# ideafisher/ssUnet-GAN

Hardware: AMD Instinct MI355X
Metric: train images/sec (512^2 tiles) (higher is better)
Workload: dtype f32; 1 GPU; UNet_R_SS_v2 generator + SRGAN-style discriminator, one G+D step (train_seg_gan.py:182-233), 16 x 3x512x512 tiles per GPU, fp32, Adam lr 2e-5; global_batch=16, tile=512, parallelism=dp1, dead_d_param_grads_of_g_step=computed

## Files before the change

### include/ssunet_hip.h

```cpp
#ifndef SSUNET_HIP_H
#define SSUNET_HIP_H

#include <stdint.h>

#ifdef __cplusplus
extern "C" {
#endif

#define SSG_OK 0
#define SSG_EINVAL (-1)
#define SSG_EALIGN (-2)

#define SSG_ACT_NONE 0
#define SSG_ACT_RELU 1
#define SSG_ACT_LRELU 2
#define SSG_ACT_SWISH 3

#define SSG_MAX_TAPS 9

const char* ssg_last_error(void);
int ssg_abi_version(void);

typedef struct {
  const float* in1; const float* in2;
// ... 39 lines not shown
int ssg_pack_weights_bf16x1_taps(const float* w_packed, int R, int Kp, int ntaps, int BN, void* out, void* stream);

int64_t ssg_conv2d_workspace_bytes(const ssg_conv_desc* d);

int ssg_conv2d_igemm_f32(const ssg_conv_desc* d, void* stream);
int ssg_conv2d_f32(const ssg_conv_desc* d, void* stream);
int ssg_conv2d_kernel_id(const ssg_conv_desc* d);
int ssg_conv2d_bnpart_rows(const ssg_conv_desc* d);

int ssg_pack_weights_f32(const float* w_oihw, int O, int I, int KH, int KW,
                         int transpose, int ntaps, const int* ky, const int* kx,
                         int kmode, int Cred_pad, int Kp, float* out, void* stream);
int ssg_pack_weights_scaled_f32(const float* w_oihw, int O, int I, int KH, int KW,
                                int transpose, int ntaps, const int* ky, const int* kx,
                                int kmode, int Cred_pad, int Kp, const float* sigma, float* out, void* stream);

typedef struct {
  const float* in1; const float* in2; int C1, C2, ld1, ld2;
  int N, H, W;
  const float* dout; int Cout, ldd; int GH, GW;
  int in_sy, in_sx;
  int ntaps; int dy[SSG_MAX_TAPS]; int dx[SSG_MAX_TAPS]; int ky[SSG_MAX_TAPS]; int kx[SSG_MAX_TAPS];
  int KH, KW, Cin_real;
  float* dw_oihw;
  float* ws; int64_t ws_bytes;
  int flags;
  const float* in_scale; const float* in_shift; int in_act; float in_slope;
} ssg_wgrad_desc;

int64_t ssg_conv2d_wgrad_workspace_bytes(const ssg_wgrad_desc* d);
int ssg_conv2d_wgrad_in_affine_ok(const ssg_wgrad_desc* d);
int ssg_conv2d_wgrad_f32(const ssg_wgrad_desc* d, void* stream);
int ssg_conv2d_wgrad_kernel_id(const ssg_wgrad_desc* d);
int ssg_wgrad_set_k32_mode(int mode);

int ssg_conv2d_wgrad_bf16x1_ok(const ssg_wgrad_desc* d);
int64_t ssg_conv2d_wgrad_bf16x1_workspace_bytes(const ssg_wgrad_desc* d);
int ssg_conv2d_wgrad_bf16x1_f32(const ssg_wgrad_desc* d, void* stream);
int ssg_conv2d_wgrad_bf16x1_kernel_id(const ssg_wgrad_desc* d);

int ssg_conv2d_wgrad_bf16x1_s2_ok(const ssg_wgrad_desc* d);
int64_t ssg_conv2d_wgrad_bf16x1_s2_workspace_bytes(const ssg_wgrad_desc* d);
int ssg_conv2d_wgrad_bf16x1_s2_f32(const ssg_wgrad_desc* d, void* stream);
int ssg_conv2d_wgrad_bf16x1_s2_kernel_id(const ssg_wgrad_desc* d);

int ssg_pixel_gate_fwd_f32(const float* x, int ldx, const float* g, int ldg, int64_t P, int C, float* y, int ldy, void* stream);
int ssg_pixel_gate_bwd_f32(const float* x, int ldx, const float* g, int ldg, const float* dy, int lddy, int64_t P, int C,
                           float* dx, int lddx, float* dg, int lddg, void* stream);

int64_t ssg_linear_fwd_workspace_bytes(int n, int k, int o);
int ssg_linear_fwd_f32(const float* x, int n, int k, int ldx, const float* w, int o, const float* bias, int act,
                       float slope, float* y, int ldy, float* ws, int64_t ws_bytes, void* stream);
int ssg_linear_wgrad_f32(const float* x, int n, int k, int ldx, const float* dy, int o, int ldd, float* dw, void* stream);

int ssg_pack_weights_bf16(const float* w, int O, int I, int transpose, int rows_pad, int Kp, void* out, void* stream);
int ssg_gemm_bf16(const void* x, int64_t P, int K, int ldx, const void* w_packed, int Kp, int N,
                  const void* res, int ldr, void* out, int ldo, void* stream);
int64_t ssg_gemm_wgrad_bf16_workspace_bytes(int64_t P, int M, int N);
int ssg_gemm_wgrad_bf16(const void* dy, int ldd, const void* x, int ldx, int64_t P, int M, int N, float* dw,
                        void* ws, int64_t ws_bytes, void* stream);

int ssg_conv2d_thin_bf16(const float* x, int N, int H, int W, int ldx, const float* w_oihw, int Cout, int Cin, int KH, int KW,
                         int stride, int pad_t, int pad_l, int OH, int OW, void* y, int ldy, void* stream);
int64_t ssg_conv2d_thin_bf16_wgrad_workspace_bytes(int N, int OH, int OW, int Cout, int KH, int KW);
int ssg_conv2d_thin_bf16_wgrad(const float* x, int N, int H, int W, int ldx, const void* dy, int lddy, int Cout, int Cin,
                               int KH, int KW, int stride, int pad_t, int pad_l, int OH, int OW, float* dw_oihw, void* ws,
                               void* stream);
int ssg_conv2d_thin_bf16_dgrad(const void* dy, int lddy, int N, int H, int W, const float* w_oihw, int Cout, int Cin, int KH, int KW,
                               int stride, int pad_t, int pad_l, int OH, int OW, float* dx, int lddx, void* stream);

int ssg_bn_stats_bf16(const void* x, int64_t P, int C, int ld, double* sums, int with_count, void* ws, void* stream);
int ssg_bn_apply_bf16(const void* x, int64_t P, int C, int ld, const float* scale, const float* shift,
                      const void* res, int ldr, int act, float slope, void* y, int ldy, void* stream);
int ssg_bn_bwd_reduce_bf16(const void* x, const void* y, const void* dy, int64_t P, int C, int ldx, int ldy, int lddy,
                           const float* mean, const float* invstd, const float* scale, const float* shift,
                           int act, float slope, double* sums, int with_count, void* ws, void* stream);
int ssg_bn_bwd_apply_bf16(const void* x, const void* y, const void* dy, int64_t P, int C, int ldx, int ldy, int lddy,
                          const float* mean, const float* invstd, const float* weight, const float* scale, const float* shift,
                          const double* sums, double count, int act, float slope, void* dx, int lddx, void* dres, int lddres,
                          float* dweight, float* dbias, void* stream);
int ssg_dwconv2d_fwd_bf16(const void* in, int N, int H, int W, int C, int ld, const float* w, const float* bias, int KH, int KW,
                          int stride, int pad_top, int pad_left, int OH, int OW, void* out, int ldo, void* stream);
int ssg_dwconv2d_dgrad_bf16(const void* dout, int lddo, int N, int H, int W, int C, const float* w, int KH, int KW, int stride,
                            int pad_top, int pad_left, int OH, int OW, void* dx, int lddx, void* stream);
int ssg_dwconv2d_wgrad_bf16(const void* in, int N, int H, int W, int C, int ld, const void* dout, int lddo, int KH, int KW,
                            int stride, int pad_top, int pad_left, int OH, int OW, float* dw, void* ws, void* stream);
int ssg_channel_scale_fwd_bf16(const void* x, int ldx, const float* s, int N, int64_t S, int C, void* y, int ldy, void* stream);
int ssg_sample_channel_sum_bf16(const void* a, int lda, const void* b, int ldb, int N, int64_t S, int C, float scale,
                                float* out, void* ws, void* stream);
int ssg_broadcast_rows_bf16(const float* s, int N, int64_t S, int C, float scale, void* y, int ldy, void* stream);
int ssg_add_bf16(const void* a, int lda, const void* b, int ldb, int64_t P, int C, void* out, int ldo, void* stream);
int ssg_convert_f32_to_bf16(const float* src, int ldsrc, int64_t P, int C, void* dst, int lddst, void* stream);
int ssg_convert_bf16_to_f32(const void* src, int ldsrc, int64_t P, int C, float* dst, int lddst, void* stream);

int ssg_nchw_to_nhwc_f32(const float* src, int N, int C, int H, int W, float* dst, int ld, void* stream);
int ssg_nhwc_to_nchw_f32(const float* src, int ld, int N, int C, int H, int W, float* dst, void* stream);

int64_t ssg_bn_workspace_bytes(int64_t P, int C);
int ssg_bn_stats_f32(const float* x, int64_t P, int C, int ld, double* sums, int with_count, void* ws, void* stream);
int64_t ssg_bn_stats_from_partials_workspace_bytes(int rows, int C);
int ssg_bn_stats_from_partials_f32(const double* part, int rows, int C, double* sums, double count, void* ws, void* stream);
int ssg_bn_finalize_f32(const double* sums, double count, int C, const float* weight, const float* bias,
                        float eps, float momentum, int var_mode,
                        float* running_mean, float* running_var,
                        float* mean, float* invstd, float* scale, float* shift, void* stream);

typedef struct ssg_bn_fin {
  const float* weight; const float* bias;
  float eps, momentum; int var_mode;
  float* running_mean; float* running_var;
  float* mean; float* invstd; float* scale; float* shift;
} ssg_bn_fin;
int ssg_bn_stats_finalize_f32(const float* x, int64_t P, int C, int ld, const ssg_bn_fin* fin, void* ws, void* stream);
int ssg_bn_stats_finalize_bf16(const void* x, int64_t P, int C, int ld, const ssg_bn_fin* fin, void* ws, void* stream);
int ssg_bn_stats_from_partials_finalize_f32(const double* part, int rows, int C, double count, const ssg_bn_fin* fin, void* ws, void* stream);
int ssg_bn_apply_f32(const float* x, int64_t P, int C, int ld, const float* scale, const float* shift,
                     const float* res, int ldr, int act, float slope, float* y, int ldy, void* stream);
int ssg_bn_bwd_reduce_f32(const float* x, const float* y, const float* dy, int64_t P, int C,
                          int ldx, int ldy, int lddy, const float* mean, const float* invstd,
                          const float* scale, const float* shift,
                          int act, float slope, double* sums, int with_count, void* ws, void* stream);
int ssg_bn_bwd_apply_f32(const float* x, const float* y, const float* dy, int64_t P, int C,
                         int ldx, int ldy, int lddy, const float* mean, const float* invstd,
                         const float* weight, const float* scale, const float* shift,
                         const double* sums, double count, int act, float slope,
                         float* dx, int lddx, float* dres, int lddres,
                         float* dweight, float* dbias, void* stream);
int ssg_bn_frozen_bwd_f32(const float* x, const float* y, const float* dy, int64_t P, int C, int ldx, int ldy, int lddy,
                          const float* mean, const float* invstd, const float* scale, const float* shift, int act, float slope,
                          float* dx, int lddx, float* dres, int lddres, double* sums, void* ws, void* stream);
int ssg_bn_fold_bwd_f32(const float* dwf, const float* w, int Cout, int64_t K, const float* s, const float* mean,
                        const float* invstd, const double* sums_g, float* dw, float* dgamma, float* dbeta, void* stream);

int ssg_maxpool2x2_fwd_f32(const float* x, int N, int H, int W, int C, int ldx, float* y, int ldy, uint8_t* idx, void* stream);
int ssg_maxpool2x2_bwd_f32(const float* dy, int lddy, const uint8_t* idx, int N, int H, int W, int C, float* dx, int lddx, void* stream);
int ssg_maxpool2x2_bwd_add_f32(const float* dy, int lddy, const uint8_t* idx, const float* res, int ldr, int N, int H, int W, int C,
                               float* dx, int lddx, void* stream);
int ssg_maxunpool2x2_fwd_f32(const float* x, int ldx, const uint8_t* idx, int N, int OH, int OW, int C, float* y, int ldy, void* stream);
int ssg_maxunpool2x2_bwd_f32(const float* dy, int lddy, const uint8_t* idx, int N, int OH, int OW, int C, float* dx, int lddx, void* stream);
int ssg_upsample2x_bilinear_fwd_f32(const float* x, int N, int H, int W, int C, int ldx, float* y, int ldy, void* stream);
int ssg_upsample2x_bilinear_bwd_f32(const float* dy, int lddy, int N, int H, int W, int C, float* dx, int lddx, void* stream);
int ssg_upsample2x_nearest_fwd_f32(const float* x, int N, int H, int W, int C, int ldx, float* y, int ldy, void* stream);
int ssg_upsample2x_nearest_bwd_f32(const float* dy, int lddy, int N, int H, int W, int C, float* dx, int lddx, void* stream);
int ssg_adaptive_avgpool_flat_fwd_f32(const float* x, int N, int H, int W, int C, int ldx, int OHW, float* y, void* stream);
int ssg_adaptive_avgpool_flat_bwd_f32(const float* dy, int N, int H, int W, int C, int OHW, float* dx, int lddx, void* stream);

int ssg_spade_conv_modulate_ok(const ssg_conv_desc* d);
int ssg_spade_conv_modulate_f32(const ssg_conv_desc* d, const float* x, int ldx, float* gamma, int ldg, void* stream);
int ssg_spade_modulate_fwd_f32(const float* x, int ldx, const float* gb, int ldgb, int64_t P, int C, float* y, int ldy, void* stream);
int ssg_spade_modulate_bwd_f32(const float* x, int ldx, const float* gb, int ldgb, const float* dy, int lddy, int64_t P, int C,
                               float* dx, int lddx, float* dgb, int lddgb, void* stream);
int ssg_spade_modulate_bwd_sums_f32(const float* x, int ldx, const float* gb, int ldgb, const float* dy, int lddy, int64_t P,
                                    int C, float* dx, int lddx, float* dgb, int lddgb, double* sums, void* ws, void* stream);
int ssg_act_bwd_f32(const float* y, int ldy, const float* dy, int lddy, int64_t P, int C, int act, float slope, float* dx, int lddx, void* stream);
int ssg_copy_channels_f32(const float* src, int ldsrc, int64_t P, int C, float* dst, int lddst, void* stream);
int ssg_add_f32(const float* a, const float* b, int64_t n, float* out, void* stream);
int ssg_nan_to_zero_f32(float* x, int64_t n, uint8_t* mask, void* stream);
int ssg_mask_zero_f32(const float* g, const uint8_t* mask, int64_t n, float* out, void* stream);

int64_t ssg_seg_loss_workspace_bytes(int N, int64_t S, int C);
int ssg_seg_loss_fwd_f32(const float* x, int ldx, const float* t, int ldt, int N, int64_t S, int C, int mc0,
                         float* res, double* stats, void* ws, void* stream);
int ssg_seg_loss_bwd_f32(const float* x, int ldx, const float* t, int ldt, int N, int64_t S, int C,
                         const float* res, const double* stats, const float* g_seg, const float* g_mse,
                         const float* g_bce, float* dx, int lddx, void* stream);
int ssg_bce_logits_const_fwd_f32(const float* x, int n, int ldx, float label, float* loss, void* stream);
int ssg_bce_logits_const_bwd_f32(const float* x, int n, int ldx, float label, const float* g, float* dx, int lddx, void* stream);

int ssg_clamp_adam_multi_f32(const void* const* ptrs, const int64_t* sizes, const int32_t* blk_tensor,
                             const int32_t* blk_chunk, int nblocks, float clip, double lr, double beta1,
                             double beta2, double eps, double weight_decay, double bias_corr1,
                             double bias_corr2_sqrt, void* stream);
int ssg_clamp_sgd_multi_f32(const void* const* ptrs, const int64_t* sizes, const int32_t* blk_tensor,
                            const int32_t* blk_chunk, int nblocks, float clip, double lr, double momentum,
                            double dampening, double weight_decay, int nesterov, void* stream);
int ssg_clamp_f32(float* x, int64_t n, float lo, float hi, void* stream);
int ssg_clamp_multi_f32(const void* const* ptrs, const int64_t* sizes, const int32_t* blk_tensor, const int32_t* blk_chunk,
                        int nblocks, int which, float lo, float hi, void* stream);

int ssg_channel_sum_f32(const float* x, int64_t P, int C, int ld, float* out, void* ws, void* stream);

int ssg_dwconv2d_fwd_f32(const float* in, int N, int H, int W, int C, int ld, const float* w, const float* bias, int KH, int KW,
                         int stride, int pad_top, int pad_left, int OH, int OW, float* out, int ldo, void* stream);
int ssg_dwconv2d_dgrad_f32(const float* dout, int lddo, int N, int H, int W, int C, const float* w, int KH, int KW, int stride,
                           int pad_top, int pad_left, int OH, int OW, float* dx, int lddx, void* stream);
int64_t ssg_dwconv2d_wgrad_workspace_bytes(int N, int OH, int OW, int C, int KH, int KW);
int ssg_dwconv2d_kernel_id(int op, int stride, int KH, int KW, int pad_left, int64_t NDH, int C, int aligned16);
int ssg_dwconv2d_wgrad_f32(const float* in, int N, int H, int W, int C, int ld, const float* dout, int lddo, int KH, int KW,
                           int stride, int pad_top, int pad_left, int OH, int OW, float* dw, void* ws, void* stream);
#define SSG_UNARY_SWISH 0
#define SSG_UNARY_SIGMOID 1
#define SSG_UNARY_GAUSSIAN 2
int ssg_unary_fwd_f32(const float* x, int ldx, int64_t P, int C, int op, float* y, int ldy, void* stream);
int ssg_unary_bwd_f32(const float* x, int ldx, const float* dy, int lddy, int64_t P, int C, int op, float* dx, int lddx, void* stream);
int ssg_mul_fwd_f32(const float* a, int lda, const float* b, int ldb, int64_t P, int C, float* y, int ldy, void* stream);
int ssg_mul_bwd_f32(const float* a, int lda, const float* b, int ldb, const float* dy, int lddy, int64_t P, int C,
                    float* da, int ldda, float* db, int lddb, void* stream);
int ssg_channel_scale_fwd_f32(const float* x, int ldx, const float* s, int N, int64_t S, int C, float* y, int ldy, void* stream);
int64_t ssg_sample_channel_sum_workspace_bytes(int N, int64_t S, int C);
int ssg_sample_channel_sum_f32(const float* a, int lda, const float* b, int ldb, int N, int64_t S, int C, float scale, float* out,
                               void* ws, void* stream);
int ssg_broadcast_rows_f32(const float* s, int N, int64_t S, int C, float scale, float* y, int ldy, void* stream);
int64_t ssg_spectral_norm_workspace_bytes(int rows, int cols);
int ssg_spectral_norm_fwd_f32(const float* W, int rows, int cols, float* u, float* v, int n_power_iterations, double eps,
                              float* W_out, float* sigma, void* ws, void* stream);
int ssg_spectral_norm_bwd_f32(const float* dWsn, const float* W, int rows, int cols, const float* u, const float* v,
                              const float* sigma, float* dW, void* ws, void* stream);

int ssg_se_gate_ok(int N, int C, int S);
int64_t ssg_se_gate_workspace_floats(int N, int C, int S);
int ssg_se_gate_fwd_f32(const float* sq, int ldq, int N, int C, const float* w1, const float* b1, const float* w2, const float* b2,
                        int S, float* h_pre, float* gate, int ldg, float* tmp, void* stream);
int ssg_se_gate_bwd_f32(const float* dgate, int ldd, const float* gate, int ldg, const float* h_pre, const float* sq, int ldq, int N, int C,
                        const float* w1, const float* w2, int S, float* dsq, int lds_, float* dw1, float* db1, float* dw2, float* db2,
                        float* tmp, void* stream);

int ssg_tool_mfma_peak_f32(float* scratch, int blocks, int iters, void* stream);
int ssg_tool_mfma_peak_bf16(float* scratch, int blocks, int iters, void* stream);
int ssg_tool_mfma_peak_bf16_data(float* scratch, int blocks, int iters, const void* data, void* stream);
int ssg_tool_mfma_peak_bf16_data16(float* scratch, int blocks, int iters, const void* data, void* stream);
int ssg_tool_copy_f32(const float* src, float* dst, int64_t n, void* stream);

int ssg_sw_gather_patches_u8_f32(const uint8_t* img, int H, int W, const int32_t* org, const int32_t* org_host, int P,
                                 int p_size, int out_size, float mean0, float mean1, float mean2,
                                 float rdenom0, float rdenom1, float rdenom2, float* out, void* stream);
int ssg_sw_merge_masks_f32_u8(const float* probs, int ld, int P, int C, int S, const int32_t* org, const int32_t* org_host,
                              const int32_t* weight, int p_size, int H, int W, uint8_t* out, void* stream);

#ifdef __cplusplus
}
#endif
#endif
```

### ssunet-gan_amd/_lib.py

```python
import ctypes as C
import os

import torch

_HERE = os.path.dirname(os.path.abspath(__file__))
LIB_PATH = os.environ.get('SSG_LIB_PATH') or os.path.join(_HERE, 'libssunet_hip.so')
MAX_TAPS = 9
ACT_NONE, ACT_RELU, ACT_LRELU, ACT_SWISH = 0, 1, 2, 3


class HipLibraryError(RuntimeError):
    pass


class ConvDesc(C.Structure):
    _fields_ = [
        ('in1', C.c_void_p), ('in2', C.c_void_p),
        ('C1', C.c_int), ('C2', C.c_int), ('ld1', C.c_int), ('ld2', C.c_int),
        ('N', C.c_int), ('H', C.c_int), ('W', C.c_int),
        ('w', C.c_void_p), ('Kp', C.c_int), ('kmode', C.c_int),
        ('bias', C.c_void_p),
        ('res', C.c_void_p), ('ldr', C.c_int),
        ('out', C.c_void_p), ('Cout', C.c_int), ('ldo', C.c_int),
        ('GH', C.c_int), ('GW', C.c_int), ('OH', C.c_int), ('OW', C.c_int),
        ('in_sy', C.c_int), ('in_sx', C.c_int), ('out_sy', C.c_int), ('out_sx', C.c_int),
        ('out_oy', C.c_int), ('out_ox', C.c_int),
        ('ntaps', C.c_int), ('dy', C.c_int * MAX_TAPS), ('dx', C.c_int * MAX_TAPS),
        ('act', C.c_int), ('slope', C.c_float),
        ('bnpart', C.c_void_p),
        ('ws', C.c_void_p), ('ws_bytes', C.c_int64),
        ('w_split', C.c_void_p), ('parity_merge', C.c_int),
        ('in_scale', C.c_void_p), ('in_shift', C.c_void_p), ('in_act', C.c_int), ('in_slope', C.c_float),
        ('bwd_x', C.c_void_p), ('bwd_ldx', C.c_int), ('bwd_scale', C.c_void_p), ('bwd_shift', C.c_void_p), ('bwd_mean', C.c_void_p),
        ('bwd_act', C.c_int), ('bwd_slope', C.c_float),
    ]


class WgradDesc(C.Structure):
    _fields_ = [
        ('in1', C.c_void_p), ('in2', C.c_void_p),
        ('C1', C.c_int), ('C2', C.c_int), ('ld1', C.c_int), ('ld2', C.c_int),
        ('N', C.c_int), ('H', C.c_int), ('W', C.c_int),
        ('dout', C.c_void_p), ('Cout', C.c_int), ('ldd', C.c_int), ('GH', C.c_int), ('GW', C.c_int),
        ('in_sy', C.c_int), ('in_sx', C.c_int),
        ('ntaps', C.c_int), ('dy', C.c_int * MAX_TAPS), ('dx', C.c_int * MAX_TAPS),
        ('ky', C.c_int * MAX_TAPS), ('kx', C.c_int * MAX_TAPS),
        ('KH', C.c_int), ('KW', C.c_int), ('Cin_real', C.c_int),
        ('dw_oihw', C.c_void_p),
        ('ws', C.c_void_p), ('ws_bytes', C.c_int64),
        ('flags', C.c_int),
        ('in_scale', C.c_void_p), ('in_shift', C.c_void_p), ('in_act', C.c_int), ('in_slope', C.c_float),
    ]


_P, _I, _L, _F, _D = C.c_void_p, C.c_int, C.c_int64, C.c_float, C.c_double


class BnFin(C.Structure):
    _fields_ = [('weight', C.c_void_p), ('bias', C.c_void_p), ('eps', C.c_float), ('momentum', C.c_float), ('var_mode', C.c_int),
                ('running_mean', C.c_void_p), ('running_var', C.c_void_p),
                ('mean', C.c_void_p), ('invstd', C.c_void_p), ('scale', C.c_void_p), ('shift', C.c_void_p)]


SIGNATURES = {
    'ssg_abi_version': [],
    'ssg_conv2d_igemm_f32': [C.POINTER(ConvDesc), _P],
    'ssg_conv2d_f32': [C.POINTER(ConvDesc), _P],
    'ssg_conv2d_kernel_id': [C.POINTER(ConvDesc)],
    'ssg_conv2d_bnpart_rows': [C.POINTER(ConvDesc)],
    'ssg_conv2d_workspace_bytes': [C.POINTER(ConvDesc)],
    'ssg_conv2d_thin_bf16': [_P, _I, _I, _I, _I, _P, _I, _I, _I, _I, _I, _I, _I, _I, _I, _P, _I, _P],
    'ssg_conv2d_thin_bf16_wgrad_workspace_bytes': [_I, _I, _I, _I, _I, _I],
    'ssg_conv2d_thin_bf16_wgrad': [_P, _I, _I, _I, _I, _P, _I, _I, _I, _I, _I, _I, _I, _I, _I, _I, _P, _P, _P],
    'ssg_conv2d_thin_bf16_dgrad': [_P, _I, _I, _I, _I, _P, _I, _I, _I, _I, _I, _I, _I, _I, _I, _P, _I, _P],
    'ssg_conv2d_split_bn': [C.POINTER(ConvDesc)],
    'ssg_conv2d_in_affine_ok': [C.POINTER(ConvDesc)],
    'ssg_conv2d_bwd_stats_ok': [C.POINTER(ConvDesc)],
    'ssg_conv2d_wgrad_in_affine_ok': [C.POINTER(WgradDesc)],
    'ssg_pack_weights_split_bytes': [_I, _I, _I],
    'ssg_conv_set_k32_mode': [_I],
    'ssg_wgrad_set_k32_mode': [_I],
    'ssg_pack_weights_split_bf16x3': [_P, _I, _I, _I, _P, _P],
    'ssg_conv2d_bf16x1_ok': [C.POINTER(ConvDesc)],
    'ssg_conv2d_bf16x1_kernel_id': [C.POINTER(ConvDesc)],
    'ssg_conv2d_bf16x1_f32': [C.POINTER(ConvDesc), _P, _P],
    'ssg_pack_weights_bf16x1_bytes': [_I, _I, _I],
    'ssg_pack_weights_bf16x1': [_P, _I, _I, _I, _P, _P],
    'ssg_conv2d_bf16x1_s2_ok': [C.POINTER(ConvDesc)],
    'ssg_conv2d_bf16x1_s2_kernel_id': [C.POINTER(ConvDesc)],
    'ssg_conv2d_bf16x1_s2_f32': [C.POINTER(ConvDesc), _P, _P],
    'ssg_conv2d_bf16x1_cls_ok': [C.POINTER(ConvDesc)],
    'ssg_conv2d_bf16x1_cls_kernel_id': [C.POINTER(ConvDesc)],
    'ssg_conv2d_bf16x1_cls_f32': [C.POINTER(ConvDesc), _P, _P],
    'ssg_pack_weights_bf16x1_taps_bytes': [_I, _I, _I, _I],
    'ssg_pack_weights_bf16x1_taps': [_P, _I, _I, _I, _I, _P, _P],
    'ssg_conv2d_wgrad_bf16x1_ok': [C.POINTER(WgradDesc)],
    'ssg_conv2d_wgrad_bf16x1_kernel_id': [C.POINTER(WgradDesc)],
    'ssg_conv2d_wgrad_bf16x1_workspace_bytes': [C.POINTER(WgradDesc)],
    'ssg_conv2d_wgrad_bf16x1_f32': [C.POINTER(WgradDesc), _P],
    'ssg_conv2d_wgrad_bf16x1_s2_ok': [C.POINTER(WgradDesc)],
    'ssg_conv2d_wgrad_bf16x1_s2_kernel_id': [C.POINTER(WgradDesc)],
    'ssg_conv2d_wgrad_bf16x1_s2_workspace_bytes': [C.POINTER(WgradDesc)],
    'ssg_conv2d_wgrad_bf16x1_s2_f32': [C.POINTER(WgradDesc), _P],
    'ssg_bn_stats_from_partials_workspace_bytes': [_I, _I],
    'ssg_bn_stats_from_partials_f32': [_P, _I, _I, _P, _D, _P, _P],
    'ssg_conv2d_wgrad_kernel_id': [C.POINTER(WgradDesc)],
    'ssg_pack_weights_f32': [_P, _I, _I, _I, _I, _I, _I, C.POINTER(C.c_int), C.POINTER(C.c_int), _I, _I, _I, _P, _P],
    'ssg_pack_weights_scaled_f32': [_P, _I, _I, _I, _I, _I, _I, C.POINTER(C.c_int), C.POINTER(C.c_int), _I, _I, _I, _P, _P, _P],
    'ssg_conv2d_wgrad_workspace_bytes': [C.POINTER(WgradDesc)],
    'ssg_conv2d_wgrad_f32': [C.POINTER(WgradDesc), _P],
    'ssg_nchw_to_nhwc_f32': [_P, _I, _I, _I, _I, _P, _I, _P],
    'ssg_nhwc_to_nchw_f32': [_P, _I, _I, _I, _I, _I, _P, _P],
    'ssg_bn_workspace_bytes': [_L, _I],
    'ssg_bn_stats_f32': [_P, _L, _I, _I, _P, _I, _P, _P],
    'ssg_bn_finalize_f32': [_P, _D, _I, _P, _P, _F, _F, _I, _P, _P, _P, _P, _P, _P, _P],
    'ssg_bn_apply_f32': [_P, _L, _I, _I, _P, _P, _P, _I, _I, _F, _P, _I, _P],
    'ssg_bn_bwd_reduce_f32': [_P, _P, _P, _L, _I, _I, _I, _I, _P, _P, _P, _P, _I, _F, _P, _I, _P, _P],
    'ssg_bn_bwd_apply_f32': [_P, _P, _P, _L, _I, _I, _I, _I, _P, _P, _P, _P, _P, _P, _D, _I, _F, _P, _I, _P, _I, _P, _P, _P],
    'ssg_bn_frozen_bwd_f32': [_P, _P, _P, _L, _I, _I, _I, _I, _P, _P, _P, _P, _I, _F, _P, _I, _P, _I, _P, _P, _P],
    'ssg_bn_fold_bwd_f32': [_P, _P, _I, _L, _P, _P, _P, _P, _P, _P, _P, _P],
    'ssg_maxpool2x2_fwd_f32': [_P, _I, _I, _I, _I, _I, _P, _I, _P, _P],
    'ssg_maxpool2x2_bwd_f32': [_P, _I, _P, _I, _I, _I, _I, _P, _I, _P],
    'ssg_maxpool2x2_bwd_add_f32': [_P, _I, _P, _P, _I, _I, _I, _I, _I, _P, _I, _P],
    'ssg_maxunpool2x2_fwd_f32': [_P, _I, _P, _I, _I, _I, _I, _P, _I, _P],
    'ssg_maxunpool2x2_bwd_f32': [_P, _I, _P, _I, _I, _I, _I, _P, _I, _P],
    'ssg_upsample2x_bilinear_fwd_f32': [_P, _I, _I, _I, _I, _I, _P, _I, _P],
    'ssg_upsample2x_bilinear_bwd_f32': [_P, _I, _I, _I, _I, _I, _P, _I, _P],
    'ssg_upsample2x_nearest_fwd_f32': [_P, _I, _I, _I, _I, _I, _P, _I, _P],
    'ssg_upsample2x_nearest_bwd_f32': [_P, _I, _I, _I, _I, _I, _P, _I, _P],
    'ssg_adaptive_avgpool_flat_fwd_f32': [_P, _I, _I, _I, _I, _I, _I, _P, _P],
    'ssg_adaptive_avgpool_flat_bwd_f32': [_P, _I, _I, _I, _I, _I, _P, _I, _P],
    'ssg_spade_conv_modulate_ok': [C.POINTER(ConvDesc)],
    'ssg_spade_conv_modulate_f32': [C.POINTER(ConvDesc), _P, _I, _P, _I, _P],
    'ssg_spade_modulate_fwd_f32': [_P, _I, _P, _I, _L, _I, _P, _I, _P],
    'ssg_spade_modulate_bwd_f32': [_P, _I, _P, _I, _P, _I, _L, _I, _P, _I, _P, _I, _P],
    'ssg_spade_modulate_bwd_sums_f32': [_P, _I, _P, _I, _P, _I, _L, _I, _P, _I, _P, _I, _P, _P, _P],
    'ssg_act_bwd_f32': [_P, _I, _P, _I, _L, _I, _I, _F, _P, _I, _P],
    'ssg_add_f32': [_P, _P, _L, _P, _P],
    'ssg_copy_channels_f32': [_P, _I, _L, _I, _P, _I, _P],
    'ssg_nan_to_zero_f32': [_P, _L, _P, _P],
    'ssg_mask_zero_f32': [_P, _P, _L, _P, _P],
    'ssg_seg_loss_workspace_bytes': [_I, _L, _I],
    'ssg_seg_loss_fwd_f32': [_P, _I, _P, _I, _I, _L, _I, _I, _P, _P, _P, _P],
    'ssg_seg_loss_bwd_f32': [_P, _I, _P, _I, _I, _L, _I, _P, _P, _P, _P, _P, _P, _I, _P],
    'ssg_bce_logits_const_fwd_f32': [_P, _I, _I, _F, _P, _P],
    'ssg_bce_logits_const_bwd_f32': [_P, _I, _I, _F, _P, _P, _I, _P],
    'ssg_clamp_adam_multi_f32': [_P, _P, _P, _P, _I, _F, _D, _D, _D, _D, _D, _D, _D, _P],
    'ssg_clamp_sgd_multi_f32': [_P, _P, _P, _P, _I, _F, _D, _D, _D, _D, _I, _P],
    'ssg_clamp_f32': [_P, _L, _F, _F, _P],
    'ssg_clamp_multi_f32': [_P, _P, _P, _P, _I, _I, _F, _F, _P],
    'ssg_channel_sum_f32': [_P, _L, _I, _I, _P, _P, _P],
    'ssg_dwconv2d_fwd_f32': [_P, _I, _I, _I, _I, _I, _P, _P, _I, _I, _I, _I, _I, _I, _I, _P, _I, _P],
    'ssg_dwconv2d_dgrad_f32': [_P, _I, _I, _I, _I, _I, _P, _I, _I, _I, _I, _I, _I, _I, _P, _I, _P],
    'ssg_dwconv2d_wgrad_workspace_bytes': [_I, _I, _I, _I, _I, _I],
    'ssg_dwconv2d_kernel_id': [_I, _I, _I, _I, _I, _L, _I, _I],
    'ssg_dwconv2d_wgrad_f32': [_P, _I, _I, _I, _I, _I, _P, _I, _I, _I, _I, _I, _I, _I, _I, _P, _P, _P],
    'ssg_unary_fwd_f32': [_P, _I, _L, _I, _I, _P, _I, _P],
    'ssg_unary_bwd_f32': [_P, _I, _P, _I, _L, _I, _I, _P, _I, _P],
    'ssg_mul_fwd_f32': [_P, _I, _P, _I, _L, _I, _P, _I, _P],
    'ssg_mul_bwd_f32': [_P, _I, _P, _I, _P, _I, _L, _I, _P, _I, _P, _I, _P],
    'ssg_channel_scale_fwd_f32': [_P, _I, _P, _I, _L, _I, _P, _I, _P],
    'ssg_sample_channel_sum_workspace_bytes': [_I, _L, _I],
    'ssg_sample_channel_sum_f32': [_P, _I, _P, _I, _I, _L, _I, _F, _P, _P, _P],
    'ssg_broadcast_rows_f32': [_P, _I, _L, _I, _F, _P, _I, _P],
    'ssg_spectral_norm_workspace_bytes': [_I, _I],
    'ssg_spectral_norm_fwd_f32': [_P, _I, _I, _P, _P, _I, _D, _P, _P, _P, _P],
    'ssg_spectral_norm_bwd_f32': [_P, _P, _I, _I, _P, _P, _P, _P, _P, _P],
    'ssg_pixel_gate_fwd_f32': [_P, _I, _P, _I, _L, _I, _P, _I, _P],
    'ssg_pixel_gate_bwd_f32': [_P, _I, _P, _I, _P, _I, _L, _I, _P, _I, _P, _I, _P],
    'ssg_linear_fwd_workspace_bytes': [_I, _I, _I],
    'ssg_linear_fwd_f32': [_P, _I, _I, _I, _P, _I, _P, _I, _F, _P, _I, _P, _L, _P],
    'ssg_linear_wgrad_f32': [_P, _I, _I, _I, _P, _I, _I, _P, _P],
    'ssg_pack_weights_bf16': [_P, _I, _I, _I, _I, _I, _P, _P],
    'ssg_gemm_bf16': [_P, _L, _I, _I, _P, _I, _I, _P, _I, _P, _I, _P],
    'ssg_gemm_wgrad_bf16_workspace_bytes': [_L, _I, _I],
    'ssg_gemm_wgrad_bf16': [_P, _I, _P, _I, _L, _I, _I, _P, _P, _L, _P],
    'ssg_bn_stats_finalize_f32': [_P, _L, _I, _I, C.POINTER(BnFin), _P, _P],
    'ssg_bn_stats_finalize_bf16': [_P, _L, _I, _I, C.POINTER(BnFin), _P, _P],
    'ssg_bn_stats_from_partials_finalize_f32': [_P, _I, _I, _D, C.POINTER(BnFin), _P, _P],
    'ssg_se_gate_ok': [_I, _I, _I],
    'ssg_se_gate_workspace_floats': [_I, _I, _I],
    'ssg_se_gate_fwd_f32': [_P, _I, _I, _I, _P, _P, _P, _P, _I, _P, _P, _I, _P, _P],
    'ssg_se_gate_bwd_f32': [_P, _I, _P, _I, _P, _P, _I, _I, _I, _P, _P, _I, _P, _I, _P, _P, _P, _P, _P, _P],
    'ssg_tool_mfma_peak_f32': [_P, _I, _I, _P],
    'ssg_tool_mfma_peak_bf16': [_P, _I, _I, _P],
    'ssg_tool_mfma_peak_bf16_data': [_P, _I, _I, _P, _P],
    'ssg_tool_mfma_peak_bf16_data16': [_P, _I, _I, _P, _P],
    'ssg_tool_copy_f32': [_P, _P, _L, _P],
    'ssg_sw_gather_patches_u8_f32': [_P, _I, _I, _P, _P, _I, _I, _I, _F, _F, _F, _F, _F, _F, _P, _P],
    'ssg_sw_merge_masks_f32_u8': [_P, _I, _I, _I, _I, _P, _P, _P, _I, _I, _I, _P, _P],
}

for _n in ('ssg_bn_stats', 'ssg_bn_apply', 'ssg_bn_bwd_reduce', 'ssg_bn_bwd_apply', 'ssg_dwconv2d_fwd', 'ssg_dwconv2d_dgrad', 'ssg_dwconv2d_wgrad', 'ssg_channel_scale_fwd', 'ssg_sample_channel_sum', 'ssg_broadcast_rows'):
    SIGNATURES[_n + '_bf16'] = SIGNATURES[_n + '_f32']
SIGNATURES['ssg_add_bf16'] = [_P, _I, _P, _I, _L, _I, _P, _I, _P]
SIGNATURES['ssg_convert_f32_to_bf16'] = [_P, _I, _L, _I, _P, _I, _P]
SIGNATURES['ssg_convert_bf16_to_f32'] = [_P, _I, _L, _I, _P, _I, _P]
_RESTYPES = {
    'ssg_conv2d_wgrad_workspace_bytes': C.c_int64,
    'ssg_conv2d_wgrad_bf16x1_workspace_bytes': C.c_int64,
    'ssg_conv2d_wgrad_bf16x1_s2_workspace_bytes': C.c_int64,
    'ssg_conv2d_workspace_bytes': C.c_int64,
    'ssg_pack_weights_split_bytes': C.c_int64,
    'ssg_pack_weights_bf16x1_bytes': C.c_int64,
    'ssg_pack_weights_bf16x1_taps_bytes': C.c_int64,
    'ssg_bn_workspace_bytes': C.c_int64,
    'ssg_se_gate_workspace_floats': C.c_int64,
    'ssg_seg_loss_workspace_bytes': C.c_int64,
    'ssg_dwconv2d_wgrad_workspace_bytes': C.c_int64,
    'ssg_spectral_norm_workspace_bytes': C.c_int64,
    'ssg_linear_fwd_workspace_bytes': C.c_int64,
    'ssg_sample_channel_sum_workspace_bytes': C.c_int64,
    'ssg_gemm_wgrad_bf16_workspace_bytes': C.c_int64,
    'ssg_conv2d_thin_bf16_wgrad_workspace_bytes': C.c_int64,
    'ssg_bn_stats_from_partials_workspace_bytes': C.c_int64,
}
_NO_STATUS = set(_RESTYPES) | {'ssg_abi_version', 'ssg_conv2d_split_bn', 'ssg_conv2d_in_affine_ok', 'ssg_conv2d_wgrad_in_affine_ok', 'ssg_conv2d_bwd_stats_ok', 'ssg_conv2d_kernel_id', 'ssg_conv2d_bnpart_rows', 'ssg_conv2d_bf16x1_ok', 'ssg_conv2d_bf16x1_kernel_id', 'ssg_conv2d_bf16x1_s2_ok', 'ssg_conv2d_bf16x1_s2_kernel_id', 'ssg_conv2d_bf16x1_cls_ok', 'ssg_conv2d_bf16x1_cls_kernel_id', 'ssg_conv2d_wgrad_bf16x1_ok', 'ssg_conv2d_wgrad_bf16x1_kernel_id', 'ssg_conv2d_wgrad_bf16x1_s2_ok', 'ssg_conv2d_wgrad_bf16x1_s2_kernel_id', 'ssg_conv2d_wgrad_kernel_id', 'ssg_dwconv2d_kernel_id',
                                'ssg_spade_conv_modulate_ok', 'ssg_se_gate_ok'}

ABI_VERSION = 10

_lib = None


def load():
    global _lib
    if _lib is not None:
        return _lib
    if not os.path.exists(LIB_PATH):
        raise HipLibraryError(
            'HIP extension not built: %s is missing. Run `python -c "import __graft_entry__ as g; g.build()"` '
            '(or `make -C ssunet-gan_amd/csrc`). There is no CPU fallback.' % LIB_PATH)
    lib = C.CDLL(LIB_PATH)
    lib.ssg_last_error.restype = C.c_char_p
    lib.ssg_last_error.argtypes = []
    for name, args in SIGNATURES.items():
        fn = getattr(lib, name)
        fn.argtypes = args
        fn.restype = _RESTYPES.get(name, C.c_int)
    got = lib.ssg_abi_version()
    if got != ABI_VERSION:
        raise HipLibraryError('%s reports ABI version %d, this package was written against %d: rebuild it '
                              '(`make -C ssunet-gan_amd/csrc`)' % (LIB_PATH, got, ABI_VERSION))
    _lib = lib
    return lib


def call(name, *args):
    lib = load()
    rc = getattr(lib, name)(*args)
    if name in _NO_STATUS:
        return rc
    if rc != 0:
        msg = lib.ssg_last_error().decode('utf-8', 'replace')
        raise HipLibraryError('%s failed (status %d): %s' % (name, rc, msg))
    return rc


def stream_ptr():
    return C.c_void_p(torch.cuda.current_stream().cuda_stream)


def require_gpu(t):
    if not t.is_cuda:
        raise HipLibraryError('ssunet-gan_amd ops run only on an MI355X (cuda/HIP) device; got a %s tensor. '
                              'There is no CPU fallback.' % t.device)


def ptr(t):
    return C.c_void_p(t.data_ptr()) if t is not None else C.c_void_p(0)
```

### ssunet-gan_amd/blocks.py

```python
import ctypes as C

import torch

from . import ops
from ._lib import ACT_NONE, ACT_RELU, call, ptr, stream_ptr
from .ops import (_act_bwd, _bn_bwd_impl, _bn_fwd_impl, _channel_sum, _conv_dgrad_impl, _conv_fwd_impl, _conv_wgrad_impl,
                  _ld, new_nhwc, to_nhwc)


class _BasicBlockFn(torch.autograd.Function):

    @staticmethod
    def forward(ctx, x1, x2, w1, g1, b1, rm1, rv1, w2, g2, b2, rm2, rv2, wsc, eps1, mom1, eps2, mom2, stride, var_mode, group):
        x1 = to_nhwc(x1)
        x2 = to_nhwc(x2) if x2 is not None else None
        ctx.x1m = x1m = ops.train_precision_mode() == 'bf16x1' and stride == 1
        p3 = 'bf16x1' if x1m else 'fp32'
        c1, part1 = _conv_fwd_impl(x1, x2, w1, None, stride, 1, ACT_NONE, 0.0, want_bn=True, precision=p3)
        y1 = None
        c2 = None
        if ops.BN_FUSE_INPUT and part1 is not None and not x1m:
            _, st1, cnt1 = _bn_fwd_impl(c1, g1, b1, rm1, rv1, None, eps1, mom1, ACT_RELU, 0.0, var_mode, group, part=part1, apply=False)
            r = _conv_fwd_impl(c1, None, w2, None, 1, 1, ACT_NONE, 0.0, want_bn=True, in_affine=(st1[2], st1[3], ACT_RELU, 0.0))
            if r is not None:
# ... 59 lines not shown
                None, None, None, None, None, None, None)


def basic_block(x1, x2, conv1, bn1, conv2, bn2, shortcut_conv, group=None):
    for bn in (bn1, bn2):
        if bn.track_running_stats and bn.num_batches_tracked is not None and not ops._synced(group):
            bn.num_batches_tracked.add_(1)
    var_mode = getattr(bn1, '_ssg_var_mode', 1 if group is not None else 0)
    return _BasicBlockFn.apply(x1, x2, conv1.weight, bn1.weight, bn1.bias, bn1.running_mean, bn1.running_var,
                               conv2.weight, bn2.weight, bn2.bias, bn2.running_mean, bn2.running_var,
                               shortcut_conv.weight if shortcut_conv is not None else None,
                               float(bn1.eps), float(bn1.momentum), float(bn2.eps), float(bn2.momentum),
                               int(conv1.stride[0]), var_mode, group)


def _fold_bwd(dwf, w, s, mean, invstd, sums_g, need_w, need_gb):
    o = w.shape[0]
    dw = torch.empty_like(dwf) if need_w else None
    dgb = torch.empty((2, o), dtype=torch.float32, device=w.device) if need_gb else None
    wc = w.detach().contiguous()
    call('ssg_bn_fold_bwd_f32', ptr(dwf), ptr(wc), o, wc.numel() // o, ptr(s), ptr(mean), ptr(invstd), ptr(sums_g), ptr(dw),
         ptr(dgb[0]) if need_gb else None, ptr(dgb[1]) if need_gb else None, stream_ptr())
    return dw, (dgb[0] if need_gb else None), (dgb[1] if need_gb else None)


class _FrozenBasicBlockFn(torch.autograd.Function):

    @staticmethod
    def forward(ctx, x1, x2, w1, g1, b1, w2, g2, b2, wsc, wf1, bf1, wf2, bf2, k1, k2, stride, record):
        x1 = to_nhwc(x1)
        x2 = to_nhwc(x2) if x2 is not None else None
        x1m = record and any(ctx.needs_input_grad) and ops.train_precision_mode() == 'bf16x1' and stride == 1
        p3 = 'bf16x1' if x1m else 'fp32'
        y1 = _conv_fwd_impl(x1, x2, wf1, bf1, stride, 1, ACT_RELU, 0.0, precision=p3)
        if wsc is not None:
            r = _conv_fwd_impl(x1, x2, wsc, None, stride, 0, ACT_NONE, 0.0)
        else:
            if x2 is not None:
                raise ValueError('identity shortcut with a two-tensor input')
            r = x1
        out = _conv_fwd_impl(y1, None, wf2, bf2, 1, 1, ACT_RELU, 0.0, res=r, precision=p3)
        if record and any(ctx.needs_input_grad):
            ctx.save_for_backward(x1, x2, y1, out, w1, w2, wsc, wf1, wf2, *k1, *k2)
            ctx.stride = stride
            ctx.x1m = x1m
        return out

    @staticmethod
    @torch.autograd.function.once_differentiable
    def backward(ctx, dout):
        x1, x2, y1, out, w1, w2, wsc, wf1, wf2, s1, m1, is1, s2, m2, is2 = ctx.saved_tensors
        stride = ctx.stride
        p3 = 'bf16x1' if ctx.x1m else 'fp32'
        dout = to_nhwc(dout)
        n, ca, h, w = x1.shape
        cb = x2.shape[1] if x2 is not None else 0
        need = ctx.needs_input_grad
        need_x1, need_x2 = need[0], (x2 is not None and need[1])
        need_w1, need_gb1, need_w2, need_gb2 = need[2], (need[3] or need[4]), need[5], (need[6] or need[7])
        need_wsc = wsc is not None and need[8]
        if stride != 1 and (need_x1 or need_x2):
            raise NotImplementedError('strided BasicBlock input gradient')
        g2, _, sums2 = ops._frozen_bwd(None, out, dout, None, None, None, None, ACT_RELU, 0.0)
        dw2 = dg2 = db2 = None
        if need_w2 or need[6]:
            dwf2 = _conv_wgrad_impl(y1, None, g2, w2.shape, 1, 1, precision=p3)
            dw2, dg2, db2 = _fold_bwd(dwf2, w2, s2, m2, is2, sums2, need_w2, need_gb2)
        elif need_gb2:
            db2 = sums2[:w2.shape[0]].float()
        dwsc = _conv_wgrad_impl(x1, x2, g2, wsc.shape, stride, 0) if need_wsc else None
        dw1 = dg1 = db1 = dx1 = dx2 = None
        if need_w1 or need_gb1 or need_x1 or need_x2:
            dy1 = _conv_dgrad_impl(g2, wf2, 1, 1, y1.shape[2], y1.shape[3], 0, y1.shape[1], precision=p3)
            g1, _, sums1 = ops._frozen_bwd(None, y1, dy1, None, None, None, None, ACT_RELU, 0.0)
            del dy1
            if need_w1 or need[3]:
                dwf1 = _conv_wgrad_impl(x1, x2, g1, w1.shape, stride, 1, precision=p3)
                dw1, dg1, db1 = _fold_bwd(dwf1, w1, s1, m1, is1, sums1, need_w1, need_gb1)
            elif need_gb1:
                db1 = sums1[:w1.shape[0]].float()
            if need_x1:
                part = _conv_dgrad_impl(g2, wsc, 1, 0, h, w, 0, ca) if wsc is not None else g2
                dx1 = _conv_dgrad_impl(g1, wf1, 1, 1, h, w, 0, ca, res=part, precision=p3)
            if need_x2:
                part = _conv_dgrad_impl(g2, wsc, 1, 0, h, w, ca, ca + cb)
                dx2 = _conv_dgrad_impl(g1, wf1, 1, 1, h, w, ca, ca + cb, res=part, precision=p3)
        return (dx1, dx2, dw1, dg1 if need[3] else None, db1 if need[4] else None, dw2, dg2 if need[6] else None,
                db2 if need[7] else None, dwsc, None, None, None, None, None, None, None, None)


def frozen_basic_block(x1, x2, conv1, bn1, conv2, bn2, shortcut_conv, folded, consts):
    wf1, bf1, wf2, bf2 = folded
    return _FrozenBasicBlockFn.apply(x1, x2, conv1.weight, bn1.weight, bn1.bias, conv2.weight, bn2.weight, bn2.bias,
                                     shortcut_conv.weight if shortcut_conv is not None else None, wf1, bf1, wf2, bf2,
                                     consts[0], consts[1], int(conv1.stride[0]), torch.is_grad_enabled())


def _spade_cat(wg, bg, wb, bb):
    stamp = tuple((t.data_ptr(), t._version) for t in (wg, bg, wb, bb)) + (ops._WEIGHT_EPOCH[0],)
    hit = wg.__dict__.get('_ssg_gb_cat')
    if hit is not None and hit[0] == stamp:
        return hit[1], hit[2]
    with torch.no_grad():
        w = torch.cat([wg.detach(), wb.detach()], 0).contiguous()
        b = torch.cat([bg.detach(), bb.detach()], 0).contiguous()
    ops._attach(wg, '_ssg_gb_cat', (stamp, w, b))
    return w, b


def _spade_fused_fwd(x, a, wgb, bgb, pad, out):
    o, i, kh, kw = wgb.shape
    n, c, h, w = x.shape
    cin = ops.pad4(a.shape[1])
    if kh != 3 or kw != 3 or pad != 1 or cin not in (4, 8) or o != 2 * c or c % 4:
        return None
    taps = ops._taps_fwd(kh, kw, pad)
    wpk, kp, kmode = ops._pack(wgb, 0, taps, cin, cin)
    d = ops._conv_desc(ops._at(a), cin, None, 0, (n, h, w), wpk.data_ptr(), kp, kmode, bgb, None, ops._at(out), o,
                       (h, w, h, w), 1, 1, (0, 0), taps, ACT_NONE, 0.0)
    if not call('ssg_spade_conv_modulate_ok', C.byref(d)):
        return None
    gamma = new_nhwc(n, c, h, w, x.device)
    with ops._Timed('thin32_cin_kernel<spade>' if ops.PROFILE is not None else None, 2.0 * n * h * w * o * a.shape[1] * 9):
        call('ssg_spade_conv_modulate_f32', C.byref(d), ptr(x), _ld(x), ptr(gamma), _ld(gamma), stream_ptr())
    return gamma


class _SpadeFn(torch.autograd.Function):

    @staticmethod
    def forward(ctx, x, wx, bx, ws, bs, wg, bg, wb, bb, pad):
        x = to_nhwc(x)
        n, c, h, w = x.shape
        seg = _conv_fwd_impl(x, None, wx, bx, 1, pad, ACT_NONE, 0.0)
        a = _conv_fwd_impl(seg, None, ws, bs, 1, pad, ACT_RELU, 0.0)
        wgb, bgb = _spade_cat(wg, bg, wb, bb)
        out = new_nhwc(n, c, h, w, x.device)
        gb = _spade_fused_fwd(x, a, wgb, bgb, pad, out)
        if gb is None:
            gb = _conv_fwd_impl(a, None, wgb, bgb, 1, pad, ACT_NONE, 0.0)
            with ops._hbm('spade_modulate_fwd', 16.0 * n * h * w * c):
                call('ssg_spade_modulate_fwd_f32', ptr(x), _ld(x), ptr(gb), _ld(gb), n * h * w, c, ptr(out), _ld(out), stream_ptr())
        ctx.save_for_backward(x, seg, a, gb, wx, ws, wgb)
        ctx.pad = pad
        return out

    @staticmethod
    @torch.autograd.function.once_differentiable
    def backward(ctx, dout):
        x, seg, a, gb, wx, ws, wgb = ctx.saved_tensors
        pad = ctx.pad
        dout = to_nhwc(dout)
        n, c, h, w = x.shape
        dxm = new_nhwc(n, c, h, w, x.device)
        dgb = new_nhwc(n, 2 * c, h, w, x.device)
        scratch = ops._ws(call('ssg_bn_workspace_bytes', n * h * w, c), x.device)
        sums = torch.empty(2 * c, dtype=torch.float64, device=x.device)
        with ops._hbm('spade_modulate_bwd', 4.0 * n * h * w * c * (3 + 3)):
            call('ssg_spade_modulate_bwd_sums_f32', ptr(x), _ld(x), ptr(gb), _ld(gb), ptr(dout), _ld(dout), n * h * w, c,
                 ptr(dxm), _ld(dxm), ptr(dgb), _ld(dgb), ptr(sums), ptr(scratch), stream_ptr())
        dwgb = _conv_wgrad_impl(a, None, dgb, wgb.shape, 1, pad)
        dbias_gb = sums.float()
        nh = a.shape[1]
        da = _conv_dgrad_impl(dgb, wgb, 1, pad, h, w, 0, nh)
        da = _act_bwd(a, da, ACT_RELU, 0.0)
        dws = _conv_wgrad_impl(seg, None, da, ws.shape, 1, pad)
        dbs = _channel_sum(da, nh)
        dseg = _conv_dgrad_impl(da, ws, 1, pad, h, w, 0, seg.shape[1])
        dwx = _conv_wgrad_impl(x, None, dseg, wx.shape, 1, pad)
        dbx = _channel_sum(dseg, seg.shape[1])
        dx = _conv_dgrad_impl(dseg, wx, 1, pad, h, w, 0, c, res=dxm) if ctx.needs_input_grad[0] else None
        return dx, dwx, dbx, dws, dbs, dwgb[:c], dbias_gb[:c], dwgb[c:], dbias_gb[c:], None


def spade_self(x, x2map, shared, gamma, beta):
    return _SpadeFn.apply(x, x2map.weight, x2map.bias, shared.weight, shared.bias, gamma.weight, gamma.bias,
                          beta.weight, beta.bias, int(x2map.padding[0]))
```

### ssunet-gan_amd/csrc/bn.hip

```cpp
#include "common.h"

namespace {

constexpr int RED_BLOCK = 256;
constexpr int MAX_PARTS = 1024;

struct RedGeom { int TQ, PR, groups, parts; long long rows_per_part; };

__host__ RedGeom red_geom(long long P, int C, int Q = 1) {
  RedGeom g;
  const int CQ = (C + 4 * Q - 1) / (4 * Q);
  g.TQ = CQ >= 64 ? 64 : 1;
  if (CQ < 64) { while (g.TQ < CQ) g.TQ <<= 1; }
  g.PR = RED_BLOCK / g.TQ;
  g.groups = (CQ + g.TQ - 1) / g.TQ;
  long long parts = (P + (long long)g.PR * 8 - 1) / ((long long)g.PR * 8);
  if (parts > MAX_PARTS) parts = MAX_PARTS;
  if (parts < 1) parts = 1;
  g.rows_per_part = (P + parts - 1) / parts;
  g.parts = (int)((P + g.rows_per_part - 1) / g.rows_per_part);
  return g;
}

template <int MODE, typename T>
// ... 3 lines not shown
    const float* __restrict__ scale, const float* __restrict__ shift, int act, float slope,
    int TQ, int PR, long long rows_per_part, double* __restrict__ part ,
    T* __restrict__ dx, int lddx, T* __restrict__ dres, int lddres ) {
  constexpr int Q = SsgQ<T>::value;
  constexpr int V = 4 * Q;
  __shared__ double red[2][RED_BLOCK][V];
  const int tid = threadIdx.x;
  const int tq = tid % TQ, pr = tid / TQ;
  const int cg = blockIdx.y * TQ + tq;
  const int CG = (C + V - 1) / V;
  const bool cok = cg < CG;
  const long long p0 = (long long)blockIdx.x * rows_per_part;
  long long p1 = p0 + rows_per_part; if (p1 > P) p1 = P;
  typedef typename SsgAcc<T>::type acc_t;
  acc_t s1[V], s2[V];
#pragma unroll
  for (int e = 0; e < V; ++e) { s1[e] = 0; s2[e] = 0; }
  float mu[V], is[V], sc[V], sh[V];
#pragma unroll
  for (int e = 0; e < V; ++e) { mu[e] = 0.f; is[e] = 0.f; sc[e] = 0.f; sh[e] = 0.f; }
  if (MODE == 1 && cok) {
#pragma unroll
    for (int e = 0; e < V; ++e) {
      const int c = V * cg + e;
      if (c < C) { mu[e] = mean[c]; is[e] = invstd[c]; if ((!y || act == SSG_ACT_SWISH) && scale) { sc[e] = scale[c]; sh[e] = shift[c]; } }
    }
  }
  if (MODE == 3 && cok) {
#pragma unroll
    for (int e = 0; e < V; ++e) {
      const int c = V * cg + e;
      if (c < C) {
        if (mean) { mu[e] = mean[c]; is[e] = invstd[c]; }
        if (scale) sc[e] = scale[c];
        if (shift) sh[e] = shift[c];
      }
    }
  }
  if (cok) {
    for (long long p = p0 + pr; p < p1; p += PR) {
      f32x4 xq[Q];
      if (MODE == 3 && !x) {
#pragma unroll
        for (int q = 0; q < Q; ++q) xq[q] = f32x4{0.f, 0.f, 0.f, 0.f};
      } else {
        ldq(x + p * ldx + V * cg, xq);
      }
      if (MODE == 0) {
#pragma unroll
        for (int q = 0; q < Q; ++q)
#pragma unroll
          for (int e = 0; e < 4; ++e) { const acc_t v = (acc_t)xq[q][e]; s1[4 * q + e] += v; s2[4 * q + e] += v * v; }
      } else if (MODE == 2) {
#pragma unroll
        for (int q = 0; q < Q; ++q)
#pragma unroll
          for (int e = 0; e < 4; ++e) s1[4 * q + e] += (acc_t)xq[q][e];
      } else {
        f32x4 gq[Q], yq[Q];
        ldq(dy + p * lddy + V * cg, gq);
        const bool use_y = act != SSG_ACT_NONE && act != SSG_ACT_SWISH && y;
        if (use_y) ldq(y + p * ldy + V * cg, yq);
#pragma unroll
        for (int q = 0; q < Q; ++q) {
#pragma unroll
          for (int e = 0; e < 4; ++e) {
            const int k = 4 * q + e;
            float g = gq[q][e];
            const float xv = xq[q][e];
            if (act == SSG_ACT_SWISH) {
              g *= ssg_swish_grad(xv * sc[k] + sh[k]);
            } else if (act != SSG_ACT_NONE) {
              const float yv = use_y ? yq[q][e] : xv * sc[k] + sh[k];
              if (!(yv > 0.f)) g *= (act == SSG_ACT_RELU ? 0.f : slope);
            }
            const acc_t xh = ((acc_t)xv - (acc_t)mu[k]) * (acc_t)is[k];
            s1[k] += (acc_t)g;
            if (MODE == 1 || mean) s2[k] += (acc_t)g * xh;
            if (MODE == 3) gq[q][e] = g;
          }
        }
        if (MODE == 3) {
          if (dres) stq(dres + p * lddres + V * cg, gq);
          if (dx) {
            if (scale) {
#pragma unroll
              for (int q = 0; q < Q; ++q)
#pragma unroll
                for (int e = 0; e < 4; ++e) gq[q][e] *= sc[4 * q + e];
            }
            stq(dx + p * lddx + V * cg, gq);
          }
        }
      }
    }
  }
#pragma unroll
  for (int e = 0; e < V; ++e) { red[0][tid][e] = (double)s1[e]; red[1][tid][e] = (double)s2[e]; }
  __syncthreads();
  if (pr == 0 && cok) {
    double a1[V], a2[V];
#pragma unroll
    for (int e = 0; e < V; ++e) { a1[e] = 0; a2[e] = 0; }
    for (int r = 0; r < PR; ++r)
#pragma unroll
      for (int e = 0; e < V; ++e) { a1[e] += red[0][r * TQ + tq][e]; a2[e] += red[1][r * TQ + tq][e]; }
    const int Cpad = V * CG;
    double* dst = part + (size_t)blockIdx.x * 2 * Cpad;
#pragma unroll
    for (int e = 0; e < V; ++e) { dst[V * cg + e] = a1[e]; dst[Cpad + V * cg + e] = a2[e]; }
  }
}

__global__ __launch_bounds__(RED_BLOCK) void modulate_bwd_sums_kernel(
    const float* __restrict__ x, int ldx, const float* __restrict__ gb, int ldgb, const float* __restrict__ dy, int lddy,
    long long P, int C, float* __restrict__ dx, int lddx, float* __restrict__ dgb, int lddgb,
    int TQ, int PR, long long rows_per_part, double* __restrict__ part ) {
  __shared__ double red[2][RED_BLOCK][4];
  const int tid = threadIdx.x;
  const int tq = tid % TQ, pr = tid / TQ;
  const int cq = blockIdx.y * TQ + tq;
  const int CQ = C / 4;
  const bool cok = cq < CQ;
  const long long p0 = (long long)blockIdx.x * rows_per_part;
  long long p1 = p0 + rows_per_part; if (p1 > P) p1 = P;
  double s1[4] = {0, 0, 0, 0}, s2[4] = {0, 0, 0, 0};
  if (cok) {
    for (long long p = p0 + pr; p < p1; p += PR) {
      const f32x4 xv = *(const f32x4*)(x + p * ldx + 4 * cq);
      const f32x4 g = *(const f32x4*)(gb + p * ldgb + 4 * cq);
      const f32x4 d = *(const f32x4*)(dy + p * lddy + 4 * cq);
      const f32x4 dg = d * xv;
      st4(dx + p * lddx + 4 * cq, d * (1.f + g));
      st4(dgb + p * lddgb + 4 * cq, dg);
      st4(dgb + p * lddgb + C + 4 * cq, d);
#pragma unroll
      for (int e = 0; e < 4; ++e) { s1[e] += (double)dg[e]; s2[e] += (double)d[e]; }
    }
  }
#pragma unroll
  for (int e = 0; e < 4; ++e) { red[0][tid][e] = s1[e]; red[1][tid][e] = s2[e]; }
  __syncthreads();
  if (pr == 0 && cok) {
    double a1[4] = {0, 0, 0, 0}, a2[4] = {0, 0, 0, 0};
    for (int r = 0; r < PR; ++r)
#pragma unroll
      for (int e = 0; e < 4; ++e) { a1[e] += red[0][r * TQ + tq][e]; a2[e] += red[1][r * TQ + tq][e]; }
    double* dst = part + (size_t)blockIdx.x * 2 * C;
#pragma unroll
    for (int e = 0; e < 4; ++e) { dst[4 * cq + e] = a1[e]; dst[C + 4 * cq + e] = a2[e]; }
  }
}

constexpr int FIN_LANES = 32;

struct BnFin {
  const float* weight; const float* bias; float eps, momentum; int var_mode;
  float* running_mean; float* running_var; float* mean; float* invstd; float* scale; float* shift;
};

__device__ __forceinline__ void bn_finalize_channel(int c, double s1, double s2, double count, const BnFin& f) {
  const double m = s1 / count;
  double var = fma(-m, m, s2 / count);
  if (var < 0) var = 0;
  double is;
  if (f.var_mode == 0) is = 1.0 / sqrt(var + (double)f.eps);
  else is = 1.0 / sqrt(var < (double)f.eps ? (double)f.eps : var);
  const float mf = (float)m, isf = (float)is;
  f.mean[c] = mf; f.invstd[c] = isf;
  const float w = f.weight ? f.weight[c] : 1.f, b = f.bias ? f.bias[c] : 0.f;
  const float sc = w * isf;
  f.scale[c] = sc; f.shift[c] = fmaf(-mf, sc, b);
  if (f.running_mean) f.running_mean[c] = fmaf(f.momentum, mf, (1.f - f.momentum) * f.running_mean[c]);
  if (f.running_var) {
    const double unb = count > 1 ? var * count / (count - 1) : var;
    f.running_var[c] = fmaf(f.momentum, (float)unb, (1.f - f.momentum) * f.running_var[c]);
  }
}

__global__ __launch_bounds__(32 * FIN_LANES) void col_reduce_final_kernel(const double* __restrict__ part, int parts, int C, int C4,
                                                                          double* __restrict__ sums, float* __restrict__ fsum,
                                                                          double count_out, BnFin fin, double fin_count) {
  __shared__ double red[2][FIN_LANES][32];
  const int cl = threadIdx.x & 31, lane = threadIdx.x >> 5;
  const int c = blockIdx.x * 32 + cl;
  double a1 = 0, a2 = 0;
  if (c < C) {
#pragma unroll 4
    for (int b = lane; b < parts; b += FIN_LANES) { a1 += part[(size_t)b * 2 * C4 + c]; a2 += part[(size_t)b * 2 * C4 + C4 + c]; }
  }
  red[0][lane][cl] = a1; red[1][lane][cl] = a2;
  __syncthreads();
  if (lane == 0 && c < C) {
    double t1 = 0, t2 = 0;
#pragma unroll
    for (int k = 0; k < FIN_LANES; ++k) { t1 += red[0][k][cl]; t2 += red[1][k][cl]; }
    if (sums) { sums[c] = t1; sums[C + c] = t2; }
    if (fsum) fsum[c] = (float)t1;
    if (fin.mean) bn_finalize_channel(c, t1, t2, fin_count, fin);
  }
  if (sums && count_out > 0 && blockIdx.x == 0 && threadIdx.x == 0) sums[2 * C] = count_out;
}

__global__ void bn_finalize_kernel(const double* __restrict__ sums, double count_arg, int C, BnFin fin) {
  const int c = blockIdx.x * blockDim.x + threadIdx.x;
  if (c >= C) return;
  const double count = count_arg > 0 ? count_arg : sums[2 * C];
  bn_finalize_channel(c, sums[c], sums[C + c], count, fin);
}

template <typename T>
__global__ __launch_bounds__(256) void bn_apply_kernel(const T* __restrict__ x, long long P, int C, int ld,
                                                       const float* __restrict__ scale, const float* __restrict__ shift,
                                                       const T* __restrict__ res, int ldr, int act, float slope,
                                                       T* __restrict__ y, int ldy) {
  constexpr int Q = SsgQ<T>::value;
  const int CG = C / (4 * Q);
  const long long total = P * CG;
  SSG_CHUNK_LOOP(i, total) {
    const long long p = i / CG; const int c0 = 4 * Q * (int)(i - p * CG);
    f32x4 xv[Q], rv[Q], o[Q];
    ldq(x + p * ld + c0, xv);
    if (res) ldq(res + p * ldr + c0, rv);
#pragma unroll
    for (int q = 0; q < Q; ++q) {
      const f32x4 sc = *(const f32x4*)(scale + c0 + 4 * q), sh = *(const f32x4*)(shift + c0 + 4 * q);
      f32x4 v = xv[q] * sc + sh;
      if (res) v += rv[q];
#pragma unroll
      for (int e = 0; e < 4; ++e) v[e] = ssg_act(v[e], act, slope);
      o[q] = v;
    }
    stq(y + p * ldy + c0, o);
  }
}

template <typename T>
__global__ __launch_bounds__(256) void bn_bwd_apply_kernel(
    const T* __restrict__ x, const T* __restrict__ y, const T* __restrict__ dy, long long P, int C, int ldx,
    int ldy, int lddy, const float* __restrict__ mean, const float* __restrict__ invstd, const float* __restrict__ weight,
    const float* __restrict__ scale, const float* __restrict__ shift,
    const double* __restrict__ sums, double count_arg, int act, float slope, T* __restrict__ dx, int lddx,
    T* __restrict__ dres, int lddres, float* __restrict__ dweight, float* __restrict__ dbias) {
  const double count = count_arg > 0 ? count_arg : sums[2 * C];
  if (blockIdx.x == 0) {
    for (int c = threadIdx.x; c < C; c += 256) {
      if (dweight) dweight[c] = (float)sums[C + c];
      if (dbias) dbias[c] = (float)sums[c];
    }
  }
  typedef typename SsgAcc<T>::type acc_t;
  extern __shared__ double kc_raw[];
  acc_t* kc = (acc_t*)kc_raw;
  acc_t* k_mean = kc; acc_t* k_is = kc + C; acc_t* k_ws = kc + 2 * C; acc_t* k_m1 = kc + 3 * C; acc_t* k_m2 = kc + 4 * C;
  for (int c = threadIdx.x; c < C; c += 256) {
    const double is = (double)invstd[c];
    k_mean[c] = (acc_t)mean[c]; k_is[c] = (acc_t)is; k_ws[c] = (acc_t)((weight ? (double)weight[c] : 1.0) * is);
    k_m1[c] = (acc_t)(sums[c] / count); k_m2[c] = (acc_t)(sums[C + c] / count);
  }
  __syncthreads();
  constexpr int Q = SsgQ<T>::value;
  const int CG = C / (4 * Q);
  const long long totalg = P * CG;
  SSG_CHUNK_LOOP(i, totalg) {
    const long long p = i / CG; const int c0 = 4 * Q * (int)(i - p * CG);
    f32x4 gq[Q], xq[Q], yq[Q], oq[Q];
    ldq(dy + p * lddy + c0, gq);
    ldq(x + p * ldx + c0, xq);
    const bool use_y = act != SSG_ACT_NONE && act != SSG_ACT_SWISH && y;
    if (use_y) ldq(y + p * ldy + c0, yq);
#pragma unroll
    for (int q = 0; q < Q; ++q) {
      const int cb = c0 + 4 * q;
      f32x4 g = gq[q];
      const f32x4 xv = xq[q];
      if (act == SSG_ACT_SWISH) {
        const f32x4 z = xv * *(const f32x4*)(scale + cb) + *(const f32x4*)(shift + cb);
#pragma unroll
        for (int e = 0; e < 4; ++e) g[e] *= ssg_swish_grad(z[e]);
      } else if (act != SSG_ACT_NONE) {
        const f32x4 yv = use_y ? yq[q] : xv * *(const f32x4*)(scale + cb) + *(const f32x4*)(shift + cb);
#pragma unroll
        for (int e = 0; e < 4; ++e) if (!(yv[e] > 0.f)) g[e] *= (act == SSG_ACT_RELU ? 0.f : slope);
      }
      gq[q] = g;
      if (dx) {
        f32x4 o;
#pragma unroll
        for (int e = 0; e < 4; ++e) {
          const int c = cb + e;
          const acc_t xh = ((acc_t)xv[e] - k_mean[c]) * k_is[c];
          o[e] = (float)(k_ws[c] * ((acc_t)g[e] - k_m1[c] - xh * k_m2[c]));
        }
        oq[q] = o;
      }
    }
    if (dres) stq(dres + p * lddres + c0, gq);
    if (dx) stq(dx + p * lddx + c0, oq);
  }
}

int elem_grid(long long total) { return ssg_elem_grid(total, 4); }

template <int MODE, typename T>
int run_reduce(const T* x, const T* y, const T* dy, long long P, int C, int ldx, int ldy, int lddy,
               const float* scale, const float* shift,
// ... 84 lines not shown
}

extern "C" int ssg_bn_stats_f32(const float* x, int64_t P, int C, int ld, double* sums, int with_count, void* ws, void* stream) {
  return bn_stats_impl<float>(x, P, C, ld, sums, with_count, ws, stream);
}
extern "C" int ssg_bn_stats_bf16(const void* x, int64_t P, int C, int ld, double* sums, int with_count, void* ws, void* stream) {
  return bn_stats_impl<ssg_bf16>((const ssg_bf16*)x, P, C, ld, sums, with_count, ws, stream);
}

namespace {
constexpr int FOLD_Z = 64;
__global__ __launch_bounds__(256) void bnpart_fold_kernel(const double* __restrict__ part, int rows, int C, int rows_per_z,
                                                          double* __restrict__ out ) {
  __shared__ double red[2][8][32];
  const int cl = threadIdx.x & 31, rl = threadIdx.x >> 5;
  const int c = blockIdx.x * 32 + cl;
  const int r0 = blockIdx.y * rows_per_z;
  int r1 = r0 + rows_per_z; if (r1 > rows) r1 = rows;
  double a1 = 0, a2 = 0;
  if (c < C)
    for (int r = r0 + rl; r < r1; r += 8) { a1 += part[(size_t)r * 2 * C + c]; a2 += part[(size_t)r * 2 * C + C + c]; }
  red[0][rl][cl] = a1; red[1][rl][cl] = a2;
  __syncthreads();
  if (rl == 0 && c < C) {
    double t1 = 0, t2 = 0;
#pragma unroll
    for (int k = 0; k < 8; ++k) { t1 += red[0][k][cl]; t2 += red[1][k][cl]; }
    out[(size_t)blockIdx.y * 2 * C + c] = t1; out[(size_t)blockIdx.y * 2 * C + C + c] = t2;
  }
}
}

extern "C" int64_t ssg_bn_stats_from_partials_workspace_bytes(int rows, int C) {
  return rows > 4 * FOLD_Z ? (int64_t)FOLD_Z * 2 * C * (int64_t)sizeof(double) : 16;
}

extern "C" int ssg_bn_stats_from_partials_f32(const double* part, int rows, int C, double* sums, double count, void* ws, void* stream) {
  SSG_REQUIRE(part && sums && ws && rows > 0 && C > 0, SSG_EINVAL, "bn_stats_from_partials: bad args");
  hipStream_t st = (hipStream_t)stream;
  const double* src = part; int nrows = rows;
  if (rows > 4 * FOLD_Z) {
    const int rpz = (rows + FOLD_Z - 1) / FOLD_Z;
    const int nz = (rows + rpz - 1) / rpz;
    hipLaunchKernelGGL(bnpart_fold_kernel, dim3((unsigned)((C + 31) / 32), (unsigned)nz), dim3(256), 0, st, part, rows, C, rpz, (double*)ws);
    SSG_LAUNCH_CHECK();
    src = (const double*)ws; nrows = nz;
  }
  hipLaunchKernelGGL(col_reduce_final_kernel, dim3((unsigned)((C + 31) / 32)), dim3(32 * FIN_LANES), 0, st, src, nrows, C, C, sums, (float*)nullptr, count, BnFin{}, 0.0);
  SSG_LAUNCH_CHECK();
  return SSG_OK;
}

extern "C" int ssg_channel_sum_f32(const float* x, int64_t P, int C, int ld, float* out, void* ws, void* stream) {
  SSG_REQUIRE(x && out && ws && P > 0 && C > 0, SSG_EINVAL, "channel_sum: bad args");
  SSG_REQUIRE(ld % 4 == 0 && ld >= C && ssg_aligned16(x), SSG_EALIGN, "channel_sum: alignment");
  return run_reduce<2, float>(x, nullptr, nullptr, P, C, ld, 0, 0, nullptr, nullptr, nullptr, nullptr, 0, 0.f, nullptr, out, ws, (hipStream_t)stream);
}

extern "C" int ssg_bn_finalize_f32(const double* sums, double count, int C, const float* weight, const float* bias,
                                   float eps, float momentum, int var_mode, float* running_mean, float* running_var,
                                   float* mean, float* invstd, float* scale, float* shift, void* stream) {
  SSG_REQUIRE(sums && mean && invstd && scale && shift && C > 0, SSG_EINVAL, "bn_finalize: bad args");
  const BnFin fin{weight, bias, eps, momentum, var_mode, running_mean, running_var, mean, invstd, scale, shift};
  hipLaunchKernelGGL(bn_finalize_kernel, dim3((unsigned)((C + 127) / 128)), dim3(128), 0, (hipStream_t)stream, sums, count, C, fin);
  SSG_LAUNCH_CHECK();
  return SSG_OK;
}

namespace {
template <typename T>
int bn_stats_finalize_impl(const T* x, int64_t P, int C, int ld, const ssg_bn_fin* f, void* ws, void* stream) {
  SSG_REQUIRE(x && f && ws && P > 0 && C > 0 && f->mean && f->invstd && f->scale && f->shift, SSG_EINVAL, "bn_stats_finalize: bad args");
  SSG_REQUIRE(C % (4 * SsgQ<T>::value) == 0 && ld % (4 * SsgQ<T>::value) == 0 && ld >= C && ssg_aligned16(x), SSG_EALIGN,
              "bn_stats_finalize: C / ld must be multiples of 4 (fp32) or 8 (bf16), rows 16-byte aligned");
  const BnFin fin{f->weight, f->bias, f->eps, f->momentum, f->var_mode, f->running_mean, f->running_var, f->mean, f->invstd, f->scale, f->shift};
  return run_reduce<0, T>(x, nullptr, nullptr, P, C, ld, 0, 0, nullptr, nullptr, nullptr, nullptr, 0, 0.f, nullptr, nullptr, ws, (hipStream_t)stream,
                          0.0, fin, (double)P);
}
}

extern "C" int ssg_bn_stats_finalize_f32(const float* x, int64_t P, int C, int ld, const ssg_bn_fin* fin, void* ws, void* stream) {
  return bn_stats_finalize_impl<float>(x, P, C, ld, fin, ws, stream);
}
extern "C" int ssg_bn_stats_finalize_bf16(const void* x, int64_t P, int C, int ld, const ssg_bn_fin* fin, void* ws, void* stream) {
  return bn_stats_finalize_impl<ssg_bf16>((const ssg_bf16*)x, P, C, ld, fin, ws, stream);
}

extern "C" int ssg_bn_stats_from_partials_finalize_f32(const double* part, int rows, int C, double count, const ssg_bn_fin* f, void* ws, void* stream) {
  SSG_REQUIRE(part && f && ws && rows > 0 && C > 0 && count > 0 && f->mean && f->invstd && f->scale && f->shift, SSG_EINVAL,
              "bn_stats_from_partials_finalize: bad args");
  hipStream_t st = (hipStream_t)stream;
  const BnFin fin{f->weight, f->bias, f->eps, f->momentum, f->var_mode, f->running_mean, f->running_var, f->mean, f->invstd, f->scale, f->shift};
  const double* src = part; int nrows = rows;
  if (rows > 4 * FOLD_Z) {
    const int rpz = (rows + FOLD_Z - 1) / FOLD_Z;
    const int nz = (rows + rpz - 1) / rpz;
    hipLaunchKernelGGL(bnpart_fold_kernel, dim3((unsigned)((C + 31) / 32), (unsigned)nz), dim3(256), 0, st, part, rows, C, rpz, (double*)ws);
    SSG_LAUNCH_CHECK();
    src = (const double*)ws; nrows = nz;
  }
  hipLaunchKernelGGL(col_reduce_final_kernel, dim3((unsigned)((C + 31) / 32)), dim3(32 * FIN_LANES), 0, st, src, nrows, C, C, (double*)nullptr,
                     (float*)nullptr, 0.0, fin, count);
  SSG_LAUNCH_CHECK();
  return SSG_OK;
}

extern "C" int ssg_bn_apply_f32(const float* x, int64_t P, int C, int ld, const float* scale, const float* shift,
                                const float* res, int ldr, int act, float slope, float* y, int ldy, void* stream) {
  return bn_apply_impl<float>(x, P, C, ld, scale, shift, res, ldr, act, slope, y, ldy, stream);
}
extern "C" int ssg_bn_apply_bf16(const void* x, int64_t P, int C, int ld, const float* scale, const float* shift,
                                 const void* res, int ldr, int act, float slope, void* y, int ldy, void* stream) {
  return bn_apply_impl<ssg_bf16>((const ssg_bf16*)x, P, C, ld, scale, shift, (const ssg_bf16*)res, ldr, act, slope, (ssg_bf16*)y, ldy, stream);
}

extern "C" int ssg_bn_bwd_reduce_f32(const float* x, const float* y, const float* dy, int64_t P, int C, int ldx, int ldy,
                                     int lddy, const float* mean, const float* invstd, const float* scale, const float* shift,
                                     int act, float slope, double* sums, int with_count, void* ws, void* stream) {
  return bn_bwd_reduce_impl<float>(x, y, dy, P, C, ldx, ldy, lddy, mean, invstd, scale, shift, act, slope, sums, with_count, ws, stream);
}
extern "C" int ssg_bn_bwd_reduce_bf16(const void* x, const void* y, const void* dy, int64_t P, int C, int ldx, int ldy,
                                      int lddy, const float* mean, const float* invstd, const float* scale, const float* shift,
                                      int act, float slope, double* sums, int with_count, void* ws, void* stream) {
  return bn_bwd_reduce_impl<ssg_bf16>((const ssg_bf16*)x, (const ssg_bf16*)y, (const ssg_bf16*)dy, P, C, ldx, ldy, lddy, mean, invstd, scale, shift,
                                      act, slope, sums, with_count, ws, stream);
}

extern "C" int ssg_bn_bwd_apply_f32(const float* x, const float* y, const float* dy, int64_t P, int C, int ldx, int ldy,
                                    int lddy, const float* mean, const float* invstd, const float* weight,
                                    const float* scale, const float* shift, const double* sums,
                                    double count, int act, float slope, float* dx, int lddx, float* dres, int lddres,
                                    float* dweight, float* dbias, void* stream) {
  return bn_bwd_apply_impl<float>(x, y, dy, P, C, ldx, ldy, lddy, mean, invstd, weight, scale, shift, sums, count, act, slope, dx, lddx, dres,
                                  lddres, dweight, dbias, stream);
}
extern "C" int ssg_bn_bwd_apply_bf16(const void* x, const void* y, const void* dy, int64_t P, int C, int ldx, int ldy,
                                     int lddy, const float* mean, const float* invstd, const float* weight,
                                     const float* scale, const float* shift, const double* sums,
                                     double count, int act, float slope, void* dx, int lddx, void* dres, int lddres,
                                     float* dweight, float* dbias, void* stream) {
  return bn_bwd_apply_impl<ssg_bf16>((const ssg_bf16*)x, (const ssg_bf16*)y, (const ssg_bf16*)dy, P, C, ldx, ldy, lddy, mean, invstd, weight, scale,
                                     shift, sums, count, act, slope, (ssg_bf16*)dx, lddx, (ssg_bf16*)dres, lddres, dweight, dbias, stream);
}

extern "C" int ssg_spade_modulate_bwd_sums_f32(const float* x, int ldx, const float* gb, int ldgb, const float* dy, int lddy, int64_t P,
                                               int C, float* dx, int lddx, float* dgb, int lddgb, double* sums, void* ws, void* stream) {
  SSG_REQUIRE(x && gb && dy && dx && dgb && sums && ws && P > 0 && C > 0 && C % 4 == 0 && ldgb >= C && lddgb >= 2 * C, SSG_EINVAL,
              "modulate_bwd_sums: bad args");
  const RedGeom g = red_geom(P, C);
  double* part = (double*)ws;
  hipStream_t st = (hipStream_t)stream;
  hipLaunchKernelGGL(modulate_bwd_sums_kernel, dim3((unsigned)g.parts, (unsigned)g.groups), dim3(RED_BLOCK), 0, st, x, ldx, gb, ldgb, dy, lddy,
                     (long long)P, C, dx, lddx, dgb, lddgb, g.TQ, g.PR, g.rows_per_part, part);
  SSG_LAUNCH_CHECK();
  hipLaunchKernelGGL(col_reduce_final_kernel, dim3((unsigned)((C + 31) / 32)), dim3(32 * FIN_LANES), 0, st, part, g.parts, C, C, sums, nullptr, 0.0, BnFin{}, 0.0);
  SSG_LAUNCH_CHECK();
  return SSG_OK;
}

extern "C" int ssg_bn_frozen_bwd_f32(const float* x, const float* y, const float* dy, int64_t P, int C, int ldx, int ldy, int lddy,
                                     const float* mean, const float* invstd, const float* scale, const float* shift, int act, float slope,
                                     float* dx, int lddx, float* dres, int lddres, double* sums, void* ws, void* stream) {
  SSG_REQUIRE(dy && sums && ws && P > 0 && C > 0, SSG_EINVAL, "bn_frozen_bwd: bad args");
  SSG_REQUIRE(act == SSG_ACT_NONE || act == SSG_ACT_RELU || act == SSG_ACT_LRELU || act == SSG_ACT_SWISH, SSG_EINVAL, "bn_frozen_bwd: unknown activation");
  SSG_REQUIRE((mean != nullptr) == (invstd != nullptr) && (!mean || x), SSG_EINVAL, "bn_frozen_bwd: mean / invstd come together and need x");
  SSG_REQUIRE(act == SSG_ACT_NONE || (y && act != SSG_ACT_SWISH) || (x && scale && shift), SSG_EINVAL,
              "bn_frozen_bwd: activation gradient needs y (ReLU family only) or (x, scale, shift)");
  const bool use_y = y && (act == SSG_ACT_RELU || act == SSG_ACT_LRELU);
  SSG_REQUIRE(C % 4 == 0 && lddy % 4 == 0 && lddy >= C && (!x || (ldx % 4 == 0 && ldx >= C)) && (!use_y || (ldy % 4 == 0 && ldy >= C)) &&
                  (!dx || (lddx % 4 == 0 && lddx >= C)) && (!dres || (lddres % 4 == 0 && lddres >= C)) && ssg_aligned16(dy) && ssg_aligned16(x) &&
                  (!use_y || ssg_aligned16(y)) && ssg_aligned16(dx) && ssg_aligned16(dres),
              SSG_EALIGN, "bn_frozen_bwd: C / ld must be multiples of 4, ld >= C, rows 16-byte aligned");
  const RedGeom g = red_geom(P, C, 1);
  double* part = (double*)ws;
  hipStream_t st = (hipStream_t)stream;
  hipLaunchKernelGGL((col_reduce_kernel<3, float>), dim3((unsigned)g.parts, (unsigned)g.groups), dim3(RED_BLOCK), 0, st, x, use_y ? y : nullptr, dy,
                     (long long)P, C, ldx, ldy, lddy, mean, invstd, scale, shift, act, slope, g.TQ, g.PR, g.rows_per_part, part, dx, lddx, dres, lddres);
  SSG_LAUNCH_CHECK();
  hipLaunchKernelGGL(col_reduce_final_kernel, dim3((unsigned)((C + 31) / 32)), dim3(32 * FIN_LANES), 0, st, part, g.parts, C, C, sums, (float*)nullptr, 0.0,
                     BnFin{}, 0.0);
  SSG_LAUNCH_CHECK();
  return SSG_OK;
}

namespace {
constexpr int FOLD_BLOCK = 256;
__global__ __launch_bounds__(FOLD_BLOCK) void bn_fold_bwd_kernel(const float* __restrict__ dwf, const float* __restrict__ w, long long K,
                                                                 const float* __restrict__ s, const float* __restrict__ mean,
                                                                 const float* __restrict__ invstd, const double* __restrict__ sums_g,
                                                                 float* __restrict__ dw, float* __restrict__ dgamma, float* __restrict__ dbeta) {
  __shared__ double red[FOLD_BLOCK];
  const int o = blockIdx.x, tid = threadIdx.x;
  const float* a = dwf + (size_t)o * K;
  const float so = s[o];
  double t = 0;
  if (dgamma) {
    const float* b = w + (size_t)o * K;
    for (long long k = tid; k < K; k += FOLD_BLOCK) t += (double)a[k] * (double)b[k];
  }
  if (dw) {
    float* d = dw + (size_t)o * K;
    for (long long k = tid; k < K; k += FOLD_BLOCK) d[k] = a[k] * so;
  }
  if (!dgamma) return;
  red[tid] = t;
  __syncthreads();
  for (int h = FOLD_BLOCK / 2; h > 0; h >>= 1) {
    if (tid < h) red[tid] += red[tid + h];
    __syncthreads();
  }
  if (tid == 0) {
    const double sg = sums_g[o];
    dgamma[o] = (float)((red[0] - (double)mean[o] * sg) * (double)invstd[o]);
    dbeta[o] = (float)sg;
  }
}
}

extern "C" int ssg_bn_fold_bwd_f32(const float* dwf, const float* w, int Cout, int64_t K, const float* s, const float* mean,
                                   const float* invstd, const double* sums_g, float* dw, float* dgamma, float* dbeta, void* stream) {
  SSG_REQUIRE(dwf && s && Cout > 0 && K > 0 && (dw || dgamma), SSG_EINVAL, "bn_fold_bwd: bad args");
  SSG_REQUIRE((dgamma != nullptr) == (dbeta != nullptr), SSG_EINVAL, "bn_fold_bwd: dgamma and dbeta come together");
  SSG_REQUIRE(!dgamma || (w && mean && invstd && sums_g), SSG_EINVAL, "bn_fold_bwd: dgamma / dbeta need w, mean, invstd, sums_g");
  hipLaunchKernelGGL(bn_fold_bwd_kernel, dim3((unsigned)Cout), dim3(FOLD_BLOCK), 0, (hipStream_t)stream, dwf, w, (long long)K, s, mean, invstd, sums_g,
                     dw, dgamma, dbeta);
  SSG_LAUNCH_CHECK();
  return SSG_OK;
}
```

### ssunet-gan_amd/csrc/conv_thin4.hip

```cpp
#include "common.h"
#include "conv_thin.h"

namespace {

struct T4Args {
  const float* in; const float* w; const float* bias; const float* res; float* out;
  int C, ld, N, H, W, Kp, kmode, ldr, Cout, ldo, ntaps;
  int tapidx[9];
  int act; float slope;
  int groups, waves_per_group, total_units, strips, ybands;
  int rh;
  int nt_store;
  float* gsave; int ldg;
};

constexpr int RH_CIN = 16;
constexpr int RH_COUT = 8;
constexpr unsigned OOB = 0xffffffffu;

__device__ __forceinline__ f32x4 ldbuf4(__amdgpu_buffer_rsrc_t rs, unsigned off) {
  return __builtin_bit_cast(f32x4, __builtin_amdgcn_raw_buffer_load_b128(rs, off, 0, 0));
}

__device__ __forceinline__ float act_apply(float v, int act, float slope) {
  if (act == SSG_ACT_RELU) return v < 0.f ? 0.f : v;
  if (act == SSG_ACT_LRELU) return v > 0.f ? v : v * slope;
  return v;
}


template <int KS, int PF, bool HAS_RES>
__global__ __launch_bounds__(256) void thin4_cin_kernel(const T4Args a) {
  constexpr int R = KS / 2, NT = KS * KS, RING = KS + PF;
  const int lane = threadIdx.x & 63, j = lane & 3, b = lane >> 2;
  const int wid = blockIdx.x * 4 + (threadIdx.x >> 6);
  const int cg = wid % a.groups, wg = wid / a.groups;
  if (wg >= a.waves_per_group) return;
  const unsigned npix = (unsigned)(a.N * a.H * a.W);
  const auto in_rs = __builtin_amdgcn_make_buffer_rsrc(const_cast<float*>(a.in), 0, (int)(npix * (unsigned)a.ld * 4u), 0x00020000);
  const unsigned ldb = (unsigned)a.ld * 4u;
  const auto res_rs = __builtin_amdgcn_make_buffer_rsrc(const_cast<float*>(HAS_RES ? a.res : a.in), 0,
                                                        (int)(npix * (unsigned)(HAS_RES ? a.ldr : a.ld) * 4u), 0x00020000);

  const int co = cg * 64 + lane;
  f32x4 wv[NT];
#pragma unroll
  for (int p = 0; p < NT; ++p) {
    const int t = a.tapidx[KS == 3 ? p : 4];
    wv[p] = (co < a.Cout && t >= 0) ? *(const f32x4*)(a.w + (size_t)co * a.Kp + t * 4) : f32x4{0.f, 0.f, 0.f, 0.f};
  }
  const int cb = cg * 64 + 4 * b;
  const bool st_ok = cb < ((a.Cout + 3) & ~3);
  f32x4 bv = {0.f, 0.f, 0.f, 0.f}, cmask;
#pragma unroll
  for (int i = 0; i < 4; ++i) {
    cmask[i] = (cb + i < a.Cout) ? 1.f : 0.f;
    if (a.bias) bv[i] = (cb + i < a.Cout) ? a.bias[cb + i] : 0.f;
  }
  const bool is_relu = a.act == SSG_ACT_RELU;
  const float neg_slope = a.act == SSG_ACT_LRELU ? a.slope : 1.f;
  f32x4 pend = {0.f, 0.f, 0.f, 0.f};
  float* pend_ptr = nullptr;

  for (int u = wg; u < a.total_units; u += a.waves_per_group) {
    const int xs = u % a.strips; const int r0 = u / a.strips;
    const int yb = r0 % a.ybands, n = r0 / a.ybands;
    const int x = xs * 4 + j;
    const int y0 = yb * RH_CIN;
    const int y1 = y0 + RH_CIN < a.H ? y0 + RH_CIN : a.H;
    unsigned coloff[KS];
#pragma unroll
    for (int e = 0; e < KS; ++e) {
      const int ix = x + e - R;
      coloff[e] = (unsigned)ix < (unsigned)a.W ? (unsigned)ix * ldb : OOB;
    }
    const unsigned imgoff = (unsigned)(n * a.H) * (unsigned)a.W * ldb;
    auto load_row = [&](f32x4* dst, int iy) {
      const bool rok = (unsigned)iy < (unsigned)a.H;
      const unsigned ro = imgoff + (unsigned)iy * (unsigned)a.W * ldb;
#pragma unroll
      for (int e = 0; e < KS; ++e) dst[e] = ldbuf4(in_rs, (rok && coloff[e] != OOB) ? ro + coloff[e] : OOB);
    };
    f32x4 v[RING][KS];
#pragma unroll
    for (int q = 0; q < KS + PF - 1; ++q) load_row(v[q], y0 - R + q);
    f32x4 rvr[HAS_RES ? RING : 1];
    auto load_res = [&](int yy) -> f32x4 {
      const bool ok = x < a.W && st_ok && yy < y1;
      return ldbuf4(res_rs, ok ? ((unsigned)((n * a.H + yy) * a.W + x) * (unsigned)a.ldr + (unsigned)cb) * 4u : OOB);
    };
    if (HAS_RES) rvr[0] = load_res(y0);
    for (int y = y0; y < y1; y += RING) {
#pragma unroll
      for (int r = 0; r < RING; ++r) {
        if (y + r < y1) {
          if (pend_ptr) { if (a.nt_store) __builtin_nontemporal_store(pend, (f32x4*)pend_ptr); else *(f32x4*)pend_ptr = pend; }
          load_row(v[(r + KS + PF - 1) % RING], y + r - R + KS + PF - 1);
          const size_t pix = (size_t)(n * a.H + y + r) * a.W + x;
          f32x4 rv = {0.f, 0.f, 0.f, 0.f};
          if (HAS_RES) { rvr[(r + 1) % RING] = load_res(y + r + 1); rv = rvr[r]; }
          f32x4 acc0 = {0.f, 0.f, 0.f, 0.f}, acc1 = {0.f, 0.f, 0.f, 0.f};
#pragma unroll
          for (int q = 0; q < KS; ++q)
#pragma unroll
            for (int e = 0; e < KS; ++e)
#pragma unroll
              for (int c = 0; c < 4; c += 2) {
                acc0 = __builtin_amdgcn_mfma_f32_4x4x1f32(wv[q * KS + e][c], v[(r + q) % RING][e][c], acc0, 0, 0, 0);
                acc1 = __builtin_amdgcn_mfma_f32_4x4x1f32(wv[q * KS + e][c + 1], v[(r + q) % RING][e][c + 1], acc1, 0, 0, 0);
              }
          const f32x4 t = acc0 + acc1 + bv + rv * cmask;
#pragma unroll
          for (int i = 0; i < 4; ++i) pend[i] = (t[i] < 0.f ? (is_relu ? 0.f : t[i] * neg_slope) : t[i]) * cmask[i];
          pend_ptr = (x < a.W && st_ok) ? a.out + pix * a.ldo + cb : nullptr;
        }
      }
    }
  }
  if (pend_ptr) *(f32x4*)pend_ptr = pend;
}

typedef float f32x2 __attribute__((ext_vector_type(2)));

__device__ __forceinline__ f32x2 ldbuf2(__amdgpu_buffer_rsrc_t rs, unsigned off) {
  return __builtin_bit_cast(f32x2, __builtin_amdgcn_raw_buffer_load_b64(rs, off, 0, 0));
}

constexpr int RH_K36 = 16;

template <int MODE, int PF, bool NT, int CIN = 4>
__global__ __launch_bounds__(256) void thin32_cin_kernel(const T4Args a) {
  constexpr bool HAS_RES = MODE >= 1, SPADE = MODE == 2;
  constexpr int CH = CIN / 2;
  typedef float vrow_t __attribute__((ext_vector_type(CH)));
  constexpr int AUX = NT ? 2 : 0;
  constexpr int RING = 3 + PF;
  const int lane = threadIdx.x & 63, l31 = lane & 31, h = lane >> 5;
  const int wid = __builtin_amdgcn_readfirstlane(blockIdx.x * 4 + (threadIdx.x >> 6));
  const int cg = wid % a.groups, wg = wid / a.groups;
  if (wg >= a.waves_per_group) return;
  const unsigned npix = (unsigned)(a.N * a.H * a.W);
  const auto in_rs = __builtin_amdgcn_make_buffer_rsrc(const_cast<float*>(a.in), 0, (int)(npix * (unsigned)a.ld * 4u), 0x00020000);
  const auto out_rs = __builtin_amdgcn_make_buffer_rsrc(a.out, 0, (int)(npix * (unsigned)a.ldo * 4u), 0x00020000);
  const auto res_rs = __builtin_amdgcn_make_buffer_rsrc(const_cast<float*>(HAS_RES ? a.res : a.in), 0,
                                                        (int)(npix * (unsigned)(HAS_RES ? a.ldr : a.ld) * 4u), 0x00020000);
  const auto g_rs = __builtin_amdgcn_make_buffer_rsrc(SPADE ? a.gsave : a.out, 0, (int)(npix * (unsigned)(SPADE ? a.ldg : a.ldo) * 4u), 0x00020000);
  const unsigned ldb = (unsigned)a.ld * 4u, ldob = (unsigned)a.ldo * 4u, ldrb = (unsigned)a.ldr * 4u, ldgb = (unsigned)a.ldg * 4u;
  const int Cmod = a.Cout >> 1;

  float wB[2][9 * CH], bv[2], keep[2];
  unsigned vo_out[2], vo_res[2];
  unsigned vo_g = OOB;
#pragma unroll
  for (int f = 0; f < 2; ++f) {
    const int cm = cg * 32 + l31;
    const int co = SPADE ? (cm < Cmod ? f * Cmod + cm : a.Cout) : cg * 64 + f * 32 + l31;
#pragma unroll
    for (int p = 0; p < 9; ++p) {
      const int t = a.tapidx[p];
      const bool ok = co < a.Cout && t >= 0;
#pragma unroll
      for (int j = 0; j < CH; ++j) wB[f][CH * p + j] = ok ? a.w[(size_t)co * a.Kp + t * CIN + CH * h + j] : 0.f;
    }
    bv[f] = (a.bias && co < a.Cout) ? a.bias[co] : 0.f;
    keep[f] = co < a.Cout ? 1.f : 0.f;
    const bool cok = SPADE ? cm < Cmod : co < ((a.Cout + 3) & ~3);
    const int cch = SPADE ? cm : co;
    vo_out[f] = cok ? 4u * (unsigned)h * ldob + (unsigned)cch * 4u : OOB;
    vo_res[f] = cok ? 4u * (unsigned)h * ldrb + (unsigned)cch * 4u : OOB;
    if (SPADE) vo_g = cok ? 4u * (unsigned)h * ldgb + (unsigned)cch * 4u : OOB;
  }
  const bool is_relu = a.act == SSG_ACT_RELU;
  const float neg_slope = a.act == SSG_ACT_LRELU ? a.slope : 1.f;

  for (int u = wg; u < a.total_units; u += a.waves_per_group) {
    const int xs = u % a.strips; const int r0 = u / a.strips;
    const int yb = r0 % a.ybands, n = r0 / a.ybands;
    const int x0 = xs * 32, x = x0 + l31;
    const int y0 = yb * RH_K36;
    const int y1 = y0 + RH_K36 < a.H ? y0 + RH_K36 : a.H;
    unsigned coloff[3];
#pragma unroll
    for (int e = 0; e < 3; ++e) {
      const int ix = x + e - 1;
      coloff[e] = (unsigned)ix < (unsigned)a.W ? (unsigned)ix * ldb + (unsigned)(4 * CH) * (unsigned)h : OOB;
    }
    const unsigned imgoff = (unsigned)(n * a.H) * (unsigned)a.W * ldb;
    auto load_row = [&](vrow_t* dst, int iy) {
      const bool rok = (unsigned)iy < (unsigned)a.H;
      const unsigned ro = imgoff + (unsigned)iy * (unsigned)a.W * ldb;
#pragma unroll
      for (int e = 0; e < 3; ++e) {
        const unsigned off = (rok && coloff[e] != OOB) ? ro + coloff[e] : OOB;
        if constexpr (CIN == 4) dst[e] = ldbuf2(in_rs, off); else dst[e] = ldbuf4(in_rs, off);
      }
    };
    unsigned inw = 0;
#pragma unroll
    for (int q = 0; q < 16; ++q) inw |= (x0 + (q & 3) + 8 * (q >> 2) + 4 * h < a.W ? 1u : 0u) << q;
    const bool full = x0 + 32 <= a.W;
    vrow_t v[RING][3];
#pragma unroll
    for (int q = 0; q < 2 + PF; ++q) load_row(v[q], y0 - 1 + q);
    auto mma_row = [&](f32x16 (&acc)[2], int r) {
#pragma unroll
      for (int f = 0; f < 2; ++f)
#pragma unroll
        for (int q = 0; q < 16; ++q) acc[f][q] = 0.f;
#pragma unroll
      for (int q = 0; q < 3; ++q)
#pragma unroll
        for (int e = 0; e < 3; ++e)
#pragma unroll
          for (int j = 0; j < CH; ++j)
#pragma unroll
            for (int f = 0; f < 2; ++f)
              acc[f] = __builtin_amdgcn_mfma_f32_32x32x2f32(v[(r + q) % RING][e][j], wB[f][CH * (q * 3 + e) + j], acc[f], 0, 0, 0);
    };
    auto store_row_full = [&](const f32x16 (&acc)[2], int yy) {
      const unsigned rowpix = (unsigned)((n * a.H + yy) * a.W + x0);
      float rv[2][16];
      const unsigned (&vo)[2] = vo_out; const unsigned (&vr)[2] = vo_res;
      if (HAS_RES) {
#pragma unroll
        for (int f = 0; f < (SPADE ? 1 : 2); ++f)
#pragma unroll
          for (int q = 0; q < 16; ++q)
            rv[f][q] = __builtin_bit_cast(float, __builtin_amdgcn_raw_buffer_load_b32(
                res_rs, vr[f], (int)((rowpix + (unsigned)((q & 3) + 8 * (q >> 2))) * ldrb), 0));
      }
      if (SPADE) {
#pragma unroll
        for (int q = 0; q < 16; ++q) {
          const float g = acc[0][q] + bv[0], bt = acc[1][q] + bv[1];
          const unsigned pq = rowpix + (unsigned)((q & 3) + 8 * (q >> 2));
          __builtin_amdgcn_raw_buffer_store_b32(__builtin_bit_cast(unsigned, g), g_rs, vo_g, (int)(pq * ldgb), AUX);
          __builtin_amdgcn_raw_buffer_store_b32(__builtin_bit_cast(unsigned, fmaf(rv[0][q], 1.f + g, bt)), out_rs, vo[0], (int)(pq * ldob), AUX);
        }
        return;
      }
#pragma unroll
      for (int f = 0; f < 2; ++f)
#pragma unroll
        for (int q = 0; q < 16; ++q) {
          float t = acc[f][q] + bv[f];
          if (HAS_RES) t += rv[f][q];
          t = (t < 0.f ? (is_relu ? 0.f : t * neg_slope) : t) * keep[f];
          __builtin_amdgcn_raw_buffer_store_b32(__builtin_bit_cast(unsigned, t), out_rs, vo[f],
                                                (int)((rowpix + (unsigned)((q & 3) + 8 * (q >> 2))) * ldob), AUX);
        }
    };
    auto store_row_edge = [&](const f32x16 (&acc)[2], int yy) {
      const unsigned rowpix = (unsigned)((n * a.H + yy) * a.W + x0);
      if (yy >= y1) return;
      if (SPADE) {
#pragma unroll
        for (int q = 0; q < 16; ++q) {
          if ((inw >> q) & 1u) {
            const unsigned pq = rowpix + (unsigned)((q & 3) + 8 * (q >> 2));
            const float g = acc[0][q] + bv[0], bt = acc[1][q] + bv[1];
            const float xv = __builtin_bit_cast(float, __builtin_amdgcn_raw_buffer_load_b32(res_rs, vo_res[0], (int)(pq * ldrb), 0));
            __builtin_amdgcn_raw_buffer_store_b32(__builtin_bit_cast(unsigned, g), g_rs, vo_g, (int)(pq * ldgb), AUX);
            __builtin_amdgcn_raw_buffer_store_b32(__builtin_bit_cast(unsigned, fmaf(xv, 1.f + g, bt)), out_rs, vo_out[0], (int)(pq * ldob), AUX);
          }
        }
        return;
      }
#pragma unroll
      for (int f = 0; f < 2; ++f)
#pragma unroll
        for (int q = 0; q < 16; ++q) {
          if ((inw >> q) & 1u) {
            float t = acc[f][q] + bv[f];
            if (HAS_RES) t += __builtin_bit_cast(float, __builtin_amdgcn_raw_buffer_load_b32(
                res_rs, vo_res[f], (int)((rowpix + (unsigned)((q & 3) + 8 * (q >> 2))) * ldrb), 0));
            t = (t < 0.f ? (is_relu ? 0.f : t * neg_slope) : t) * keep[f];
            __builtin_amdgcn_raw_buffer_store_b32(__builtin_bit_cast(unsigned, t), out_rs, vo_out[f],
                                                  (int)((rowpix + (unsigned)((q & 3) + 8 * (q >> 2))) * ldob), AUX);
          }
        }
    };
    f32x16 acc[2];
    for (int y = y0; y < y1; y += RING) {
#pragma unroll
      for (int r = 0; r < RING; ++r) {
        if (y + r < y1) {
          load_row(v[(r + 2 + PF) % RING], y + r + 1 + PF);
          mma_row(acc, r);
          if (full) store_row_full(acc, y + r);
          else store_row_edge(acc, y + r);
        }
      }
    }
  }
}

template <int CO4>
__global__ __launch_bounds__(256) void tiny4_kernel(const T4Args a) {
  const long long p = (long long)blockIdx.x * 256 + threadIdx.x;
  const long long npix = (long long)a.N * a.H * a.W;
  if (p >= npix) return;
  const int x = (int)(p % a.W); const long long r0 = p / a.W;
  const int y = (int)(r0 % a.H);
  const auto in_rs = __builtin_amdgcn_make_buffer_rsrc(const_cast<float*>(a.in), 0, (int)((unsigned)npix * (unsigned)a.ld * 4u), 0x00020000);
  const unsigned ldb = (unsigned)a.ld * 4u;
  float acc[CO4 * 4];
#pragma unroll
  for (int co = 0; co < CO4 * 4; ++co) acc[co] = (a.bias && co < a.Cout) ? a.bias[co] : 0.f;
  f32x4 v[9];
#pragma unroll
  for (int q = 0; q < 9; ++q) {
    const int iy = y + q / 3 - 1, ix = x + q % 3 - 1;
    const bool ok = a.tapidx[q] >= 0 && (unsigned)iy < (unsigned)a.H && (unsigned)ix < (unsigned)a.W;
    v[q] = ldbuf4(in_rs, ok ? (unsigned)(p + (long long)(q / 3 - 1) * a.W + (q % 3 - 1)) * ldb : OOB);
  }
#pragma unroll
  for (int q = 0; q < 9; ++q) {
    const int t = a.tapidx[q];
    const float* wt = a.w + (t < 0 ? 0 : t) * 4;
    const float on = t < 0 ? 0.f : 1.f;
#pragma unroll
    for (int co = 0; co < CO4 * 4; ++co) {
      const float* wr = wt + (size_t)(co < a.Cout ? co : 0) * a.Kp;
      const float m = co < a.Cout ? on : 0.f;
      acc[co] = fmaf(v[q][3], wr[3] * m, fmaf(v[q][2], wr[2] * m, fmaf(v[q][1], wr[1] * m, fmaf(v[q][0], wr[0] * m, acc[co]))));
    }
  }
#pragma unroll
  for (int g = 0; g < CO4; ++g) {
    if (4 * g < ((a.Cout + 3) & ~3)) {
      f32x4 o;
#pragma unroll
      for (int e = 0; e < 4; ++e) {
        const int co = 4 * g + e;
        float t = acc[co];
        if (a.res && co < a.Cout) t += a.res[p * a.ldr + co];
        o[e] = co < a.Cout ? act_apply(t, a.act, a.slope) : 0.f;
      }
      *(f32x4*)(a.out + p * a.ldo + 4 * g) = o;
    }
  }
}

__device__ __forceinline__ void t4_fold_store(const T4Args& a, const f32x4* acc, int lane, int g, int n, int x, int y0, int my_s, int my_c,
                                              float bias0g, float bias1g) {
    float h4[4][4];
    {
      const bool hi = (lane >> 5) & 1;
#pragma unroll
      for (int s = 0; s < 4; ++s)
#pragma unroll
        for (int i = 0; i < 4; ++i) {
          const float keep = hi ? acc[s + 4][i] : acc[s][i];
          const float send = hi ? acc[s][i] : acc[s + 4][i];
          h4[s][i] = keep + __shfl_xor(send, 32);
        }
    }
    float h2[2][4];
    {
      const bool hi = (lane >> 4) & 1;
#pragma unroll
      for (int s = 0; s < 2; ++s)
#pragma unroll
        for (int i = 0; i < 4; ++i) {
          const float keep = hi ? h4[s + 2][i] : h4[s][i];
          const float send = hi ? h4[s][i] : h4[s + 2][i];
          h2[s][i] = keep + __shfl_xor(send, 16);
        }
    }
    float h1[4];
    {
      const bool hi = (lane >> 3) & 1;
#pragma unroll
      for (int i = 0; i < 4; ++i) {
        const float keep = hi ? h2[1][i] : h2[0][i];
        const float send = hi ? h2[0][i] : h2[1][i];
        h1[i] = keep + __shfl_xor(send, 8);
      }
    }
    float o0, o1;
    {
      const bool hi = (lane >> 2) & 1;
      const float k0 = hi ? h1[2] : h1[0], k1 = hi ? h1[3] : h1[1];
      const float s0 = hi ? h1[0] : h1[2], s1 = hi ? h1[1] : h1[3];
      o0 = k0 + __shfl_xor(s0, 4);
      o1 = k1 + __shfl_xor(s1, 4);
    }
    const int y = y0 + my_s;
    if (x < a.W && y < a.H) {
      const size_t pix = (size_t)(n * a.H + y) * a.W + x;
      const int ch = 4 * g + my_c;
      float t0 = o0 + bias0g, t1 = o1 + bias1g;
      if (a.res) {
        if (ch < a.Cout) t0 += a.res[pix * a.ldr + ch];
        if (ch + 1 < a.Cout) t1 += a.res[pix * a.ldr + ch + 1];
      }
      float2 o;
      o.x = ch < a.Cout ? act_apply(t0, a.act, a.slope) : 0.f;
      o.y = ch + 1 < a.Cout ? act_apply(t1, a.act, a.slope) : 0.f;
      if (ch < ((a.Cout + 3) & ~3)) *(float2*)(a.out + pix * a.ldo + ch) = o;
    }
}

template <int KS, int NG>
__global__ __launch_bounds__(256) void thin4_cout_kernel(const T4Args a) {
  constexpr int R = KS / 2, NT = KS * KS, S = RH_COUT, RING = KS + 1;
  const int lane = threadIdx.x & 63, j = lane & 3, b = lane >> 2;
  const int wg = blockIdx.x * 4 + (threadIdx.x >> 6);
  if (wg >= a.waves_per_group) return;
  const unsigned npix = (unsigned)(a.N * a.H * a.W);
  const auto in_rs = __builtin_amdgcn_make_buffer_rsrc(const_cast<float*>(a.in), 0, (int)(npix * (unsigned)a.ld * 4u), 0x00020000);
  const unsigned ldb = (unsigned)a.ld * 4u;
  const int nchunks = a.C >> 6;
  const int my_s = b >> 1, my_c = 2 * (b & 1);
  float bias0[NG], bias1[NG];
#pragma unroll
  for (int g = 0; g < NG; ++g) {
    bias0[g] = (a.bias && 4 * g + my_c < a.Cout) ? a.bias[4 * g + my_c] : 0.f;
    bias1[g] = (a.bias && 4 * g + my_c + 1 < a.Cout) ? a.bias[4 * g + my_c + 1] : 0.f;
  }

  for (int u = wg; u < a.total_units; u += a.waves_per_group) {
    const int xs = u % a.strips; const int r0 = u / a.strips;
    const int yb = r0 % a.ybands, n = r0 / a.ybands;
    const int x = xs * 4 + j;
    const int y0 = yb * S;
    unsigned coloff[KS];
#pragma unroll
    for (int e = 0; e < KS; ++e) {
      const int ix = x + e - R;
      coloff[e] = (unsigned)ix < (unsigned)a.W ? (unsigned)ix * ldb + 16u * b : OOB;
    }
    const unsigned imgoff = (unsigned)(n * a.H) * (unsigned)a.W * ldb;
    f32x4 accg[NG][S];
#pragma unroll
    for (int g = 0; g < NG; ++g)
#pragma unroll
      for (int s = 0; s < S; ++s) accg[g][s] = f32x4{0.f, 0.f, 0.f, 0.f};
    for (int ch = 0; ch < nchunks; ++ch) {
      const int c0 = ch * 64 + 4 * b;
      f32x4 wv[NG][NT];
#pragma unroll
      for (int p = 0; p < NT; ++p) {
        const int t = a.tapidx[KS == 3 ? p : 4];
        const int k = a.kmode == 0 ? (c0 >> 4) * a.ntaps * 16 + t * 16 + (c0 & 15) : t * a.C + c0;
#pragma unroll
        for (int g = 0; g < NG; ++g) {
          const int co = 4 * g + j;
          wv[g][p] = (co < a.Cout && t >= 0) ? *(const f32x4*)(a.w + (size_t)co * a.Kp + k) : f32x4{0.f, 0.f, 0.f, 0.f};
        }
      }
      auto load_row = [&](f32x4* dst, int iy) {
        const bool rok = (unsigned)iy < (unsigned)a.H;
        const unsigned ro = imgoff + (unsigned)iy * (unsigned)a.W * ldb + (unsigned)ch * 256u;
#pragma unroll
        for (int e = 0; e < KS; ++e) dst[e] = ldbuf4(in_rs, (rok && coloff[e] != OOB) ? ro + coloff[e] : OOB);
      };
      f32x4 v[RING][KS];
#pragma unroll
      for (int q = 0; q < KS; ++q) load_row(v[q], y0 - R + q);
#pragma unroll
      for (int s = 0; s < S; ++s) {
        load_row(v[(s + KS) % RING], y0 + s - R + KS);
#pragma unroll
        for (int q = 0; q < KS; ++q)
#pragma unroll
          for (int e = 0; e < KS; ++e)
#pragma unroll
            for (int c = 0; c < 4; ++c)
#pragma unroll
              for (int g = 0; g < NG; ++g) {
                accg[g][s] = __builtin_amdgcn_mfma_f32_4x4x1f32(wv[g][q * KS + e][c], v[(s + q) % RING][e][c], accg[g][s], 0, 0, 0);
              }
      }
    }
#pragma unroll
    for (int g = 0; g < NG; ++g) t4_fold_store(a, accg[g], lane, g, n, x, y0, my_s, my_c, bias0[g], bias1[g]);
  }
}

template <int MT, int KC>
__global__ __launch_bounds__(256) void thin4_cout_kernel_rows(const T4Args a) {
  constexpr int RING = MT >= 5 ? 3 : 4, NL = KC * 4;
  __shared__ float P[RING][MT * 16][64];
  const int lane = threadIdx.x & 63, p = lane & 15, g = lane >> 4;
  const int wv_id = __builtin_amdgcn_readfirstlane(threadIdx.x >> 6);
  const unsigned npix = (unsigned)(a.N * a.H * a.W);
  const auto in_rs = __builtin_amdgcn_make_buffer_rsrc(const_cast<float*>(a.in), 0, (int)(npix * (unsigned)a.ld * 4u), 0x00020000);
  const unsigned ldb = (unsigned)a.ld * 4u;
  const int u = blockIdx.x;
  const int xs = u % a.strips; const int r0 = u / a.strips;
  const int yb = r0 % a.ybands, n = r0 / a.ybands;
  const int col = 16 * wv_id + p;
  const int x = xs * 62 - 1 + col;
  const int y0 = yb * a.rh;
  const int y1 = y0 + a.rh < a.H ? y0 + a.rh : a.H;

  f32x4 wA[MT][NL];
#pragma unroll
  for (int t = 0; t < MT; ++t) {
    const int row = 16 * t + p;
    const int q = row / a.Cout, co = row - q * a.Cout;
    const int tap = q < 9 ? a.tapidx[q] : -1;
#pragma unroll
    for (int l = 0; l < NL; ++l) {
      const int c0 = 16 * l + 4 * g;
      const int k = a.kmode == 0 ? (c0 >> 4) * a.ntaps * 16 + tap * 16 + (c0 & 15) : tap * a.C + c0;
      wA[t][l] = tap >= 0 ? *(const f32x4*)(a.w + (size_t)co * a.Kp + k) : f32x4{0.f, 0.f, 0.f, 0.f};
    }
  }
  const unsigned coloff = (unsigned)x < (unsigned)a.W ? (unsigned)x * ldb + 16u * (unsigned)g : OOB;
  const unsigned imgoff = (unsigned)(n * a.H) * (unsigned)a.W * ldb;
  auto load_row = [&](f32x4* dst, int iy) {
    const bool rok = (unsigned)iy < (unsigned)a.H && coloff != OOB;
    const unsigned ro = imgoff + (unsigned)iy * (unsigned)a.W * ldb + coloff;
#pragma unroll
    for (int l = 0; l < NL; ++l) dst[l] = ldbuf4(in_rs, rok ? ro + 64u * (unsigned)l : OOB);
  };
  const int cpad = (a.Cout + 3) & ~3;
  const bool st_col = col >= 1 && col <= 62 && x < a.W;
  unsigned tapmask = 0;
#pragma unroll
  for (int q = 0; q < 9; ++q) tapmask |= (a.tapidx[q] >= 0 ? 1u : 0u) << q;
  float bv[2];
#pragma unroll
  for (int h = 0; h < 2; ++h) bv[h] = (a.bias && 4 * h + g < a.Cout) ? a.bias[4 * h + g] : 0.f;

  f32x4 xv[2][NL];
  load_row(xv[0], y0 - 1);
  const int nrows = y1 - y0 + 2;
  auto body = [&](int it, f32x4* cur, f32x4* nxt) {
    if (it + 1 < nrows) load_row(nxt, y0 + it);
    f32x4 acc[MT];
#pragma unroll
    for (int t = 0; t < MT; ++t) acc[t] = f32x4{0.f, 0.f, 0.f, 0.f};
#pragma unroll
    for (int l = 0; l < NL; ++l)
#pragma unroll
      for (int e = 0; e < 4; ++e)
#pragma unroll
        for (int t = 0; t < MT; ++t) acc[t] = __builtin_amdgcn_mfma_f32_16x16x4f32(wA[t][l][e], cur[l][e], acc[t], 0, 0, 0);
    float (*Ps)[64] = P[it % RING];
#pragma unroll
    for (int t = 0; t < MT; ++t)
#pragma unroll
      for (int r = 0; r < 4; ++r) Ps[16 * t + 4 * g + r][(col + 16 * ((r + g) & 3)) & 63] = acc[t][r];
    __syncthreads();
    if (it >= 2) {
      const int y = y0 + it - 2;
      const size_t pix = (size_t)(n * a.H + y) * a.W + x;
#pragma unroll
      for (int h = 0; h < 2; ++h) {
        const int co = 4 * h + g;
        if (4 * h >= cpad) break;
        const int cor = co < a.Cout ? co : a.Cout - 1;
        float pv[9];
#pragma unroll
        for (int q = 0; q < 9; ++q) {
          const int row = q * a.Cout + cor;
          pv[q] = P[(it - 2 + q / 3) % RING][row][(col + (q % 3 - 1) + 16 * ((row + (row >> 2)) & 3)) & 63];
        }
        float s = 0.f;
#pragma unroll
        for (int q = 0; q < 9; ++q) s += ((tapmask >> q) & 1u) ? pv[q] : 0.f;
        if (co >= a.Cout) s = 0.f;
        if (st_col) {
          if (co < a.Cout) {
            s += bv[h];
            if (a.res) s += a.res[pix * a.ldr + co];
            s = act_apply(s, a.act, a.slope);
          }
          a.out[pix * a.ldo + co] = s;
        }
      }
    }
    if (RING == 3) __syncthreads();
  };
  for (int it = 0; it < nrows; it += 2) {
    body(it, xv[0], xv[1]);
    if (it + 1 < nrows) body(it + 1, xv[1], xv[0]);
  }
}


bool window_taps(const ssg_conv_desc* d, int* tapidx) {
  for (int p = 0; p < 9; ++p) tapidx[p] = -1;
  bool only_center = true;
  for (int t = 0; t < d->ntaps; ++t) {
    const int dy = d->dy[t], dx = d->dx[t];
    if (dy < -1 || dy > 1 || dx < -1 || dx > 1) return false;
    if (tapidx[(dy + 1) * 3 + dx + 1] >= 0) return false;
    tapidx[(dy + 1) * 3 + dx + 1] = t;
    if (dy || dx) only_center = false;
  }
  (void)only_center;
  return true;
}

}

int ssg_thin4_conv_kind(const ssg_conv_desc* d) {
  if (d->C2 != 0 || d->in_sy != 1 || d->in_sx != 1 || d->out_sy != 1 || d->out_sx != 1 || d->out_oy || d->out_ox) return 0;
  if (d->GH != d->H || d->GW != d->W || d->OH != d->H || d->OW != d->W) return 0;
  if ((long long)d->N * d->H * d->W * d->ld1 >= (1ll << 30)) return 0;
  if (((uintptr_t)d->in1 & 15) || d->ld1 % 4 || ((uintptr_t)d->w & 15) || d->Kp % 4) return 0;
  int tapidx[9];
  if (!window_taps(d, tapidx)) return 0;
  if (d->C1 == 4 && d->kmode == 1 && d->ldo % 4 == 0 && !((uintptr_t)d->out & 15) &&
      (!d->res || (d->ldr % 4 == 0 && !((uintptr_t)d->res & 15) && (long long)d->N * d->H * d->W * d->ldr < (1ll << 30)))) return 3;
  if (d->Cout <= 8 && d->C1 >= 64 && d->C1 % 64 == 0 && d->ldo % 2 == 0 && !((uintptr_t)d->out & 7)) return 4;
  return 0;
}

static bool routes_tiny(const ssg_conv_desc* d, int kind) {
  return kind == 3 && d->Cout <= 8 && (long long)d->N * d->H * d->W * d->ld1 < (1ll << 30);
}

static bool routes_thin32(const ssg_conv_desc* d, int kind) {
  if (kind != 3 || d->Cout < 32 || (long long)d->N * d->H * d->W * d->ldo >= (1ll << 30)) return false;
  if (d->W < 32 || (long long)d->N * d->H * d->W < 65536) return false;
  for (int t = 0; t < d->ntaps; ++t) if (d->dy[t] || d->dx[t]) return true;
  return false;
}

static int rows_form_mt(const ssg_conv_desc* d, int kind, bool ks1) {
  if (kind != 4 || ks1) return 0;
  const int kc = d->C1 / 64;
  if (kc != 1 && kc != 2 && kc != 4) return 0;
  const int need = (9 * d->Cout + 15) / 16;
  const int mt = need <= 2 ? 2 : need <= 3 ? 3 : 5;
  if (mt * kc * 16 > 128 || (kc == 4 && mt != 2)) return 0;
  if ((long long)d->N * d->H * d->W * d->ldo >= (1ll << 30) || (d->res && (long long)d->N * d->H * d->W * d->ldr >= (1ll << 30))) return 0;
  return mt;
}

int ssg_thin4_conv_id(const ssg_conv_desc* d, int kind) {
  if (routes_tiny(d, kind)) return 14;
  if (routes_thin32(d, kind)) return 15;
  return 9 + kind;
}

int ssg_thin4_conv_launch(const ssg_conv_desc* d, int kind, hipStream_t st) {
  T4Args a;
  a.in = d->in1; a.w = d->w; a.bias = d->bias; a.res = d->res; a.out = d->out;
  a.C = d->C1; a.ld = d->ld1; a.N = d->N; a.H = d->H; a.W = d->W; a.Kp = d->Kp; a.kmode = d->kmode;
  a.ldr = d->ldr; a.Cout = d->Cout; a.ldo = d->ldo; a.ntaps = d->ntaps;
  a.act = d->act; a.slope = d->slope;
  a.gsave = nullptr; a.ldg = 0;
  window_taps(d, a.tapidx);
  a.nt_store = (long long)d->N * d->H * d->W * d->ldo * 4 >= (256ll << 20);
  bool ks1 = true;
  for (int p = 0; p < 9; ++p) if (p != 4 && a.tapidx[p] >= 0) ks1 = false;
  const int rh = kind == 3 ? RH_CIN : RH_COUT;
  a.strips = (d->W + 3) / 4;
  a.ybands = (d->H + rh - 1) / rh;
  a.total_units = d->N * a.ybands * a.strips;
  a.groups = kind == 3 ? (d->Cout + 63) / 64 : 1;
  int wpg = 8192 / a.groups;
  if (wpg > a.total_units) wpg = a.total_units;
  a.waves_per_group = wpg;
  const dim3 grid((unsigned)((wpg * a.groups + 3) / 4)), block(256);
  if (routes_tiny(d, kind)) {
    const dim3 gridt((unsigned)(((long long)d->N * d->H * d->W + 255) / 256));
    if (d->Cout <= 4) hipLaunchKernelGGL(tiny4_kernel<1>, gridt, block, 0, st, a);
    else hipLaunchKernelGGL(tiny4_kernel<2>, gridt, block, 0, st, a);
    SSG_LAUNCH_CHECK();
    return SSG_OK;
  }
  if (routes_thin32(d, kind)) {
    a.strips = (d->W + 31) / 32;
    a.ybands = (d->H + RH_K36 - 1) / RH_K36;
    a.total_units = d->N * a.ybands * a.strips;
    int wpg2 = 8192 / a.groups;
    if (wpg2 > a.total_units) wpg2 = a.total_units;
    a.waves_per_group = wpg2;
    const dim3 grid2((unsigned)((wpg2 * a.groups + 3) / 4));
    const bool nt = a.nt_store;
    if (d->res) {
      if (nt) hipLaunchKernelGGL((thin32_cin_kernel<1, 1, true>), grid2, block, 0, st, a);
      else hipLaunchKernelGGL((thin32_cin_kernel<1, 1, false>), grid2, block, 0, st, a);
    } else {
      if (nt) hipLaunchKernelGGL((thin32_cin_kernel<0, 1, true>), grid2, block, 0, st, a);
      else hipLaunchKernelGGL((thin32_cin_kernel<0, 1, false>), grid2, block, 0, st, a);
    }
    SSG_LAUNCH_CHECK();
    return SSG_OK;
  }
  if (const int mt = rows_form_mt(d, kind, ks1)) {
    a.strips = (d->W + 61) / 62;
    a.rh = 32;
    while (a.rh > 8 && (long long)d->N * ((d->H + a.rh - 1) / a.rh) * a.strips < 1024) a.rh >>= 1;
    a.ybands = (d->H + a.rh - 1) / a.rh;
    a.total_units = d->N * a.ybands * a.strips;
    const dim3 gridr((unsigned)a.total_units);
    const int kc = d->C1 / 64;
    if (mt == 2 && kc == 1) hipLaunchKernelGGL((thin4_cout_kernel_rows<2, 1>), gridr, block, 0, st, a);
    else if (mt == 2 && kc == 2) hipLaunchKernelGGL((thin4_cout_kernel_rows<2, 2>), gridr, block, 0, st, a);
    else if (mt == 2) hipLaunchKernelGGL((thin4_cout_kernel_rows<2, 4>), gridr, block, 0, st, a);
    else if (mt == 3 && kc == 1) hipLaunchKernelGGL((thin4_cout_kernel_rows<3, 1>), gridr, block, 0, st, a);
    else if (mt == 3) hipLaunchKernelGGL((thin4_cout_kernel_rows<3, 2>), gridr, block, 0, st, a);
    else hipLaunchKernelGGL((thin4_cout_kernel_rows<5, 1>), gridr, block, 0, st, a);
    SSG_LAUNCH_CHECK();
    return SSG_OK;
  }
  if (kind == 3) {
    if (d->res) {
      if (ks1) hipLaunchKernelGGL((thin4_cin_kernel<1, 1, true>), grid, block, 0, st, a);
      else hipLaunchKernelGGL((thin4_cin_kernel<3, 1, true>), grid, block, 0, st, a);
    } else if (ks1) hipLaunchKernelGGL((thin4_cin_kernel<1, 2, false>), grid, block, 0, st, a);
    else hipLaunchKernelGGL((thin4_cin_kernel<3, 2, false>), grid, block, 0, st, a);
  } else {
    if (d->Cout <= 4) {
      if (ks1) hipLaunchKernelGGL((thin4_cout_kernel<1, 1>), grid, block, 0, st, a);
      else hipLaunchKernelGGL((thin4_cout_kernel<3, 1>), grid, block, 0, st, a);
    } else {
      if (ks1) hipLaunchKernelGGL((thin4_cout_kernel<1, 2>), grid, block, 0, st, a);
      else hipLaunchKernelGGL((thin4_cout_kernel<3, 2>), grid, block, 0, st, a);
    }
  }
  SSG_LAUNCH_CHECK();
  return SSG_OK;
}

static int spade_fused_cin(const ssg_conv_desc* d) {
  if (!d || d->res || d->act != SSG_ACT_NONE || d->bnpart || (d->Cout & 7) || d->ntaps != 9 || d->kmode != 1) return 0;
  if (d->C2 != 0 || d->in_sy != 1 || d->in_sx != 1 || d->out_sy != 1 || d->out_sx != 1 || d->out_oy || d->out_ox) return 0;
  if (d->GH != d->H || d->GW != d->W || d->OH != d->H || d->OW != d->W) return 0;
  if (((uintptr_t)d->in1 & 15) || d->ld1 % 4 || ((uintptr_t)d->w & 15) || d->Kp % 4 || d->ldo % 4 || ((uintptr_t)d->out & 15)) return 0;
  int tapidx[9];
  if (!window_taps(d, tapidx)) return 0;
  if (d->W < 32 || (long long)d->N * d->H * d->W < 65536) return 0;
  if ((long long)d->N * d->H * d->W * (d->Cout / 2) >= (1ll << 30) || (long long)d->N * d->H * d->W * d->ld1 >= (1ll << 30)) return 0;
  if (d->C1 == 4) return 4;
  if (d->C1 == 8) return 8;
  return 0;
}

static bool spade_fused_ok(const ssg_conv_desc* d) { return spade_fused_cin(d) != 0; }

extern "C" int ssg_spade_conv_modulate_ok(const ssg_conv_desc* d) { return spade_fused_ok(d) ? 1 : 0; }

extern "C" int ssg_spade_conv_modulate_f32(const ssg_conv_desc* d, const float* x, int ldx, float* gamma, int ldg, void* stream) {
  SSG_REQUIRE(d && x && gamma && d->in1 && d->w && d->out, SSG_EINVAL, "spade_conv_modulate: null pointer");
  SSG_REQUIRE(spade_fused_ok(d), SSG_EINVAL, "spade_conv_modulate: shape not handled by the fused kernel (ssg_spade_conv_modulate_ok == 0)");
  const int C = d->Cout / 2;
  SSG_REQUIRE(ldx >= C && ldg >= C && d->ldo >= C, SSG_EINVAL, "spade_conv_modulate: pixel strides < C");
  T4Args a;
  a.in = d->in1; a.w = d->w; a.bias = d->bias; a.res = x; a.out = d->out;
  a.C = d->C1; a.ld = d->ld1; a.N = d->N; a.H = d->H; a.W = d->W; a.Kp = d->Kp; a.kmode = d->kmode;
  a.ldr = ldx; a.Cout = d->Cout; a.ldo = d->ldo; a.ntaps = d->ntaps;
  a.act = SSG_ACT_NONE; a.slope = 0.f;
  a.gsave = gamma; a.ldg = ldg;
  window_taps(d, a.tapidx);
  a.nt_store = (long long)d->N * d->H * d->W * C * 4 >= (256ll << 20);
  a.groups = (C + 31) / 32;
  a.strips = (d->W + 31) / 32;
  a.ybands = (d->H + RH_K36 - 1) / RH_K36;
  a.total_units = d->N * a.ybands * a.strips;
  int wpg = 8192 / a.groups;
  if (wpg > a.total_units) wpg = a.total_units;
  a.waves_per_group = wpg;
  const dim3 grid((unsigned)((wpg * a.groups + 3) / 4)), block(256);
  if (spade_fused_cin(d) == 8) {
    if (a.nt_store) hipLaunchKernelGGL((thin32_cin_kernel<2, 1, true, 8>), grid, block, 0, (hipStream_t)stream, a);
    else hipLaunchKernelGGL((thin32_cin_kernel<2, 1, false, 8>), grid, block, 0, (hipStream_t)stream, a);
  } else if (a.nt_store) hipLaunchKernelGGL((thin32_cin_kernel<2, 1, true>), grid, block, 0, (hipStream_t)stream, a);
  else hipLaunchKernelGGL((thin32_cin_kernel<2, 1, false>), grid, block, 0, (hipStream_t)stream, a);
  SSG_LAUNCH_CHECK();
  return SSG_OK;
}
```

### ssunet-gan_amd/csrc/conv_wgrad4.hip

```cpp
#include "common.h"
#include "conv_thin.h"

namespace {

struct W4Args {
  const float* wide; const float* thin; float* ws;
  int Cw, ldw, ldt, N, H, W, Cout, Cin;
  int groups, nz;
  long long units_per_z;
  int segs_per_row;
};

constexpr int SEG = 32;
constexpr int U = 8;

template <bool THIN_COUT, int KS>
__global__ __launch_bounds__(256) void wgrad4_kernel(const W4Args a) {
  constexpr int R = KS / 2, NT = KS * KS, COLS = U + KS - 1;
  const int lane = threadIdx.x & 63;
  const int wave = threadIdx.x >> 6;
  const int zb = blockIdx.x / a.groups, cg = blockIdx.x - zb * a.groups;
  const int z = zb * 4 + wave;
  const int j = lane & 3;
  const int cw = cg * 64 + lane;
  const bool cw_ok = cw < a.Cw;
  const float* tapT = THIN_COUT ? a.wide : a.thin;
  const float* fixT = THIN_COUT ? a.thin : a.wide;
  const unsigned ldtap = THIN_COUT ? a.ldw : a.ldt, ldfix = THIN_COUT ? a.ldt : a.ldw;
  const unsigned npix = (unsigned)(a.N * a.H * a.W);
  const auto tap_rs = __builtin_amdgcn_make_buffer_rsrc(const_cast<float*>(tapT), 0, (int)(npix * ldtap * 4u), 0x00020000);
  const auto fix_rs = __builtin_amdgcn_make_buffer_rsrc(const_cast<float*>(fixT), 0, (int)(npix * ldfix * 4u), 0x00020000);
  const unsigned chtap = THIN_COUT ? cw : j, chfix = THIN_COUT ? j : cw;
  const bool tap_lane_ok = THIN_COUT ? cw_ok : true, fix_lane_ok = THIN_COUT ? true : cw_ok;
  constexpr unsigned OOB = 0xffffffffu;

  f32x4 acc[NT];
#pragma unroll
  for (int t = 0; t < NT; ++t) acc[t] = f32x4{0.f, 0.f, 0.f, 0.f};

  const int u0 = z * (int)a.units_per_z;
  const int total_units = a.N * a.H * a.segs_per_row;
  int u1 = u0 + (int)a.units_per_z; if (u1 > total_units) u1 = total_units;
  for (int u = u0; u < u1; ++u) {
    const int r = u / a.segs_per_row; const int seg = u - r * a.segs_per_row;
    const int y = r % a.H, n = r / a.H;
    const int x0 = seg * SEG;
    const int x1 = x0 + SEG < a.W ? x0 + SEG : a.W;
    unsigned rowoff[KS]; bool rowok[KS];
#pragma unroll
    for (int q = 0; q < KS; ++q) {
      const int iy = y + q - R;
      rowok[q] = tap_lane_ok && (unsigned)iy < (unsigned)a.H;
      rowoff[q] = ((unsigned)((n * a.H + iy) * a.W) * ldtap + chtap) * 4u;
    }
    const unsigned fixoff = ((unsigned)((n * a.H + y) * a.W) * ldfix + chfix) * 4u;
    for (int xb = x0; xb < x1; xb += U) {
      float f[U], v[KS][COLS];
#pragma unroll
      for (int k = 0; k < U; ++k) {
        const bool ok = fix_lane_ok && (xb + k < x1);
        f[k] = __builtin_bit_cast(float, __builtin_amdgcn_raw_buffer_load_b32(
            fix_rs, ok ? fixoff + (unsigned)(xb + k) * ldfix * 4u : OOB, 0, 0));
      }
#pragma unroll
      for (int c = 0; c < COLS; ++c) {
        const int ix = xb + c - R;
        const bool cok = (unsigned)ix < (unsigned)a.W;
        const unsigned xo = (unsigned)ix * ldtap * 4u;
#pragma unroll
        for (int q = 0; q < KS; ++q)
          v[q][c] = __builtin_bit_cast(float, __builtin_amdgcn_raw_buffer_load_b32(
              tap_rs, (cok && rowok[q]) ? rowoff[q] + xo : OOB, 0, 0));
      }
#pragma unroll
      for (int k = 0; k < U; ++k)
#pragma unroll
        for (int q = 0; q < KS; ++q)
#pragma unroll
          for (int e = 0; e < KS; ++e) {
            if (THIN_COUT) acc[q * KS + e] = __builtin_amdgcn_mfma_f32_4x4x1f32(v[q][k + e], f[k], acc[q * KS + e], 0, 0, 0);
            else acc[q * KS + e] = __builtin_amdgcn_mfma_f32_4x4x1f32(f[k], v[q][k + e], acc[q * KS + e], 0, 0, 0);
          }
    }
  }
  __shared__ float red[4][NT * 4][64];
#pragma unroll
  for (int t = 0; t < NT; ++t)
#pragma unroll
    for (int i = 0; i < 4; ++i) red[wave][t * 4 + i][lane] = acc[t][i];
  __syncthreads();
  float* slab = a.ws + (size_t)zb * NT * a.Cin * a.Cout;
  const int b4 = (lane >> 2) * 4;
  for (int e = wave; e < NT * 4; e += 4) {
    const int t = e >> 2, i = e & 3;
    const float sum = ((red[0][e][lane] + red[1][e][lane]) + red[2][e][lane]) + red[3][e][lane];
    int co, c;
    if (THIN_COUT) { co = j; c = cg * 64 + b4 + i; }
    else { co = cg * 64 + b4 + i; c = j; }
    if (co < a.Cout && c < a.Cin) slab[((size_t)t * a.Cin + c) * a.Cout + co] = sum;
  }
}

__global__ __launch_bounds__(256) void wgrad32_cin_kernel(const W4Args a) {
  const int lane = threadIdx.x & 63, l31 = lane & 31, h = lane >> 5;
  const int wave = threadIdx.x >> 6;
  const int zb = blockIdx.x / a.groups, cg = blockIdx.x - zb * a.groups;
  const int z = zb * 4 + wave;
  const unsigned npix = (unsigned)(a.N * a.H * a.W);
  const auto do_rs = __builtin_amdgcn_make_buffer_rsrc(const_cast<float*>(a.wide), 0, (int)(npix * (unsigned)a.ldw * 4u), 0x00020000);
  const auto in_rs = __builtin_amdgcn_make_buffer_rsrc(const_cast<float*>(a.thin), 0, (int)(npix * (unsigned)a.ldt * 4u), 0x00020000);
  constexpr unsigned OOB = 0xffffffffu;
  const unsigned ldwb = (unsigned)a.ldw * 4u, ldtb = (unsigned)a.ldt * 4u;
  unsigned aoff[2];
#pragma unroll
  for (int f = 0; f < 2; ++f) { const int co = cg * 64 + f * 32 + l31; aoff[f] = co < a.Cout ? (unsigned)co * 4u : OOB; }
  const int t0 = l31 >> 2, c = l31 & 3;
  const int dy0 = t0 / 3 - 1, dx0 = t0 % 3 - 1;
  const bool has1 = l31 < 4;

  f32x16 acc[2][2];
#pragma unroll
  for (int f = 0; f < 2; ++f)
#pragma unroll
    for (int g = 0; g < 2; ++g)
#pragma unroll
      for (int q = 0; q < 16; ++q) acc[f][g][q] = 0.f;

  const int u0 = z * (int)a.units_per_z;
  const int total_units = a.N * a.H * a.segs_per_row;
  int u1 = u0 + (int)a.units_per_z; if (u1 > total_units) u1 = total_units;
  constexpr int UP = 8;
  for (int u = u0; u < u1; ++u) {
    const int r = u / a.segs_per_row; const int seg = u - r * a.segs_per_row;
    const int y = r % a.H, n = r / a.H;
    const int x0 = seg * SEG;
    const int x1 = x0 + SEG < a.W ? x0 + SEG : a.W;
    const unsigned rowpix = (unsigned)((n * a.H + y) * a.W);
    const bool r0ok = (unsigned)(y + dy0) < (unsigned)a.H, r1ok = has1 && y + 1 < a.H;
    const unsigned b0row = (rowpix + (unsigned)(dy0 * a.W)) * ldtb + (unsigned)c * 4u;
    const unsigned b1row = (rowpix + (unsigned)a.W) * ldtb + (unsigned)c * 4u;
    for (int xb = x0; xb < x1; xb += 2 * UP) {
      float av[2][UP], bv[2][UP];
#pragma unroll
      for (int k = 0; k < UP; ++k) {
        const int x = xb + 2 * k + h;
        const bool pok = x < x1;
        const unsigned po = (rowpix + (unsigned)x) * ldwb;
#pragma unroll
        for (int f = 0; f < 2; ++f)
          av[f][k] = __builtin_bit_cast(float, __builtin_amdgcn_raw_buffer_load_b32(do_rs, (pok && aoff[f] != OOB) ? po + aoff[f] : OOB, 0, 0));
        const int ix0 = x + dx0, ix1 = x + 1;
        bv[0][k] = __builtin_bit_cast(float, __builtin_amdgcn_raw_buffer_load_b32(
            in_rs, (pok && r0ok && (unsigned)ix0 < (unsigned)a.W) ? b0row + (unsigned)ix0 * ldtb : OOB, 0, 0));
        bv[1][k] = __builtin_bit_cast(float, __builtin_amdgcn_raw_buffer_load_b32(
            in_rs, (pok && r1ok && ix1 < a.W) ? b1row + (unsigned)ix1 * ldtb : OOB, 0, 0));
      }
#pragma unroll
      for (int k = 0; k < UP; ++k)
#pragma unroll
        for (int f = 0; f < 2; ++f)
#pragma unroll
          for (int g = 0; g < 2; ++g)
            acc[f][g] = __builtin_amdgcn_mfma_f32_32x32x2f32(av[f][k], bv[g][k], acc[f][g], 0, 0, 0);
    }
  }
  __shared__ float red[4][36][64];
#pragma unroll
  for (int f = 0; f < 2; ++f)
#pragma unroll
    for (int g = 0; g < 2; ++g) {
      const int nn = g * 32 + l31;
      if (nn < 36) {
#pragma unroll
        for (int q = 0; q < 16; ++q) red[wave][nn][f * 32 + (q & 3) + 8 * (q >> 2) + 4 * h] = acc[f][g][q];
      }
    }
  __syncthreads();
  float* slab = a.ws + (size_t)zb * 9 * a.Cin * a.Cout;
  for (int e = threadIdx.x; e < 36 * 64; e += 256) {
    const int nn = e >> 6, m = e & 63;
    const float sum = ((red[0][nn][m] + red[1][nn][m]) + red[2][nn][m]) + red[3][nn][m];
    const int co = cg * 64 + m;
    if (co < a.Cout) slab[(size_t)nn * a.Cout + co] = sum;
  }
}

constexpr int TINY_PIX = 4096;

__global__ __launch_bounds__(256) void wgrad_tiny4_kernel(const W4Args a) {
  const int co = threadIdx.x & 7, slot = threadIdx.x >> 3;
  const long long npix = (long long)a.N * a.H * a.W;
  const long long p0 = (long long)blockIdx.x * TINY_PIX;
  const long long p1 = p0 + TINY_PIX < npix ? p0 + TINY_PIX : npix;
  const auto in_rs = __builtin_amdgcn_make_buffer_rsrc(const_cast<float*>(a.thin), 0, (int)((unsigned)npix * (unsigned)a.ldt * 4u), 0x00020000);
  const auto do_rs = __builtin_amdgcn_make_buffer_rsrc(const_cast<float*>(a.wide), 0, (int)((unsigned)npix * (unsigned)a.ldw * 4u), 0x00020000);
  constexpr unsigned OOB = 0xffffffffu;
  const bool co_ok = co < a.Cout;
  f32x4 acc[9];
#pragma unroll
  for (int t = 0; t < 9; ++t) acc[t] = f32x4{0.f, 0.f, 0.f, 0.f};
  for (long long p = p0 + slot; p < p1; p += 32) {
    const int x = (int)(p % a.W); const int y = (int)((p / a.W) % a.H);
    const float g = __builtin_bit_cast(float, __builtin_amdgcn_raw_buffer_load_b32(do_rs, co_ok ? ((unsigned)p * (unsigned)a.ldw + (unsigned)co) * 4u : OOB, 0, 0));
#pragma unroll
    for (int t = 0; t < 9; ++t) {
      const int iy = y + t / 3 - 1, ix = x + t % 3 - 1;
      const bool ok = (unsigned)iy < (unsigned)a.H && (unsigned)ix < (unsigned)a.W;
      const f32x4 v = __builtin_bit_cast(f32x4, __builtin_amdgcn_raw_buffer_load_b128(
          in_rs, ok ? (unsigned)(p + (long long)(t / 3 - 1) * a.W + (t % 3 - 1)) * (unsigned)a.ldt * 4u : OOB, 0, 0));
      acc[t] += v * g;
    }
  }
  __shared__ float red[32][36][8];
#pragma unroll
  for (int t = 0; t < 9; ++t)
#pragma unroll
    for (int c = 0; c < 4; ++c) red[slot][t * 4 + c][co] = acc[t][c];
  __syncthreads();
  float* slab = a.ws + (size_t)blockIdx.x * 9 * a.Cin * a.Cout;
  for (int e = threadIdx.x; e < 36 * 8; e += 256) {
    const int c8 = e & 7, row = e >> 3;
    float sum = 0.f;
#pragma unroll 8
    for (int k = 0; k < 32; ++k) sum += red[k][row][c8];
    const int t = row >> 2, c = row & 3;
    if (c8 < a.Cout && c < a.Cin) slab[((size_t)t * a.Cin + c) * a.Cout + c8] = sum;
  }
}

}

int ssg_wgrad4_kind(const ssg_wgrad_desc* d) {
  if (d->C2 != 0 || d->in_sy != 1 || d->in_sx != 1 || d->GH != d->H || d->GW != d->W) return 0;
  if (d->ntaps == 9) {
    for (int t = 0; t < 9; ++t) if (d->dy[t] != t / 3 - 1 || d->dx[t] != t % 3 - 1) return 0;
  } else if (d->ntaps != 1 || d->dy[0] != 0 || d->dx[0] != 0) {
    return 0;
  }
  if ((long long)d->N * d->H * d->W * (d->ld1 > d->ldd ? d->ld1 : d->ldd) >= (1ll << 30)) return 0;
  if (d->Cout <= 4 && d->C1 >= 16 && d->C1 % 4 == 0) return 5;
  if (d->C1 == 4 && d->Cout <= 8 && d->ntaps == 9) return 7;
  if (d->C1 == 4 && d->ntaps == 9 && d->Cout >= 32 && (long long)d->N * d->H * d->W >= 65536) return 8;
  if (d->C1 == 4) return 6;
  return 0;
}

int ssg_wgrad4_slices(const ssg_wgrad_desc* d, int kind, int* groups, long long* units_per_z, int* segs_per_row) {
  if (kind == 7) {
    if (groups) *groups = 1;
    if (units_per_z) *units_per_z = TINY_PIX;
    if (segs_per_row) *segs_per_row = 1;
    return (int)(((long long)d->N * d->H * d->W + TINY_PIX - 1) / TINY_PIX);
  }
  const int cw = kind == 5 ? d->C1 : d->Cout;
  const int g = (cw + 63) / 64;
  const int spr = (d->W + SEG - 1) / SEG;
  const long long units = (long long)d->N * d->H * spr;
  long long nz = 8192 / g;
  if (nz > units) nz = units;
  if (nz < 1) nz = 1;
  const long long upz = (units + nz - 1) / nz;
  nz = (units + upz - 1) / upz;
  nz = (nz + 3) / 4;
  if (groups) *groups = g;
  if (units_per_z) *units_per_z = upz;
  if (segs_per_row) *segs_per_row = spr;
  return (int)nz;
}

int ssg_wgrad4_launch(const ssg_wgrad_desc* d, int kind, hipStream_t st) {
  W4Args a;
  a.ws = d->ws; a.N = d->N; a.H = d->H; a.W = d->W; a.Cout = d->Cout; a.Cin = d->C1;
  a.nz = ssg_wgrad4_slices(d, kind, &a.groups, &a.units_per_z, &a.segs_per_row);
  const dim3 grid((unsigned)(a.nz * a.groups)), block(256);
  if (kind == 7) {
    a.wide = d->dout; a.Cw = d->Cout; a.ldw = d->ldd; a.thin = d->in1; a.ldt = d->ld1;
    hipLaunchKernelGGL(wgrad_tiny4_kernel, grid, block, 0, st, a);
    SSG_LAUNCH_CHECK();
    return SSG_OK;
  }
  if (kind == 8) {
    a.wide = d->dout; a.Cw = d->Cout; a.ldw = d->ldd; a.thin = d->in1; a.ldt = d->ld1;
    hipLaunchKernelGGL(wgrad32_cin_kernel, grid, block, 0, st, a);
    SSG_LAUNCH_CHECK();
    return SSG_OK;
  }
  if (kind == 5) { a.wide = d->in1; a.Cw = d->C1; a.ldw = d->ld1; a.thin = d->dout; a.ldt = d->ldd; }
  else { a.wide = d->dout; a.Cw = d->Cout; a.ldw = d->ldd; a.thin = d->in1; a.ldt = d->ld1; }
  if (kind == 5 && d->ntaps == 9) hipLaunchKernelGGL((wgrad4_kernel<true, 3>), grid, block, 0, st, a);
  else if (kind == 5) hipLaunchKernelGGL((wgrad4_kernel<true, 1>), grid, block, 0, st, a);
  else if (d->ntaps == 9) hipLaunchKernelGGL((wgrad4_kernel<false, 3>), grid, block, 0, st, a);
  else hipLaunchKernelGGL((wgrad4_kernel<false, 1>), grid, block, 0, st, a);
  SSG_LAUNCH_CHECK();
  return SSG_OK;
}
```

### ssunet-gan_amd/ops.py

```python
import ctypes as C
import math

import torch
import torch.distributed as dist

from . import _lib
from ._lib import ACT_LRELU, ACT_NONE, ACT_RELU, ACT_SWISH, ConvDesc, WgradDesc, call, ptr, stream_ptr

__all__ = ['conv2d', 'batch_norm_act', 'max_pool2x2', 'max_pool2x2_skip', 'max_unpool2x2', 'upsample2x_bilinear', 'upsample2x_nearest',
           'spade_modulate', 'adaptive_avgpool_flat', 'linear', 'seg_loss', 'bce_with_logits_const', 'nan_to_zero_',
           'to_nhwc', 'new_nhwc', 'bump_weight_epoch', 'dwconv2d', 'swish', 'sigmoid', 'gaussian', 'mul', 'global_avgpool',
           'channel_scale', 'spectral_norm_weight', 'conv2d_sn']


def pad4(c):
    return (c + 3) // 4 * 4


def new_nhwc(n, c, h, w, device, ld=None, zero=False):
    ld = pad4(c) if ld is None else ld
    buf = (torch.zeros if zero else torch.empty)(n * h * w * ld, device=device, dtype=torch.float32)
    return torch.empty(0, device=device, dtype=torch.float32).set_(
        buf.untyped_storage(), 0, (n, c, h, w), (h * w * ld, 1, w * ld, ld))

# ... 332 lines not shown
    if hit is None:
        nbytes = call('ssg_pack_weights_split_bytes', rows, kp, bn)
        hit = torch.empty(nbytes // 2, dtype=torch.int16, device=wpk.device)
        call('ssg_pack_weights_split_bf16x3', wpk.data_ptr() + row0 * kp * 4, rows, kp, bn, ptr(hit), stream_ptr())
        cache[key] = hit
    return hit


def _out_size(h, k, s, p):
    return (h + 2 * p - k) // s + 1


def _out_hw(h, w, kh, kw, s, pad):
    pt, pb, pl, pr = _pad4(pad)
    return (h + pt + pb - kh) // s + 1, (w + pl + pr - kw) // s + 1


def _x1_routed(precision, stride, pad, wscale, fused):
    if precision == 'fp32':
        return False
    if precision != 'bf16x1':
        raise ValueError('conv: unknown precision %r (one of %s)' % (precision, ', '.join(_PRECISIONS)))
    if fused is not None:
        raise ValueError("conv: in_affine / bwd_stats cannot be combined with precision='bf16x1'")
    return stride == 1 and _pad4(pad) == (1, 1, 1, 1) and wscale is None


def _x1_s2_routed(precision, x1_s2, stride, pad, wscale):
    return bool(x1_s2) and precision == 'bf16x1' and stride == 2 and _pad4(pad) == (1, 1, 1, 1) and wscale is None


def _conv_fwd_impl(x1, x2, weight, bias, stride, pad, act, slope, res=None, out=None, wscale=None, want_bn=False, in_affine=None, precision='fp32',
                   x1_s2=False):
    if _x1_routed(precision, stride, pad, wscale, in_affine) and conv2d_bf16x1_ok(x1, weight, x2=x2, res=res):
        y = _conv_bf16x1_impl(x1, weight, bias, act, slope, x2=x2, res=res, out=out)
        return (y, None) if want_bn else y
    if _x1_s2_routed(precision, x1_s2, stride, pad, wscale) and x2 is None and res is None and in_affine is None:
        y = _conv_s2_bf16x1_impl(x1, weight, bias, act, slope, out=out)
        if y is not None:
            return (y, None) if want_bn else y
    o, i, kh, kw = weight.shape
    n, c1, h, w = x1.shape
    c2 = x2.shape[1] if x2 is not None else 0
    if x2 is not None and c1 % 4:
        raise ValueError('two-input conv needs C1 %% 4 == 0 (got %d)' % c1)
    if c1 + c2 != i:
        raise ValueError('conv: input channels %d+%d != weight in-channels %d' % (c1, c2, i))
    cred_pad = pad4(c1) + pad4(c2)
    taps = _taps_fwd(kh, kw, pad)
    wpk, kp, kmode = _pack(weight, 0, taps, cred_pad, pad4(c1), sigma=wscale)
    oh, ow = _out_hw(h, w, kh, kw, stride, pad)
    if out is None:
        out = new_nhwc(n, o, oh, ow, x1.device)
    try:
        part = _conv_launch(x1, x2, wpk, kp, kmode, 0, o, bias, res, act, slope, taps, n, h, w, oh, ow, oh, ow, stride, 1, 0, 0, out,
                            want_bn=want_bn and res is None and act == ACT_NONE,
                            tag=_ROLE[0] if (kh == 3 and kw == 3 and _ROLE[0] is not None) else None, in_affine=in_affine)
    except _Declined:
        return None
    return (out, part) if want_bn else out


def _conv_dgrad_impl(dy, weight, stride, pad, h, w, c_lo, c_hi, res=None, wscale=None, bwd_stats=None, precision='fp32', x1_s2=False):
    if _x1_routed(precision, stride, pad, wscale, bwd_stats):
        dx = _conv_dgrad_bf16x1_impl(dy, weight, h, w, c_lo, c_hi, res=res)
        if dx is not None:
            return dx
    if _x1_s2_routed(precision, x1_s2, stride, pad, wscale) and res is None and bwd_stats is None:
        dx = _conv_dgrad_s2_bf16x1_impl(dy, weight, h, w, c_lo, c_hi)
        if dx is not None:
            return dx
    o, i, kh, kw = weight.shape
    n, _, oh, ow = dy.shape
    cred_pad = pad4(o)
    pt, _, pl, _ = _pad4(pad)
    dx = new_nhwc(n, c_hi - c_lo, h, w, dy.device)
    if stride == 1:
        taps = [(ky, kx, pt - ky, pl - kx) for ky in range(kh) for kx in range(kw)]
        wpk, kp, kmode = _pack(weight, 1, taps, cred_pad, cred_pad, sigma=wscale)
        try:
            part = _conv_launch(dy, None, wpk, kp, kmode, c_lo, c_hi - c_lo, None, res, ACT_NONE, 0.0, taps, n, oh, ow, h, w, h, w, 1, 1, 0, 0,
                                dx, bwd_stats=bwd_stats)
        except _Declined:
            return None
        return dx if bwd_stats is None else (dx, part)
    if bwd_stats is not None:
        return None
    if res is not None:
        raise NotImplementedError('strided dgrad with fused accumulation')
    s = stride
    classes = []
    for py in range(s):
        for px in range(s):
            taps = [(ky, kx, (py + pt - ky) // s, (px + pl - kx) // s) for ky in range(kh) for kx in range(kw)
                    if (py + pt - ky) % s == 0 and (px + pl - kx) % s == 0]
            classes.append((py, px, taps))
    if (PARITY_MERGE and s == 2 and kh == 3 and kw == 3 and (pt, pl) == (1, 1) and MFMA_SPLIT and ow >= 17
            and (c_hi - c_lo) % 64 == 0 and dy.numel() * 4 <= 0xfffffff0):
        merged = [t for _, _, taps in classes for t in taps]
        wpk, kp, kmode = _pack(weight, 1, merged, cred_pad, cred_pad, sigma=wscale)
        try:
            _conv_launch(dy, None, wpk, kp, kmode, c_lo, c_hi - c_lo, None, None, ACT_NONE, 0.0, merged, n, oh, ow,
                         (h + 1) // 2, (w + 1) // 2, h, w, 1, s, 0, 0, dx, parity_merge=True)
            return dx
        except _Declined:
            pass
    if any(len(t) == 0 for _, _, t in classes):
        _relabel(dx, _ld(dx)).zero_()
    for py, px, taps in classes:
        gh, gw = (h - py + s - 1) // s, (w - px + s - 1) // s
        if not taps or gh <= 0 or gw <= 0:
            continue
        wpk, kp, kmode = _pack(weight, 1, taps, cred_pad, cred_pad, sigma=wscale)
        _conv_launch(dy, None, wpk, kp, kmode, c_lo, c_hi - c_lo, None, None, ACT_NONE, 0.0, taps, n, oh, ow, gh, gw, h, w, 1, s, py, px, dx)
    return dx


def _check_wgrad_s2(who, precision, wgrad_s2):
    if wgrad_s2 not in _PRECISIONS:
        raise ValueError('%s: unknown wgrad_s2 %r (one of %s)' % (who, wgrad_s2, ', '.join(_PRECISIONS)))
    if wgrad_s2 == 'bf16x1' and precision != 'bf16x1':
        raise ValueError("%s: wgrad_s2='bf16x1' needs precision='bf16x1' (got %r)" % (who, precision))


def _conv_wgrad_impl(x1, x2, dy, weight_shape, stride, pad, in_affine=None, precision='fp32', wgrad_s2='fp32'):
    if _x1_routed(precision, stride, pad, None, in_affine):
        dw = _conv_wgrad_bf16x1_impl(x1, x2, dy, weight_shape)
        if dw is not None:
            return dw
    if (precision == 'bf16x1' and wgrad_s2 == 'bf16x1' and stride == 2 and _pad4(pad) == (1, 1, 1, 1) and x2 is None
            and in_affine is None):
        dw = _conv_wgrad_s2_bf16x1_impl(x1, dy, weight_shape)
        if dw is not None:
            return dw
    o, i, kh, kw = weight_shape
    n = x1.shape[0]
    _, _, oh, ow = dy.shape
    d = _wgrad_desc(x1, pad4(x1.shape[1]), x2, pad4(x2.shape[1]) if x2 is not None else 0, dy, weight_shape, stride,
                    _taps_fwd(kh, kw, pad))
    dw = torch.empty((o, i, kh, kw), device=dy.device, dtype=torch.float32)
    d.dw_oihw = dw.data_ptr()
    d.flags = 1 if MFMA_SPLIT else 0
    if in_affine is not None:
        d.in_scale = in_affine[0].data_ptr(); d.in_shift = in_affine[1].data_ptr(); d.in_act = int(in_affine[2]); d.in_slope = float(in_affine[3])
        if not call('ssg_conv2d_wgrad_in_affine_ok', C.byref(d)):
            return None
    nbytes = call('ssg_conv2d_wgrad_workspace_bytes', C.byref(d))
    ws = _ws(nbytes, dy.device)
    d.ws = ws.data_ptr(); d.ws_bytes = ws.numel() * 8
    _timed_call(_WGRAD_KIND, 'ssg_conv2d_wgrad_f32', d, (), (n, oh, ow, i, o, kh, stride), 2.0 * n * oh * ow * o * i * kh * kw)
    return dw


def _channel_sum(x, c):
    n, _, h, w = x.shape
    p = n * h * w
    out = torch.empty(c, device=x.device, dtype=torch.float32)
    ws = _ws(call('ssg_bn_workspace_bytes', p, c), x.device)
    call('ssg_channel_sum_f32', ptr(x), p, c, _ld(x), ptr(out), ptr(ws), stream_ptr())
    return out


def _act_bwd(y, dy, act, slope):
    n, c, h, w = y.shape
    dx = new_nhwc(n, c, h, w, y.device)
    call('ssg_act_bwd_f32', ptr(y), _ld(y), ptr(dy), _ld(dy), n * h * w, pad4(c), act, slope, ptr(dx), _ld(dx), stream_ptr())
    return dx


class _Conv2d(torch.autograd.Function):

    @staticmethod
    def forward(ctx, x1, x2, weight, bias, stride, pad, act, slope, res=None, want_bn=False, precision='fp32', wgrad_s2='fp32'):
        ctx.set_materialize_grads(False)
        x1 = to_nhwc(x1)
        x2 = to_nhwc(x2) if x2 is not None else None
        res = to_nhwc(res) if res is not None else None
        r = _conv_fwd_impl(x1, x2, weight, bias, stride, pad, act, slope, res=res, want_bn=want_bn, precision=precision, x1_s2=True)
        y, part = r if want_bn else (r, None)
        ctx.cfg = (stride, pad, act, slope, precision, wgrad_s2)
        ctx.save_for_backward(x1, x2, weight, y if act != ACT_NONE else None)
        ctx.has_bias = bias is not None
        ctx.has_res = res is not None
        if part is None:
            part = torch.empty(0, dtype=torch.float64, device=y.device)
        ctx.mark_non_differentiable(part)
        return y, part

    @staticmethod
    @torch.autograd.function.once_differentiable
    def backward(ctx, dy, _=None):
        if dy is None:
            return (None,) * 12
        x1, x2, weight, y = ctx.saved_tensors
        stride, pad, act, slope, precision, wgrad_s2 = ctx.cfg
        dy = to_nhwc(dy)
        if act != ACT_NONE:
            dy = _act_bwd(y, dy, act, slope)
        n, c1, h, w = x1.shape
        dx1 = dx2 = dw = db = None
        if ctx.needs_input_grad[0]:
            dx1 = _conv_dgrad_impl(dy, weight, stride, pad, h, w, 0, c1, precision=precision, x1_s2=True)
        if x2 is not None and ctx.needs_input_grad[1]:
            dx2 = _conv_dgrad_impl(dy, weight, stride, pad, h, w, c1, c1 + x2.shape[1], precision=precision, x1_s2=True)
        if ctx.needs_input_grad[2]:
            dw = _conv_wgrad_impl(x1, x2, dy, weight.shape, stride, pad, precision=precision, wgrad_s2=wgrad_s2)
        if ctx.has_bias and ctx.needs_input_grad[3]:
            db = _channel_sum(dy, weight.shape[0])
        dres = dy if (ctx.has_res and ctx.needs_input_grad[8]) else None
        return dx1, dx2, dw, db, None, None, None, None, dres, None, None, None


def conv2d(x, weight, bias=None, stride=1, padding=0, act=ACT_NONE, slope=0.0, x2=None, res=None, bn_stats=False, precision='fp32',
           wgrad_s2='fp32'):
    _lib.require_gpu(x)
    if precision not in _PRECISIONS:
        raise ValueError('conv2d: unknown precision %r (one of %s)' % (precision, ', '.join(_PRECISIONS)))
    _check_wgrad_s2('conv2d', precision, wgrad_s2)
    pad = tuple(int(v) for v in padding) if isinstance(padding, (tuple, list)) else int(padding)
    y, part = _Conv2d.apply(x, x2, weight, bias, int(stride), pad, int(act), float(slope), res, bool(bn_stats), precision, wgrad_s2)
    return (y, part) if bn_stats else y


_X1_LABELS = {70: 'conv_halo_k32_x1_kernel<128>', 71: 'conv_halo_k32_x1_kernel<64>'}
_X1_KIND = (_X1_LABELS, 'ssg_conv2d_bf16x1_kernel_id', _CONV_SHAPE)
_X1_TAPS = _taps_fwd(3, 3, 1)
_PRECISIONS = ('fp32', 'bf16x1')


class _precision(object):

    def __init__(self, mode):
        if mode not in _PRECISIONS:
            raise ValueError('%s: unknown mode %r (one of %s)' % (type(self).__name__, mode, ', '.join(_PRECISIONS)))
        self.mode = mode

    def __enter__(self):
        self.prev = self._state[0]; self._state[0] = self.mode
        return self

    def __exit__(self, *a):
        self._state[0] = self.prev


class infer_precision(_precision):
    _state = ['fp32']


def infer_precision_mode():
    return infer_precision._state[0]


def _x1_desc(x, x2, weight, res, out=None):
    def side(t):
        ld = nhwc_ld(t)
        return (t.data_ptr(), ld) if ld is not None else (16, pad4(t.shape[1]))
    n, c1, h, w = x.shape
    c2 = x2.shape[1] if x2 is not None else 0
    o = weight.shape[0]
    return _conv_desc(side(x), c1, side(x2) if x2 is not None else None, c2, (n, h, w), 16, 9 * (c1 + c2), 0, None,
                      side(res) if res is not None else None, side(out) if out is not None else (16, pad4(o)), o,
                      (h, w, h, w), 1, 1, (0, 0), _X1_TAPS, ACT_NONE, 0.0)


def _x1_shapes_ok(x, weight, x2, res):
    if x.dim() != 4 or weight.dim() != 4 or tuple(weight.shape[2:]) != (3, 3) or x.dtype != torch.float32 or weight.dtype != torch.float32:
        return False
    c2 = x2.shape[1] if x2 is not None else 0
    if x.shape[1] + c2 != weight.shape[1] or (x2 is not None and (x2.dtype != torch.float32 or x2.shape[0] != x.shape[0] or x2.shape[2:] != x.shape[2:])):
        return False
    return res is None or (res.dtype == torch.float32 and tuple(res.shape) == (x.shape[0], weight.shape[0], x.shape[2], x.shape[3]))


def conv2d_bf16x1_ok(x, weight, x2=None, res=None):
    if not _x1_shapes_ok(x, weight, x2, res):
        return False
    return call('ssg_conv2d_bf16x1_ok', C.byref(_x1_desc(x, x2, weight, res))) != 0


def _x1_pack(weight, wpk, kp, fmt, transpose=0, row0=0, rows=None):
    cache = _stamped_cache(weight, '_ssg_pack_bf16x1')
    if rows is None:
        rows = weight.shape[0]
    key = (transpose, row0, rows, fmt) if transpose else fmt
    hit = cache.get(key)
    if hit is None:
        nbytes = call('ssg_pack_weights_bf16x1_bytes', rows, kp, fmt)
        hit = torch.empty(nbytes // 2, dtype=torch.int16, device=weight.device)
        call('ssg_pack_weights_bf16x1', wpk.data_ptr() + row0 * kp * 4, rows, kp, fmt, ptr(hit), stream_ptr())
        cache[key] = hit
    return hit


def _conv_bf16x1_impl(x, weight, bias, act, slope, x2=None, res=None, out=None):
    x = to_nhwc(x.detach())
    x2 = to_nhwc(x2.detach()) if x2 is not None else None
    res = to_nhwc(res.detach()) if res is not None else None
    n, c1, h, w = x.shape
    o = weight.shape[0]
    wpk, kp, kmode = _pack(weight, 0, _X1_TAPS, weight.shape[1], c1)
    if out is None:
        out = new_nhwc(n, o, h, w, x.device)
    d = _x1_desc(x, x2, weight, res, out)
    d.w = wpk.data_ptr(); d.Kp = kp; d.kmode = kmode
    d.bias = bias.data_ptr() if bias is not None else None
    d.act = int(act); d.slope = float(slope)
# ... 1339 lines not shown
```

Baseline: 85.30 images/sec.

## Virtualize SPADE backward dgb tensor by fusing dy*x into wgrad/dgrad loads

The SPADE modulate backward no longer materializes the 2C-channel dgb gradient tensor or the dxm residual. A dedicated reduction kernel computes only the bias sums. The gamma/beta wgrad and dgrad kernels now recompute dgb on the fly from dy and x in their load paths. The final dx dgrad kernel fuses the dy*(1+gamma) residual into its epilogue. This removes large full-resolution writes and reads of dgb and dxm, at the cost of extra loads and multiplies inside the conv kernels and new templated kernel variants.

```diff
diff --git a/include/ssunet_hip.h b/include/ssunet_hip.h
--- a/include/ssunet_hip.h
+++ b/include/ssunet_hip.h
@@ -215,6 +215,14 @@
                                float* dx, int lddx, float* dgb, int lddgb, void* stream);
 int ssg_spade_modulate_bwd_sums_f32(const float* x, int ldx, const float* gb, int ldgb, const float* dy, int lddy, int64_t P,
                                     int C, float* dx, int lddx, float* dgb, int lddgb, double* sums, void* ws, void* stream);
+int ssg_spade_bwd_sums_ok(const float* x, int ldx, const float* dy, int lddy, int64_t P, int C);
+int ssg_spade_bwd_sums_f32(const float* x, int ldx, const float* dy, int lddy, int64_t P, int C, double* sums, void* ws, void* stream);
+int ssg_spade_dgrad_virtual_ok(const ssg_conv_desc* d, int lddy, const float* x, int ldx);
+int ssg_spade_dgrad_virtual_f32(const ssg_conv_desc* d, int lddy, const float* x, int ldx, void* stream);
+int ssg_spade_wgrad_virtual_ok(const ssg_wgrad_desc* d, int lddy, const float* x, int ldx);
+int ssg_spade_wgrad_virtual_f32(const ssg_wgrad_desc* d, int lddy, const float* x, int ldx, void* stream);
+int ssg_spade_dgrad_dx_ok(const ssg_conv_desc* d, const float* gamma, int ldg);
+int ssg_spade_dgrad_dx_f32(const ssg_conv_desc* d, const float* gamma, int ldg, void* stream);
 int ssg_act_bwd_f32(const float* y, int ldy, const float* dy, int lddy, int64_t P, int C, int act, float slope, float* dx, int lddx, void* stream);
 int ssg_copy_channels_f32(const float* src, int ldsrc, int64_t P, int C, float* dst, int lddst, void* stream);
 int ssg_add_f32(const float* a, const float* b, int64_t n, float* out, void* stream);
diff --git a/ssunet-gan_amd/_lib.py b/ssunet-gan_amd/_lib.py
--- a/ssunet-gan_amd/_lib.py
+++ b/ssunet-gan_amd/_lib.py
@@ -135,6 +135,14 @@
     'ssg_spade_modulate_fwd_f32': [_P, _I, _P, _I, _L, _I, _P, _I, _P],
     'ssg_spade_modulate_bwd_f32': [_P, _I, _P, _I, _P, _I, _L, _I, _P, _I, _P, _I, _P],
     'ssg_spade_modulate_bwd_sums_f32': [_P, _I, _P, _I, _P, _I, _L, _I, _P, _I, _P, _I, _P, _P, _P],
+    'ssg_spade_bwd_sums_ok': [_P, _I, _P, _I, _L, _I],
+    'ssg_spade_bwd_sums_f32': [_P, _I, _P, _I, _L, _I, _P, _P, _P],
+    'ssg_spade_dgrad_virtual_ok': [C.POINTER(ConvDesc), _I, _P, _I],
+    'ssg_spade_dgrad_virtual_f32': [C.POINTER(ConvDesc), _I, _P, _I, _P],
+    'ssg_spade_wgrad_virtual_ok': [C.POINTER(WgradDesc), _I, _P, _I],
+    'ssg_spade_wgrad_virtual_f32': [C.POINTER(WgradDesc), _I, _P, _I, _P],
+    'ssg_spade_dgrad_dx_ok': [C.POINTER(ConvDesc), _P, _I],
+    'ssg_spade_dgrad_dx_f32': [C.POINTER(ConvDesc), _P, _I, _P],
     'ssg_act_bwd_f32': [_P, _I, _P, _I, _L, _I, _I, _F, _P, _I, _P],
     'ssg_add_f32': [_P, _P, _L, _P, _P],
     'ssg_copy_channels_f32': [_P, _I, _L, _I, _P, _I, _P],
@@ -216,7 +224,8 @@
     'ssg_bn_stats_from_partials_workspace_bytes': C.c_int64,
 }
 _NO_STATUS = set(_RESTYPES) | {'ssg_abi_version', 'ssg_conv2d_split_bn', 'ssg_conv2d_in_affine_ok', 'ssg_conv2d_wgrad_in_affine_ok', 'ssg_conv2d_bwd_stats_ok', 'ssg_conv2d_kernel_id', 'ssg_conv2d_bnpart_rows', 'ssg_conv2d_bf16x1_ok', 'ssg_conv2d_bf16x1_kernel_id', 'ssg_conv2d_bf16x1_s2_ok', 'ssg_conv2d_bf16x1_s2_kernel_id', 'ssg_conv2d_bf16x1_cls_ok', 'ssg_conv2d_bf16x1_cls_kernel_id', 'ssg_conv2d_wgrad_bf16x1_ok', 'ssg_conv2d_wgrad_bf16x1_kernel_id', 'ssg_conv2d_wgrad_bf16x1_s2_ok', 'ssg_conv2d_wgrad_bf16x1_s2_kernel_id', 'ssg_conv2d_wgrad_kernel_id', 'ssg_dwconv2d_kernel_id',
-                                'ssg_spade_conv_modulate_ok', 'ssg_se_gate_ok'}
+                                'ssg_spade_conv_modulate_ok', 'ssg_se_gate_ok', 'ssg_spade_bwd_sums_ok', 'ssg_spade_dgrad_virtual_ok',
+                                'ssg_spade_wgrad_virtual_ok', 'ssg_spade_dgrad_dx_ok'}
 
 ABI_VERSION = 10
 
diff --git a/ssunet-gan_amd/blocks.py b/ssunet-gan_amd/blocks.py
--- a/ssunet-gan_amd/blocks.py
+++ b/ssunet-gan_amd/blocks.py
@@ -235,24 +235,39 @@
         pad = ctx.pad
         dout = to_nhwc(dout)
         n, c, h, w = x.shape
-        dxm = new_nhwc(n, c, h, w, x.device)
-        dgb = new_nhwc(n, 2 * c, h, w, x.device)
+        need_dx = ctx.needs_input_grad[0]
+        nh = a.shape[1]
         scratch = ops._ws(call('ssg_bn_workspace_bytes', n * h * w, c), x.device)
         sums = torch.empty(2 * c, dtype=torch.float64, device=x.device)
-        with ops._hbm('spade_modulate_bwd', 4.0 * n * h * w * c * (3 + 3)):
-            call('ssg_spade_modulate_bwd_sums_f32', ptr(x), _ld(x), ptr(gb), _ld(gb), ptr(dout), _ld(dout), n * h * w, c,
-                 ptr(dxm), _ld(dxm), ptr(dgb), _ld(dgb), ptr(sums), ptr(scratch), stream_ptr())
-        dwgb = _conv_wgrad_impl(a, None, dgb, wgb.shape, 1, pad)
-        dbias_gb = sums.float()
-        nh = a.shape[1]
-        da = _conv_dgrad_impl(dgb, wgb, 1, pad, h, w, 0, nh)
+        virt = ops._spade_bwd_virtual_ok(x, dout, a, gb, wgb, wx, seg.shape[1], pad, need_dx)
+        if virt:
+            with ops._hbm('spade_modulate_bwd', 4.0 * n * h * w * c * 2):
+                call('ssg_spade_bwd_sums_f32', ptr(x), _ld(x), ptr(dout), _ld(dout), n * h * w, c, ptr(sums), ptr(scratch), stream_ptr())
+            dwgb = ops._spade_wgrad_virtual(a, dout, x, wgb.shape, pad)
+            dbias_gb = sums.float()
+            da = ops._spade_dgrad_virtual(dout, x, wgb, pad, out=new_nhwc(n, nh, h, w, x.device))
+        else:
+            dxm = new_nhwc(n, c, h, w, x.device)
+            dgb = new_nhwc(n, 2 * c, h, w, x.device)
+            ops.SPADE_DGB_ALLOCS[0] += 1
+            with ops._hbm('spade_modulate_bwd', 4.0 * n * h * w * c * (3 + 3)):
+                call('ssg_spade_modulate_bwd_sums_f32', ptr(x), _ld(x), ptr(gb), _ld(gb), ptr(dout), _ld(dout), n * h * w, c,
+                     ptr(dxm), _ld(dxm), ptr(dgb), _ld(dgb), ptr(sums), ptr(scratch), stream_ptr())
+            dwgb = _conv_wgrad_impl(a, None, dgb, wgb.shape, 1, pad)
+            dbias_gb = sums.float()
+            da = _conv_dgrad_impl(dgb, wgb, 1, pad, h, w, 0, nh)
         da = _act_bwd(a, da, ACT_RELU, 0.0)
         dws = _conv_wgrad_impl(seg, None, da, ws.shape, 1, pad)
         dbs = _channel_sum(da, nh)
         dseg = _conv_dgrad_impl(da, ws, 1, pad, h, w, 0, seg.shape[1])
         dwx = _conv_wgrad_impl(x, None, dseg, wx.shape, 1, pad)
         dbx = _channel_sum(dseg, seg.shape[1])
-        dx = _conv_dgrad_impl(dseg, wx, 1, pad, h, w, 0, c, res=dxm) if ctx.needs_input_grad[0] else None
+        if not need_dx:
+            dx = None
+        elif virt:
+            dx = ops._spade_dgrad_dx(dseg, seg.shape[1], wx, pad, c, dout, gb, out=new_nhwc(n, c, h, w, x.device))
+        else:
+            dx = _conv_dgrad_impl(dseg, wx, 1, pad, h, w, 0, c, res=dxm)
         return dx, dwx, dbx, dws, dbs, dwgb[:c], dbias_gb[:c], dwgb[c:], dbias_gb[c:], None
 
 
diff --git a/ssunet-gan_amd/csrc/bn.hip b/ssunet-gan_amd/csrc/bn.hip
--- a/ssunet-gan_amd/csrc/bn.hip
+++ b/ssunet-gan_amd/csrc/bn.hip
@@ -179,6 +179,41 @@
   }
 }
 
+__global__ __launch_bounds__(RED_BLOCK) void spade_bwd_sums_kernel(
+    const float* __restrict__ x, int ldx, const float* __restrict__ dy, int lddy, long long P, int C,
+    int TQ, int PR, long long rows_per_part, double* __restrict__ part ) {
+  __shared__ double red[2][RED_BLOCK][4];
+  const int tid = threadIdx.x;
+  const int tq = tid % TQ, pr = tid / TQ;
+  const int cq = blockIdx.y * TQ + tq;
+  const int CQ = C / 4;
+  const bool cok = cq < CQ;
+  const long long p0 = (long long)blockIdx.x * rows_per_part;
+  long long p1 = p0 + rows_per_part; if (p1 > P) p1 = P;
+  double s1[4] = {0, 0, 0, 0}, s2[4] = {0, 0, 0, 0};
+  if (cok) {
+    for (long long p = p0 + pr; p < p1; p += PR) {
+      const f32x4 xv = *(const f32x4*)(x + p * ldx + 4 * cq);
+      const f32x4 d = *(const f32x4*)(dy + p * lddy + 4 * cq);
+      const f32x4 dg = d * xv;
+#pragma unroll
+      for (int e = 0; e < 4; ++e) { s1[e] += (double)dg[e]; s2[e] += (double)d[e]; }
+    }
+  }
+#pragma unroll
+  for (int e = 0; e < 4; ++e) { red[0][tid][e] = s1[e]; red[1][tid][e] = s2[e]; }
+  __syncthreads();
+  if (pr == 0 && cok) {
+    double a1[4] = {0, 0, 0, 0}, a2[4] = {0, 0, 0, 0};
+    for (int r = 0; r < PR; ++r)
+#pragma unroll
+      for (int e = 0; e < 4; ++e) { a1[e] += red[0][r * TQ + tq][e]; a2[e] += red[1][r * TQ + tq][e]; }
+    double* dst = part + (size_t)blockIdx.x * 2 * C;
+#pragma unroll
+    for (int e = 0; e < 4; ++e) { dst[4 * cq + e] = a1[e]; dst[C + 4 * cq + e] = a2[e]; }
+  }
+}
+
 constexpr int FIN_LANES = 32;
 
 struct BnFin {
@@ -569,6 +604,28 @@
   hipStream_t st = (hipStream_t)stream;
   hipLaunchKernelGGL(modulate_bwd_sums_kernel, dim3((unsigned)g.parts, (unsigned)g.groups), dim3(RED_BLOCK), 0, st, x, ldx, gb, ldgb, dy, lddy,
                      (long long)P, C, dx, lddx, dgb, lddgb, g.TQ, g.PR, g.rows_per_part, part);
+  SSG_LAUNCH_CHECK();
+  hipLaunchKernelGGL(col_reduce_final_kernel, dim3((unsigned)((C + 31) / 32)), dim3(32 * FIN_LANES), 0, st, part, g.parts, C, C, sums, nullptr, 0.0, BnFin{}, 0.0);
+  SSG_LAUNCH_CHECK();
+  return SSG_OK;
+}
+
+extern "C" int ssg_spade_bwd_sums_ok(const float* x, int ldx, const float* dy, int lddy, int64_t P, int C) {
+  if (!x || !dy || P <= 0 || C <= 0 || C % 4) return 0;
+  if (ldx % 4 || lddy % 4 || ldx < C || lddy < C || !ssg_aligned16(x) || !ssg_aligned16(dy)) return 0;
+  return 1;
+}
+
+extern "C" int ssg_spade_bwd_sums_f32(const float* x, int ldx, const float* dy, int lddy, int64_t P, int C, double* sums, void* ws,
+                                      void* stream) {
+  SSG_REQUIRE(sums && ws, SSG_EINVAL, "spade_bwd_sums: null pointer");
+  SSG_REQUIRE(ssg_spade_bwd_sums_ok(x, ldx, dy, lddy, P, C), SSG_EINVAL,
+              "spade_bwd_sums: bad args (ssg_spade_bwd_sums_ok == 0: C % 4, strides % 4 and >= C, 16-byte aligned rows)");
+  const RedGeom g = red_geom(P, C);
+  double* part = (double*)ws;
+  hipStream_t st = (hipStream_t)stream;
+  hipLaunchKernelGGL(spade_bwd_sums_kernel, dim3((unsigned)g.parts, (unsigned)g.groups), dim3(RED_BLOCK), 0, st, x, ldx, dy, lddy,
+                     (long long)P, C, g.TQ, g.PR, g.rows_per_part, part);
   SSG_LAUNCH_CHECK();
   hipLaunchKernelGGL(col_reduce_final_kernel, dim3((unsigned)((C + 31) / 32)), dim3(32 * FIN_LANES), 0, st, part, g.parts, C, C, sums, nullptr, 0.0, BnFin{}, 0.0);
   SSG_LAUNCH_CHECK();
diff --git a/ssunet-gan_amd/csrc/conv_thin4.hip b/ssunet-gan_amd/csrc/conv_thin4.hip
--- a/ssunet-gan_amd/csrc/conv_thin4.hip
+++ b/ssunet-gan_amd/csrc/conv_thin4.hip
@@ -12,6 +12,7 @@
   int rh;
   int nt_store;
   float* gsave; int ldg;
+  const float* vx; int ldvx;
 };
 
 constexpr int RH_CIN = 16;
@@ -130,7 +131,7 @@
 
 template <int MODE, int PF, bool NT, int CIN = 4>
 __global__ __launch_bounds__(256) void thin32_cin_kernel(const T4Args a) {
-  constexpr bool HAS_RES = MODE >= 1, SPADE = MODE == 2;
+  constexpr bool HAS_RES = MODE >= 1, SPADE = MODE == 2, DXG = MODE == 3;
   constexpr int CH = CIN / 2;
   typedef float vrow_t __attribute__((ext_vector_type(CH)));
   constexpr int AUX = NT ? 2 : 0;
@@ -144,13 +145,15 @@
   const auto out_rs = __builtin_amdgcn_make_buffer_rsrc(a.out, 0, (int)(npix * (unsigned)a.ldo * 4u), 0x00020000);
   const auto res_rs = __builtin_amdgcn_make_buffer_rsrc(const_cast<float*>(HAS_RES ? a.res : a.in), 0,
                                                         (int)(npix * (unsigned)(HAS_RES ? a.ldr : a.ld) * 4u), 0x00020000);
-  const auto g_rs = __builtin_amdgcn_make_buffer_rsrc(SPADE ? a.gsave : a.out, 0, (int)(npix * (unsigned)(SPADE ? a.ldg : a.ldo) * 4u), 0x00020000);
+  const auto g_rs = __builtin_amdgcn_make_buffer_rsrc((SPADE || DXG) ? a.gsave : a.out, 0,
+                                                      (int)(npix * (unsigned)((SPADE || DXG) ? a.ldg : a.ldo) * 4u), 0x00020000);
   const unsigned ldb = (unsigned)a.ld * 4u, ldob = (unsigned)a.ldo * 4u, ldrb = (unsigned)a.ldr * 4u, ldgb = (unsigned)a.ldg * 4u;
   const int Cmod = a.Cout >> 1;
 
   float wB[2][9 * CH], bv[2], keep[2];
   unsigned vo_out[2], vo_res[2];
   unsigned vo_g = OOB;
+  unsigned vo_gm[2] = {OOB, OOB};
 #pragma unroll
   for (int f = 0; f < 2; ++f) {
     const int cm = cg * 32 + l31;
@@ -169,6 +172,7 @@
     vo_out[f] = cok ? 4u * (unsigned)h * ldob + (unsigned)cch * 4u : OOB;
     vo_res[f] = cok ? 4u * (unsigned)h * ldrb + (unsigned)cch * 4u : OOB;
     if (SPADE) vo_g = cok ? 4u * (unsigned)h * ldgb + (unsigned)cch * 4u : OOB;
+    if (DXG) vo_gm[f] = cok ? 4u * (unsigned)h * ldgb + (unsigned)cch * 4u : OOB;
   }
   const bool is_relu = a.act == SSG_ACT_RELU;
   const float neg_slope = a.act == SSG_ACT_LRELU ? a.slope : 1.f;
@@ -239,6 +243,23 @@
         }
         return;
       }
+      if (DXG) {
+        float gm[2][16];
+#pragma unroll
+        for (int f = 0; f < 2; ++f)
+#pragma unroll
+          for (int q = 0; q < 16; ++q)
+            gm[f][q] = __builtin_bit_cast(float, __builtin_amdgcn_raw_buffer_load_b32(
+                g_rs, vo_gm[f], (int)((rowpix + (unsigned)((q & 3) + 8 * (q >> 2))) * ldgb), 0));
+#pragma unroll
+        for (int f = 0; f < 2; ++f)
+#pragma unroll
+          for (int q = 0; q < 16; ++q) {
+            float m = rv[f][q] * (1.f + gm[f][q]);
+            asm("" : "+v"(m));
+            rv[f][q] = m;
+          }
+      }
 #pragma unroll
       for (int f = 0; f < 2; ++f)
 #pragma unroll
@@ -272,7 +293,14 @@
         for (int q = 0; q < 16; ++q) {
           if ((inw >> q) & 1u) {
             float t = acc[f][q] + bv[f];
-            if (HAS_RES) t += __builtin_bit_cast(float, __builtin_amdgcn_raw_buffer_load_b32(
+            if (DXG) {
+              const unsigned pq = rowpix + (unsigned)((q & 3) + 8 * (q >> 2));
+              const float dv = __builtin_bit_cast(float, __builtin_amdgcn_raw_buffer_load_b32(res_rs, vo_res[f], (int)(pq * ldrb), 0));
+              const float gm = __builtin_bit_cast(float, __builtin_amdgcn_raw_buffer_load_b32(g_rs, vo_gm[f], (int)(pq * ldgb), 0));
+              float m = dv * (1.f + gm);
+              asm("" : "+v"(m));
+              t += m;
+            } else if (HAS_RES) t += __builtin_bit_cast(float, __builtin_amdgcn_raw_buffer_load_b32(
                 res_rs, vo_res[f], (int)((rowpix + (unsigned)((q & 3) + 8 * (q >> 2))) * ldrb), 0));
             t = (t < 0.f ? (is_relu ? 0.f : t * neg_slope) : t) * keep[f];
             __builtin_amdgcn_raw_buffer_store_b32(__builtin_bit_cast(unsigned, t), out_rs, vo_out[f],
@@ -479,9 +507,9 @@
   }
 }
 
-template <int MT, int KC>
+template <int MT, int KC, bool VIRT = false>
 __global__ __launch_bounds__(256) void thin4_cout_kernel_rows(const T4Args a) {
-  constexpr int RING = MT >= 5 ? 3 : 4, NL = KC * 4;
+  constexpr int RING = MT >= 5 ? 3 : 4, NL = KC * 4, NLH = NL / 2;
   __shared__ float P[RING][MT * 16][64];
   const int lane = threadIdx.x & 63, p = lane & 15, g = lane >> 4;
   const int wv_id = __builtin_amdgcn_readfirstlane(threadIdx.x >> 6);
@@ -511,11 +539,23 @@
   }
   const unsigned coloff = (unsigned)x < (unsigned)a.W ? (unsigned)x * ldb + 16u * (unsigned)g : OOB;
   const unsigned imgoff = (unsigned)(n * a.H) * (unsigned)a.W * ldb;
+  const auto vx_rs = __builtin_amdgcn_make_buffer_rsrc(const_cast<float*>(VIRT ? a.vx : a.in), 0,
+                                                       (int)(npix * (unsigned)(VIRT ? a.ldvx : a.ld) * 4u), 0x00020000);
+  const unsigned ldvb = (unsigned)a.ldvx * 4u;
   auto load_row = [&](f32x4* dst, int iy) {
     const bool rok = (unsigned)iy < (unsigned)a.H && coloff != OOB;
     const unsigned ro = imgoff + (unsigned)iy * (unsigned)a.W * ldb + coloff;
-#pragma unroll
-    for (int l = 0; l < NL; ++l) dst[l] = ldbuf4(in_rs, rok ? ro + 64u * (unsigned)l : OOB);
+    if constexpr (VIRT) {
+      const unsigned rx = ((unsigned)(n * a.H + iy) * (unsigned)a.W + (unsigned)x) * ldvb + 16u * (unsigned)g;
+#pragma unroll
+      for (int l = 0; l < NLH; ++l) {
+        dst[l] = ldbuf4(vx_rs, rok ? rx + 64u * (unsigned)l : OOB);
+        dst[NLH + l] = ldbuf4(in_rs, rok ? ro + 64u * (unsigned)l : OOB);
+      }
+    } else {
+#pragma unroll
+      for (int l = 0; l < NL; ++l) dst[l] = ldbuf4(in_rs, rok ? ro + 64u * (unsigned)l : OOB);
+    }
   };
   const int cpad = (a.Cout + 3) & ~3;
   const bool st_col = col >= 1 && col <= 62 && x < a.W;
@@ -531,6 +571,10 @@
   const int nrows = y1 - y0 + 2;
   auto body = [&](int it, f32x4* cur, f32x4* nxt) {
     if (it + 1 < nrows) load_row(nxt, y0 + it);
+    if constexpr (VIRT) {
+#pragma unroll
+      for (int l = 0; l < NLH; ++l) cur[l] = cur[NLH + l] * cur[l];
+    }
     f32x4 acc[MT];
 #pragma unroll
     for (int t = 0; t < MT; ++t) acc[t] = f32x4{0.f, 0.f, 0.f, 0.f};
@@ -640,13 +684,15 @@
   return 9 + kind;
 }
 
-int ssg_thin4_conv_launch(const ssg_conv_desc* d, int kind, hipStream_t st) {
+static int thin4_launch(const ssg_conv_desc* d, int kind, hipStream_t st, const float* vx, int ldvx, int lddy, const float* gamma, int ldg) {
   T4Args a;
   a.in = d->in1; a.w = d->w; a.bias = d->bias; a.res = d->res; a.out = d->out;
   a.C = d->C1; a.ld = d->ld1; a.N = d->N; a.H = d->H; a.W = d->W; a.Kp = d->Kp; a.kmode = d->kmode;
   a.ldr = d->ldr; a.Cout = d->Cout; a.ldo = d->ldo; a.ntaps = d->ntaps;
   a.act = d->act; a.slope = d->slope;
-  a.gsave = nullptr; a.ldg = 0;
+  a.gsave = const_cast<float*>(gamma); a.ldg = ldg;
+  a.vx = vx; a.ldvx = ldvx;
+  if (vx) a.ld = lddy;
   window_taps(d, a.tapidx);
   a.nt_store = (long long)d->N * d->H * d->W * d->ldo * 4 >= (256ll << 20);
   bool ks1 = true;
@@ -676,7 +722,10 @@
     a.waves_per_group = wpg2;
     const dim3 grid2((unsigned)((wpg2 * a.groups + 3) / 4));
     const bool nt = a.nt_store;
-    if (d->res) {
+    if (gamma) {
+      if (nt) hipLaunchKernelGGL((thin32_cin_kernel<3, 1, true>), grid2, block, 0, st, a);
+      else hipLaunchKernelGGL((thin32_cin_kernel<3, 1, false>), grid2, block, 0, st, a);
+    } else if (d->res) {
       if (nt) hipLaunchKernelGGL((thin32_cin_kernel<1, 1, true>), grid2, block, 0, st, a);
       else hipLaunchKernelGGL((thin32_cin_kernel<1, 1, false>), grid2, block, 0, st, a);
     } else {
@@ -694,7 +743,8 @@
     a.total_units = d->N * a.ybands * a.strips;
     const dim3 gridr((unsigned)a.total_units);
     const int kc = d->C1 / 64;
-    if (mt == 2 && kc == 1) hipLaunchKernelGGL((thin4_cout_kernel_rows<2, 1>), gridr, block, 0, st, a);
+    if (vx) hipLaunchKernelGGL((thin4_cout_kernel_rows<3, 2, true>), gridr, block, 0, st, a);
+    else if (mt == 2 && kc == 1) hipLaunchKernelGGL((thin4_cout_kernel_rows<2, 1>), gridr, block, 0, st, a);
     else if (mt == 2 && kc == 2) hipLaunchKernelGGL((thin4_cout_kernel_rows<2, 2>), gridr, block, 0, st, a);
     else if (mt == 2) hipLaunchKernelGGL((thin4_cout_kernel_rows<2, 4>), gridr, block, 0, st, a);
     else if (mt == 3 && kc == 1) hipLaunchKernelGGL((thin4_cout_kernel_rows<3, 1>), gridr, block, 0, st, a);
@@ -722,6 +772,46 @@
   return SSG_OK;
 }
 
+int ssg_thin4_conv_launch(const ssg_conv_desc* d, int kind, hipStream_t st) { return thin4_launch(d, kind, st, nullptr, 0, 0, nullptr, 0); }
+
+static bool spade_bwd_plain(const ssg_conv_desc* d) {
+  if (!d || !d->in1 || !d->w || !d->out || d->bnpart || d->ws || d->w_split || d->parity_merge || d->in_scale || d->bwd_x) return false;
+  if (d->N <= 0 || d->H <= 0 || d->W <= 0 || d->Cout <= 0 || d->C1 <= 0 || d->ntaps != 9 || d->act != SSG_ACT_NONE) return false;
+  if (d->kmode != 0 && d->kmode != 1) return false;
+  if (d->Kp < d->C1 * d->ntaps || d->ldo < d->Cout || d->ld1 < d->C1) return false;
+  return true;
+}
+
+extern "C" int ssg_spade_dgrad_virtual_ok(const ssg_conv_desc* d, int lddy, const float* x, int ldx) {
+  if (!spade_bwd_plain(d) || !x || d->res) return 0;
+  if (ssg_thin4_conv_kind(d) != 4 || d->C1 != 128 || rows_form_mt(d, 4, false) != 3) return 0;
+  const int C = d->C1 / 2;
+  if (lddy % 4 || ldx % 4 || lddy < C || ldx < C || ((uintptr_t)x & 15)) return 0;
+  const long long npix = (long long)d->N * d->H * d->W;
+  if (npix * lddy >= (1ll << 30) || npix * ldx >= (1ll << 30)) return 0;
+  return 1;
+}
+
+extern "C" int ssg_spade_dgrad_virtual_f32(const ssg_conv_desc* d, int lddy, const float* x, int ldx, void* stream) {
+  SSG_REQUIRE(ssg_spade_dgrad_virtual_ok(d, lddy, x, ldx), SSG_EINVAL,
+              "spade_dgrad_virtual: not handled (ssg_spade_dgrad_virtual_ok == 0: 3x3, 2C = 128 -> 4..5 channels, aligned rows, strides % 4, < 2^30 elements)");
+  return thin4_launch(d, 4, (hipStream_t)stream, x, ldx, lddy, nullptr, 0);
+}
+
+extern "C" int ssg_spade_dgrad_dx_ok(const ssg_conv_desc* d, const float* gamma, int ldg) {
+  if (!spade_bwd_plain(d) || !gamma || !d->res || d->Cout % 4) return 0;
+  if (ssg_thin4_conv_kind(d) != 3 || routes_tiny(d, 3) || !routes_thin32(d, 3)) return 0;
+  if (ldg % 4 || ldg < d->Cout || d->ldr < d->Cout || ((uintptr_t)gamma & 15)) return 0;
+  if ((long long)d->N * d->H * d->W * ldg >= (1ll << 30)) return 0;
+  return 1;
+}
+
+extern "C" int ssg_spade_dgrad_dx_f32(const ssg_conv_desc* d, const float* gamma, int ldg, void* stream) {
+  SSG_REQUIRE(ssg_spade_dgrad_dx_ok(d, gamma, ldg), SSG_EINVAL,
+              "spade_dgrad_dx: not handled (ssg_spade_dgrad_dx_ok == 0: 4 -> Cout >= 32, Cout % 4 == 0, 3x3, >= 65536 pixels, W >= 32, aligned rows, < 2^30 elements)");
+  return thin4_launch(d, 3, (hipStream_t)stream, nullptr, 0, 0, gamma, ldg);
+}
+
 static int spade_fused_cin(const ssg_conv_desc* d) {
   if (!d || d->res || d->act != SSG_ACT_NONE || d->bnpart || (d->Cout & 7) || d->ntaps != 9 || d->kmode != 1) return 0;
   if (d->C2 != 0 || d->in_sy != 1 || d->in_sx != 1 || d->out_sy != 1 || d->out_sx != 1 || d->out_oy || d->out_ox) return 0;
@@ -751,6 +841,7 @@
   a.ldr = ldx; a.Cout = d->Cout; a.ldo = d->ldo; a.ntaps = d->ntaps;
   a.act = SSG_ACT_NONE; a.slope = 0.f;
   a.gsave = gamma; a.ldg = ldg;
+  a.vx = nullptr; a.ldvx = 0;
   window_taps(d, a.tapidx);
   a.nt_store = (long long)d->N * d->H * d->W * C * 4 >= (256ll << 20);
   a.groups = (C + 31) / 32;
diff --git a/ssunet-gan_amd/csrc/conv_wgrad4.hip b/ssunet-gan_amd/csrc/conv_wgrad4.hip
--- a/ssunet-gan_amd/csrc/conv_wgrad4.hip
+++ b/ssunet-gan_amd/csrc/conv_wgrad4.hip
@@ -1,5 +1,6 @@
 #include "common.h"
 #include "conv_thin.h"
+#include "conv_wgrad_args.h"
 
 namespace {
 
@@ -9,6 +10,7 @@
   int groups, nz;
   long long units_per_z;
   int segs_per_row;
+  const float* vx; int ldvx;
 };
 
 constexpr int SEG = 32;
@@ -101,6 +103,7 @@
   }
 }
 
+template <bool VIRT = false>
 __global__ __launch_bounds__(256) void wgrad32_cin_kernel(const W4Args a) {
   const int lane = threadIdx.x & 63, l31 = lane & 31, h = lane >> 5;
   const int wave = threadIdx.x >> 6;
@@ -109,11 +112,18 @@
   const unsigned npix = (unsigned)(a.N * a.H * a.W);
   const auto do_rs = __builtin_amdgcn_make_buffer_rsrc(const_cast<float*>(a.wide), 0, (int)(npix * (unsigned)a.ldw * 4u), 0x00020000);
   const auto in_rs = __builtin_amdgcn_make_buffer_rsrc(const_cast<float*>(a.thin), 0, (int)(npix * (unsigned)a.ldt * 4u), 0x00020000);
+  const auto vx_rs = __builtin_amdgcn_make_buffer_rsrc(const_cast<float*>(VIRT ? a.vx : a.wide), 0,
+                                                       (int)(npix * (unsigned)(VIRT ? a.ldvx : a.ldw) * 4u), 0x00020000);
   constexpr unsigned OOB = 0xffffffffu;
-  const unsigned ldwb = (unsigned)a.ldw * 4u, ldtb = (unsigned)a.ldt * 4u;
+  const unsigned ldwb = (unsigned)a.ldw * 4u, ldtb = (unsigned)a.ldt * 4u, ldvb = (unsigned)a.ldvx * 4u;
+  const int Cmod = a.Cout >> 1;
   unsigned aoff[2];
 #pragma unroll
-  for (int f = 0; f < 2; ++f) { const int co = cg * 64 + f * 32 + l31; aoff[f] = co < a.Cout ? (unsigned)co * 4u : OOB; }
+  for (int f = 0; f < 2; ++f) {
+    const int co = cg * 64 + f * 32 + l31;
+    if (VIRT) aoff[f] = cg * 32 + l31 < Cmod ? (unsigned)(cg * 32 + l31) * 4u : OOB;
+    else aoff[f] = co < a.Cout ? (unsigned)co * 4u : OOB;
+  }
   const int t0 = l31 >> 2, c = l31 & 3;
   const int dy0 = t0 / 3 - 1, dx0 = t0 % 3 - 1;
   const bool has1 = l31 < 4;
@@ -146,15 +156,25 @@
         const int x = xb + 2 * k + h;
         const bool pok = x < x1;
         const unsigned po = (rowpix + (unsigned)x) * ldwb;
-#pragma unroll
-        for (int f = 0; f < 2; ++f)
-          av[f][k] = __builtin_bit_cast(float, __builtin_amdgcn_raw_buffer_load_b32(do_rs, (pok && aoff[f] != OOB) ? po + aoff[f] : OOB, 0, 0));
+        if constexpr (VIRT) {
+          const bool aok = pok && aoff[0] != OOB;
+          av[0][k] = __builtin_bit_cast(float, __builtin_amdgcn_raw_buffer_load_b32(vx_rs, aok ? (rowpix + (unsigned)x) * ldvb + aoff[0] : OOB, 0, 0));
+          av[1][k] = __builtin_bit_cast(float, __builtin_amdgcn_raw_buffer_load_b32(do_rs, aok ? po + aoff[0] : OOB, 0, 0));
+        } else {
+#pragma unroll
+          for (int f = 0; f < 2; ++f)
+            av[f][k] = __builtin_bit_cast(float, __builtin_amdgcn_raw_buffer_load_b32(do_rs, (pok && aoff[f] != OOB) ? po + aoff[f] : OOB, 0, 0));
+        }
         const int ix0 = x + dx0, ix1 = x + 1;
         bv[0][k] = __builtin_bit_cast(float, __builtin_amdgcn_raw_buffer_load_b32(
             in_rs, (pok && r0ok && (unsigned)ix0 < (unsigned)a.W) ? b0row + (unsigned)ix0 * ldtb : OOB, 0, 0));
         bv[1][k] = __builtin_bit_cast(float, __builtin_amdgcn_raw_buffer_load_b32(
             in_rs, (pok && r1ok && ix1 < a.W) ? b1row + (unsigned)ix1 * ldtb : OOB, 0, 0));
       }
+      if constexpr (VIRT) {
+#pragma unroll
+        for (int k = 0; k < UP; ++k) av[0][k] = av[1][k] * av[0][k];
+      }
 #pragma unroll
       for (int k = 0; k < UP; ++k)
 #pragma unroll
@@ -180,7 +200,8 @@
   for (int e = threadIdx.x; e < 36 * 64; e += 256) {
     const int nn = e >> 6, m = e & 63;
     const float sum = ((red[0][nn][m] + red[1][nn][m]) + red[2][nn][m]) + red[3][nn][m];
-    const int co = cg * 64 + m;
+    const int cm = cg * 32 + (m & 31);
+    const int co = VIRT ? (cm < Cmod ? (m >> 5) * Cmod + cm : a.Cout) : cg * 64 + m;
     if (co < a.Cout) slab[(size_t)nn * a.Cout + co] = sum;
   }
 }
@@ -270,6 +291,7 @@
 
 int ssg_wgrad4_launch(const ssg_wgrad_desc* d, int kind, hipStream_t st) {
   W4Args a;
+  a.vx = nullptr; a.ldvx = 0;
   a.ws = d->ws; a.N = d->N; a.H = d->H; a.W = d->W; a.Cout = d->Cout; a.Cin = d->C1;
   a.nz = ssg_wgrad4_slices(d, kind, &a.groups, &a.units_per_z, &a.segs_per_row);
   const dim3 grid((unsigned)(a.nz * a.groups)), block(256);
@@ -281,7 +303,7 @@
   }
   if (kind == 8) {
     a.wide = d->dout; a.Cw = d->Cout; a.ldw = d->ldd; a.thin = d->in1; a.ldt = d->ld1;
-    hipLaunchKernelGGL(wgrad32_cin_kernel, grid, block, 0, st, a);
+    hipLaunchKernelGGL(wgrad32_cin_kernel<false>, grid, block, 0, st, a);
     SSG_LAUNCH_CHECK();
     return SSG_OK;
   }
@@ -294,3 +316,33 @@
   SSG_LAUNCH_CHECK();
   return SSG_OK;
 }
+
+extern "C" int ssg_spade_wgrad_virtual_ok(const ssg_wgrad_desc* d, int lddy, const float* x, int ldx) {
+  if (!d || !d->in1 || !d->dout || !x || d->in_scale || d->C2 != 0 || d->N <= 0 || d->H <= 0 || d->W <= 0) return 0;
+  if (d->Cout < 64 || d->Cout % 64 || d->ldd < d->Cout || d->ldd % 4 || d->ld1 % 4 || d->ld1 < d->C1) return 0;
+  if (ssg_wgrad4_kind(d) != 8) return 0;
+  if (d->KH != 3 || d->KW != 3 || d->Cin_real <= 0 || d->Cin_real > d->C1) return 0;
+  for (int t = 0; t < 9; ++t) if (d->ky[t] != t / 3 || d->kx[t] != t % 3) return 0;
+  const int C = d->Cout / 2;
+  if (lddy % 4 || ldx % 4 || lddy < C || ldx < C) return 0;
+  if (((uintptr_t)d->in1 & 15) || ((uintptr_t)d->dout & 15) || ((uintptr_t)x & 15)) return 0;
+  const long long npix = (long long)d->N * d->H * d->W;
+  if (npix * lddy >= (1ll << 30) || npix * ldx >= (1ll << 30)) return 0;
+  return 1;
+}
+
+extern "C" int ssg_spade_wgrad_virtual_f32(const ssg_wgrad_desc* d, int lddy, const float* x, int ldx, void* stream) {
+  SSG_REQUIRE(ssg_spade_wgrad_virtual_ok(d, lddy, x, ldx), SSG_EINVAL,
+              "spade_wgrad_virtual: not handled (ssg_spade_wgrad_virtual_ok == 0: 4 -> 2C, C % 32 == 0, 3x3, >= 65536 pixels, aligned rows, strides % 4, < 2^30 elements)");
+  SSG_REQUIRE(d->dw_oihw && d->ws && !((uintptr_t)d->ws & 15), SSG_EINVAL, "spade_wgrad_virtual: dw_oihw / ws");
+  W4Args a;
+  a.ws = d->ws; a.N = d->N; a.H = d->H; a.W = d->W; a.Cout = d->Cout; a.Cin = d->C1;
+  a.nz = ssg_wgrad4_slices(d, 8, &a.groups, &a.units_per_z, &a.segs_per_row);
+  SSG_REQUIRE(d->ws_bytes >= (int64_t)a.nz * 9 * d->C1 * d->Cout * (int64_t)sizeof(float), SSG_EINVAL, "spade_wgrad_virtual: workspace too small");
+  a.wide = d->dout; a.Cw = d->Cout; a.ldw = lddy; a.thin = d->in1; a.ldt = d->ld1;
+  a.vx = x; a.ldvx = ldx;
+  hipStream_t st = (hipStream_t)stream;
+  hipLaunchKernelGGL(wgrad32_cin_kernel<true>, dim3((unsigned)(a.nz * a.groups)), dim3(256), 0, st, a);
+  SSG_LAUNCH_CHECK();
+  return ssg_wgrad_reduce_launch(d, a.nz, st);
+}
diff --git a/ssunet-gan_amd/ops.py b/ssunet-gan_amd/ops.py
--- a/ssunet-gan_amd/ops.py
+++ b/ssunet-gan_amd/ops.py
@@ -508,6 +508,82 @@
     return dw
 
 
+SPADE_BWD_VIRTUAL = _os.environ.get('SSG_SPADE_BWD_VIRTUAL', '1') != '0'
+SPADE_DGB_ALLOCS = [0]
+
+
+def _spade_wgrad_virtual_desc(a, dy, weight_shape, pad):
+    o, i, kh, kw = weight_shape
+    d = _wgrad_desc(a, pad4(a.shape[1]), None, 0, dy, weight_shape, 1, _taps_fwd(kh, kw, pad))
+    d.ldd = pad4(o)
+    d.flags = 1 if MFMA_SPLIT else 0
+    return d
+
+
+def _spade_wgrad_virtual(a, dy, x, weight_shape, pad):
+    o, i, kh, kw = weight_shape
+    n, _, oh, ow = dy.shape
+    d = _spade_wgrad_virtual_desc(a, dy, weight_shape, pad)
+    dw = torch.empty((o, i, kh, kw), device=dy.device, dtype=torch.float32)
+    d.dw_oihw = dw.data_ptr()
+    ws = _ws(call('ssg_conv2d_wgrad_workspace_bytes', C.byref(d)), dy.device)
+    d.ws = ws.data_ptr(); d.ws_bytes = ws.numel() * 8
+    _timed_call(_WGRAD_KIND, 'ssg_spade_wgrad_virtual_f32', d, (_ld(dy), ptr(x), _ld(x)), (n, oh, ow, i, o, kh, 1),
+                2.0 * n * oh * ow * o * i * kh * kw)
+    return dw
+
+
+def _spade_dgrad_desc(src, n, weight, pad, h, w, res, out, cout):
+    o, i, kh, kw = weight.shape
+    cred_pad = pad4(o)
+    pt, _, pl, _ = _pad4(pad)
+    taps = [(ky, kx, pt - ky, pl - kx) for ky in range(kh) for kx in range(kw)]
+    wpk, kp, kmode = _pack(weight, 1, taps, cred_pad, cred_pad)
+    return _conv_desc(src, cred_pad, None, 0, (n, h, w), wpk.data_ptr(), kp, kmode, None, res, out, cout, (h, w, h, w), 1, 1, (0, 0),
+                      taps, ACT_NONE, 0.0), len(taps)
+
+
+def _spade_dgrad_virtual(dy, x, weight, pad, out=None):
+    o, nh, kh, kw = weight.shape
+    n, _, h, w = dy.shape
+    probe = out is None
+    da = out
+    d, nt = _spade_dgrad_desc((dy.data_ptr(), pad4(o)), n, weight, pad, h, w, None, (16, pad4(nh)) if probe else _at(da), nh)
+    if probe:
+        return call('ssg_spade_dgrad_virtual_ok', C.byref(d), _ld(dy), ptr(x), _ld(x)) != 0
+    _timed_call(_CONV_KIND, 'ssg_spade_dgrad_virtual_f32', d, (_ld(dy), ptr(x), _ld(x)), (n, h, w, o, nh, nt, 1, 1),
+                2.0 * n * h * w * nh * o * nt)
+    return da
+
+
+def _spade_dgrad_dx(dseg, seg_c, weight, pad, c, dy, gamma, out=None):
+    n, _, h, w = dy.shape
+    probe = out is None
+    dx = out
+    d, nt = _spade_dgrad_desc((16, pad4(seg_c)) if probe else _at(dseg), n, weight, pad, h, w, _at(dy),
+                              (16, pad4(c)) if probe else _at(dx), c)
+    if probe:
+        return call('ssg_spade_dgrad_dx_ok', C.byref(d), ptr(gamma), _ld(gamma)) != 0
+    _timed_call(_CONV_KIND, 'ssg_spade_dgrad_dx_f32', d, (ptr(gamma), _ld(gamma)), (n, h, w, seg_c, c, nt, 1, 1),
+                2.0 * n * h * w * c * seg_c * nt)
+    return dx
+
+
+def _spade_bwd_virtual_ok(x, dy, a, gamma, wgb, wx, seg_c, pad, need_dx):
+    if not SPADE_BWD_VIRTUAL or x.dtype != torch.float32 or dy.dtype != torch.float32:
+        return False
+    n, c, h, w = x.shape
+    if n * h * w < 65536:
+        return False
+    if not call('ssg_spade_bwd_sums_ok', ptr(x), _ld(x), ptr(dy), _ld(dy), n * h * w, c):
+        return False
+    if not call('ssg_spade_wgrad_virtual_ok', C.byref(_spade_wgrad_virtual_desc(a, dy, wgb.shape, pad)), _ld(dy), ptr(x), _ld(x)):
+        return False
+    if not _spade_dgrad_virtual(dy, x, wgb, pad):
+        return False
+    return not need_dx or _spade_dgrad_dx(None, seg_c, wx, pad, c, dy, gamma)
+
+
 def _channel_sum(x, c):
     n, _, h, w = x.shape
     p = n * h * w
```

Result: no change. 85.97 images/sec (median of 6 runs) (+0.8%).
